# xaskasdf/ntransformer

Measured on AMD Instinct MI355X. Metric: decode tokens/sec (Llama-3.1-8B Q8_0 class, resident weights, greedy, batch 1), higher is better.
Workload: dtype f32; 1 GPU; Llama-3.1-8B-shaped Q8_0 GGUF tensors (seed 20260925), resident in HBM, 16-token prompt, greedy decode; ctx=4096, replicas=1, hipgraph=True

## Files before the change

### include/ntk_engine.h

```cpp
#ifndef NTK_ENGINE_H
#define NTK_ENGINE_H

#include "ntk.h"

#if defined(__GNUC__)
#pragma GCC visibility push(default)
#endif
#ifdef __cplusplus
extern "C" {
#endif

int ntk_rope_kv_store(float* q, const float* k, const float* v, const int* positions, int seq_len, int n_heads, int n_kv_heads, int head_dim,
                      float theta_base, float freq_scale, int interleaved, void* k_cache, void* v_cache, int start_pos, int max_seq, void* stream);
typedef struct ntk_gemv_seg {
    const void* W;
    float*      y;
    int         rows;
    int         dtype;
} ntk_gemv_seg;

int ntk_gemv_fused(const ntk_gemv_seg* segs, int nseg, const float* x, int in_features, const float* norm_w,
                   float eps, const float* resid, int silu_pair, void* stream);

size_t ntk_q8l_bytes(int rows, int in_features);
int ntk_q8l_pack(void* dst, const void* raw, int rows, int in_features, void* stream);
int ntk_q8l_unpack(void* raw, const void* packed, int rows, int in_features, void* stream);

size_t ntk_rp_bytes(int dtype, int rows, int in_features);
int ntk_rp_pack(void* dst, const void* raw, int rows, int in_features, int dtype, void* stream);
int ntk_rp_dequant(float* out, const void* rp, int rows, int in_features, int dtype, void* stream);
int ntk_rp_unpack(void* raw, const void* rp, int rows, int in_features, int dtype, void* stream);
int ntk_gemv_rp(float* y, const void* rp, const float* x, int out_features, int in_features, int weight_dtype, void* stream);
int ntk_gemv_rp_fused(const ntk_gemv_seg* segs, int nseg, const float* x, int in_features, const float* norm_w, float eps,
                      const float* resid, int silu_pair, void* stream);
int ntk_debug_rp_prologue(uint8_t* out, const float* x, const float* norm_w, float eps, int in_features, int nsub, int nwaves, void* stream);
int ntk_debug_mfma_i8_probe(int* D, const int8_t* A, const int8_t* B, void* stream);

int ntk_attention_decode_fused(float* output, const float* q, const float* k, const float* v, void* k_cache,
                               void* v_cache, const int* d_pos, const float* inv_freq, int n_heads, int n_kv_heads,
                               int head_dim, int max_seq, float scale, float theta_base, float freq_scale,
                               void* stream);

size_t ntk_attention_split_scratch_bytes(int n_heads, int head_dim, int nsplit);
int ntk_attention_decode_split(float* output, const float* q, const float* k, const float* v, void* k_cache,
                               void* v_cache, const int* d_pos, const float* inv_freq, int n_heads, int n_kv_heads,
                               int head_dim, int max_seq, float scale, float theta_base, float freq_scale, int nsplit,
                               float* scratch, void* stream);
int ntk_attention_split_scratch_init(float* scratch, int n_heads, void* stream);
int ntk_attention_decode_split_merged(float* output, const float* q, const float* k, const float* v, void* k_cache,
                                      void* v_cache, const int* d_pos, const float* inv_freq, int n_heads, int n_kv_heads,
                                      int head_dim, int max_seq, float scale, float theta_base, float freq_scale, int nsplit,
                                      float* scratch, void* stream);

#define NTK_ATTN_BATCH_MAX 16
typedef struct ntk_kv_batch {
    void* k[NTK_ATTN_BATCH_MAX];
    void* v[NTK_ATTN_BATCH_MAX];
} ntk_kv_batch;
int ntk_attention_decode_batch(float* output, const float* q, const float* k, const float* v, const ntk_kv_batch* caches, const int* positions,
                               int n_rows, const float* inv_freq, int n_heads, int n_kv_heads, int head_dim, int max_seq, float scale,
                               float theta_base, float freq_scale, int nsplit, float* scratch, void* stream);

size_t ntk_kv_q8_cache_bytes(int max_seq, int n_kv_heads, int head_dim);
int ntk_kv_store_q8(void* k_cache, void* v_cache, const float* k, const float* v, int seq_len, int n_kv_heads, int head_dim, int start_pos,
                    int max_seq, void* stream);
int ntk_rope_kv_store_q8(float* q, const float* k, const float* v, const int* positions, int seq_len, int n_heads, int n_kv_heads, int head_dim,
                         float theta_base, float freq_scale, int interleaved, void* k_cache, void* v_cache, int start_pos, int max_seq,
                         void* stream);
int ntk_attention_decode_q8(float* output, const float* q, const float* k, const float* v, void* k_cache, void* v_cache, const int* d_pos,
                            const float* inv_freq, int n_heads, int n_kv_heads, int head_dim, int max_seq, float scale, float theta_base,
                            float freq_scale, int nsplit, float* scratch, void* stream);
int ntk_kv_dequant_q8_f16(void* k_f16, void* v_f16, const void* k_cache, const void* v_cache, int n_rows, int n_kv_heads, int head_dim,
                          int max_seq, void* stream);

int ntk_debug_gemv_fused_form(const ntk_gemv_seg* segs, int nseg, const float* x, int in_features, const float* norm_w, float eps,
                              const float* resid, int silu_pair, int integer_activations, void* stream);

size_t   ntk_tp_comm_bytes(size_t max_floats);
void*    ntk_tp_comm_alloc(size_t bytes);
int      ntk_tp_comm_reset(void* comm, void* stream);
float*   ntk_tp_slot(void* comm, size_t max_floats, unsigned call_index);
int      ntk_tp_allreduce_add(float* hidden, void* const* peers, int rank, int world, size_t max_floats, unsigned call_index, int n, void* stream);
int      ntk_tp_advance_epoch(void* comm, void* stream);
unsigned ntk_tp_error(void* comm);
int      ntk_ipc_export(void* devptr, void* handle64);
int      ntk_ipc_open(const void* handle64, void** devptr);
int      ntk_ipc_close(void* devptr);

int ntk_gemm_quant(float* Y, const void* W, const float* X, int n_tokens, int out_features, int in_features,
                   int weight_dtype, const float* resid, void* stream);

typedef struct ntk_gemm_partials {
    const float* part[3];
    float*       y[3];
    int          rows[3];
    int          nseg, n_tokens, nsplit;
} ntk_gemm_partials;
typedef struct ntk_gemm_desc {
    const ntk_gemv_seg* segs;
    int                 nseg;
    const float*        X;
    int                 n_tokens, in_features;
    const float*        resid;
    void*               workspace;
    size_t              workspace_bytes;
    int                 reuse_x;
    const float*        row_max;
    ntk_gemm_partials*  partials;
    int                 weights_repacked;
    int                 full_form;
} ntk_gemm_desc;
size_t ntk_gemm_quant_workspace_bytes(int in_features, int out_features);
int ntk_gemm_quant_f16(const ntk_gemm_desc* desc, void* stream);
int ntk_reduce_rmsnorm_rowmax(float* hidden, const ntk_gemm_partials* partials, const float* weight, float eps, float* x_out, float* row_max,
                              float* zero_tokens, void* stream);
int ntk_reduce_silu_mul_rowmax(float* output, const ntk_gemm_partials* partials, float* row_max, void* stream);
int ntk_rmsnorm_rowmax(float* output, const float* input, const float* weight, int n_tokens, int hidden_size, float eps, float* row_max,
                       float* zero_tokens, void* stream);
int ntk_silu_mul_rowmax(float* output, const float* gate, const float* up, int n_tokens, int width, float* row_max, void* stream);
int ntk_gemm_prepare_x(const float* X, int n_tokens, int in_features, void* workspace, void* stream);
int ntk_rmsnorm_prepare_x(float* output, const float* input, const float* weight, int n_tokens, int hidden_size, float eps, void* workspace, void* stream);
int ntk_reduce_rmsnorm_prepare_x(float* hidden, const ntk_gemm_partials* partials, const float* weight, float eps, float* x_out, void* workspace, void* stream);
int ntk_silu_mul_prepare_x(float* output, const float* gate, const float* up, int n_tokens, int width, void* workspace, void* stream);
int ntk_reduce_silu_mul_prepare_x(float* output, const ntk_gemm_partials* partials, void* workspace, void* stream);

int ntk_embed_rows(float* out, const void* table, const int* tokens, int n_tokens, int hidden, int dtype,
                   void* stream);

int ntk_argmax(const float* logits, int n, int* d_out_token, int* h_mirror, float* scratch, void* stream);

int ntk_logprob_rows(const float* logits, int n_rows, int vocab, int ld, const int* targets, float* logprob, int* top1, void* stream);

size_t ntk_sample_scratch_bytes(int n);
int ntk_sample_top_k(float* logits, int n, const int* d_recent, int n_recent, float repeat_penalty, float temperature,
                     int top_k, float top_p, float r, int* d_out_token, int* h_mirror, void* scratch, void* stream);
int ntk_repeat_penalty(float* logits, int n, const int* d_recent, int n_recent, float repeat_penalty, void* stream);

#define NTK_SAMPLE_ROWS_MAX 16
typedef struct ntk_sample_rows {
    float temperature[NTK_SAMPLE_ROWS_MAX], top_p[NTK_SAMPLE_ROWS_MAX], repeat_penalty[NTK_SAMPLE_ROWS_MAX], r[NTK_SAMPLE_ROWS_MAX];
    int   top_k[NTK_SAMPLE_ROWS_MAX], n_recent[NTK_SAMPLE_ROWS_MAX];
} ntk_sample_rows;
size_t ntk_sample_rows_scratch_bytes(int n_rows, int vocab);
int ntk_sample_rows_top_k(float* logits, int n_rows, int vocab, int ld, const int* d_recent, int recent_ld, const ntk_sample_rows* rows, int* d_out,
                          int* h_mirror, void* scratch, void* stream);

int ntk_argmax_advance(const float* logits, int n, int* d_out_token, int* h_mirror, unsigned long long* h_ring4, int* d_pos,
                       float* scratch, void* stream);

int ntk_debug_sclk(unsigned long long* d_out2, void* stream);
int ntk_debug_sclk_begin(unsigned* d_flag, unsigned long long* d_out2, void* side_stream);
int ntk_debug_sclk_end(unsigned* d_flag, void* other_stream);

void ntk_debug_malloc_budget(long long bytes);

int ntk_advance_pos(int* d_pos, void* stream);

#ifdef __cplusplus
}
#endif
#if defined(__GNUC__)
#pragma GCC visibility pop
#endif
#endif
```

### ntransformer_amd/_lib.py

```python
from __future__ import annotations

import ctypes as C
import os

_HERE = os.path.dirname(os.path.abspath(__file__))
LIB_PATH = os.environ.get("NTK_LIB_PATH") or os.path.join(_HERE, "libntransformer_hip.so")

NTK_OK = 0
_STATUS = {0: "ok", -1: "unsupported dtype", -2: "bad shape", -3: "HIP launch/runtime error", -4: "misaligned pointer",
           -5: "null pointer", -6: "no usable GPU", -7: "out of memory", -8: "I/O error", -9: "malformed GGUF"}


class NtkError(RuntimeError):
    def __init__(self, status: int, what: str = ""):
        self.status = status
        super().__init__("ntk status %d (%s)%s" % (status, _STATUS.get(status, "?"), (": " + what) if what else ""))


def check(status: int, what: str = "") -> None:
    if status != NTK_OK:
        raise NtkError(status, what)


class KvBatch(C.Structure):
    _fields_ = [("k", C.c_void_p * 16), ("v", C.c_void_p * 16)]


class SampleRows(C.Structure):
    _fields_ = [("temperature", C.c_float * 16), ("top_p", C.c_float * 16), ("repeat_penalty", C.c_float * 16), ("r", C.c_float * 16),
                ("top_k", C.c_int * 16), ("n_recent", C.c_int * 16)]


class GemvSeg(C.Structure):
    _fields_ = [("W", C.c_void_p), ("y", C.c_void_p), ("rows", C.c_int), ("dtype", C.c_int)]


class GemmPartials(C.Structure):
    _fields_ = [("part", C.c_void_p * 3), ("y", C.c_void_p * 3), ("rows", C.c_int * 3), ("nseg", C.c_int), ("n_tokens", C.c_int), ("nsplit", C.c_int)]


class GemmDesc(C.Structure):
    _fields_ = [("segs", C.POINTER(GemvSeg)), ("nseg", C.c_int), ("X", C.c_void_p), ("n_tokens", C.c_int), ("in_features", C.c_int), ("resid", C.c_void_p),
                ("workspace", C.c_void_p), ("workspace_bytes", C.c_size_t), ("reuse_x", C.c_int), ("row_max", C.c_void_p),
                ("partials", C.POINTER(GemmPartials)), ("weights_repacked", C.c_int), ("full_form", C.c_int)]


_lib = None


def lib() -> C.CDLL:
    global _lib
    if _lib is not None:
        return _lib
    if not os.path.exists(LIB_PATH):
        raise ImportError("%s is missing: run `python -c 'import __graft_entry__ as g; g.build()'` "
                          "(hipcc --offload-arch=gfx950); there is no CPU fallback" % LIB_PATH)
    L = C.CDLL(LIB_PATH, mode=C.RTLD_GLOBAL)
    vp, i, f, sz = C.c_void_p, C.c_int, C.c_float, C.c_size_t
    sig = {
        "ntk_abi_version": (i, []),
        "ntk_status_string": (C.c_char_p, [i]),
        "ntk_row_bytes": (sz, [i, C.c_int64]),
        "ntk_device_count": (i, []),
        "ntk_device_init": (i, [i]),
        "ntk_device_name": (i, [C.c_char_p, sz]),
        "ntk_device_mem_info": (i, [C.POINTER(sz), C.POINTER(sz)]),
        "ntk_stream": (vp, [i]),
        "ntk_stream_synchronize": (i, [vp]),
        "ntk_device_synchronize": (i, []),
        "ntk_event_create": (vp, []),
        "ntk_event_destroy": (i, [vp]),
        "ntk_event_record": (i, [vp, vp]),
        "ntk_event_synchronize": (i, [vp]),
        "ntk_event_elapsed_ms": (i, [vp, vp, C.POINTER(f)]),
        "nt_hip_malloc": (vp, [sz]), "nt_hip_free": (None, [vp]),
        "nt_hip_memcpy_h2d": (None, [vp, vp, sz]), "nt_hip_memcpy_d2h": (None, [vp, vp, sz]),
        "nt_hip_memcpy_d2d": (None, [vp, vp, sz]), "nt_hip_memset": (None, [vp, i, sz]),
        "nt_hip_malloc_host": (vp, [sz]), "nt_hip_free_host": (None, [vp]),
        "ntk_memcpy_h2d_async": (i, [vp, vp, sz, vp]), "ntk_memcpy_d2h_async": (i, [vp, vp, sz, vp]),
        "nt_cuda_malloc": (vp, [sz]), "nt_cuda_free": (None, [vp]),
        "nt_cuda_memcpy_h2d": (None, [vp, vp, sz]), "nt_cuda_memcpy_d2h": (None, [vp, vp, sz]),
        "nt_cuda_memcpy_d2d": (None, [vp, vp, sz]), "nt_cuda_memset": (None, [vp, i, sz]),
        "nt_cuda_malloc_host": (vp, [sz]), "nt_cuda_free_host": (None, [vp]),
        "ntk_rmsnorm": (i, [vp, vp, vp, i, i, f, vp]),
        "ntk_rmsnorm_f16": (i, [vp, vp, vp, i, i, f, vp]),
        "ntk_rope": (i, [vp, vp, vp, i, i, i, i, i, f, f, i, vp]),
        "ntk_softmax": (i, [vp, vp, i, i, vp]),
        "ntk_masked_softmax": (i, [vp, vp, vp, i, i, vp]),
        "ntk_gemv": (i, [vp, vp, vp, i, i, i, vp]),
        "ntk_gemv_add": (i, [vp, vp, vp, i, i, i, vp]),
        "ntk_gemm_f32": (i, [vp, vp, vp, i, i, i, vp]),
        "ntk_silu_mul": (i, [vp, vp, vp, i, vp]),
        "ntk_rmsnorm_rowmax": (i, [vp, vp, vp, i, i, f, vp, vp, vp]),
        "ntk_rope_kv_store": (i, [vp, vp, vp, vp, i, i, i, i, f, f, i, vp, vp, i, i, vp]),
        "ntk_silu_mul_rowmax": (i, [vp, vp, vp, i, i, vp, vp]),
        "ntk_add_bias": (i, [vp, vp, i, vp]),
        "ntk_attention_decode": (i, [vp, vp, vp, vp, i, i, i, i, i, f, vp]),
        "ntk_attention_prefill": (i, [vp, vp, vp, vp, i, i, i, i, i, i, f, vp]),
        "ntk_copy_to_kv_cache": (i, [vp, vp, vp, vp, i, i, i, i, i, vp]),
        "ntk_add": (i, [vp, vp, vp, i, vp]),
        "ntk_add_inplace": (i, [vp, vp, i, vp]),
        "ntk_copy": (i, [vp, vp, i, vp]),
        "ntk_cosine_similarity": (i, [vp, vp, vp, i, vp]),
        "ntk_gemv_fused": (i, [C.POINTER(GemvSeg), i, vp, i, vp, f, vp, i, vp]),
        "ntk_debug_gemv_fused_form": (i, [C.POINTER(GemvSeg), i, vp, i, vp, f, vp, i, i, vp]),
        "ntk_q8l_bytes": (sz, [i, i]),
        "ntk_q8l_pack": (i, [vp, vp, i, i, vp]),
        "ntk_q8l_unpack": (i, [vp, vp, i, i, vp]),
        "ntk_rp_bytes": (sz, [i, i, i]),
        "ntk_rp_pack": (i, [vp, vp, i, i, i, vp]),
        "ntk_rp_dequant": (i, [vp, vp, i, i, i, vp]),
        "ntk_rp_unpack": (i, [vp, vp, i, i, i, vp]),
        "ntk_gemv_rp": (i, [vp, vp, vp, i, i, i, vp]),
        "ntk_gemv_rp_fused": (i, [C.POINTER(GemvSeg), i, vp, i, vp, f, vp, i, vp]),
        "ntk_debug_rp_prologue": (i, [vp, vp, vp, f, i, i, i, vp]),
        "ntk_debug_mfma_i8_probe": (i, [vp, vp, vp, vp]),
        "ntk_gemm_quant": (i, [vp, vp, vp, i, i, i, i, vp, vp]),
        "ntk_attention_decode_split": (i, [vp, vp, vp, vp, vp, vp, vp, vp, i, i, i, i, f, f, f, i, vp, vp]),
        "ntk_attention_split_scratch_bytes": (C.c_size_t, [i, i, i]),
        "ntk_attention_split_scratch_init": (i, [vp, i, vp]),
        "ntk_attention_decode_split_merged": (i, [vp, vp, vp, vp, vp, vp, vp, vp, i, i, i, i, f, f, f, i, vp, vp]),
        "ntk_attention_decode_fused": (i, [vp, vp, vp, vp, vp, vp, vp, vp, i, i, i, i, f, f, f, vp]),
        "ntk_attention_decode_batch": (i, [vp, vp, vp, vp, vp, vp, i, vp, i, i, i, i, f, f, f, i, vp, vp]),
        "ntk_kv_q8_cache_bytes": (C.c_size_t, [i, i, i]),
        "ntk_kv_store_q8": (i, [vp, vp, vp, vp, i, i, i, i, i, vp]),
        "ntk_rope_kv_store_q8": (i, [vp, vp, vp, vp, i, i, i, i, f, f, i, vp, vp, i, i, vp]),
        "ntk_attention_decode_q8": (i, [vp, vp, vp, vp, vp, vp, vp, vp, i, i, i, i, f, f, f, i, vp, vp]),
        "ntk_kv_dequant_q8_f16": (i, [vp, vp, vp, vp, i, i, i, i, vp]),
        "ntk_embed_rows": (i, [vp, vp, vp, i, i, i, vp]),
        "ntk_argmax": (i, [vp, i, vp, vp, vp, vp]),
        "ntk_logprob_rows": (i, [vp, i, i, i, vp, vp, vp, vp]),
        "ntk_sample_rows_scratch_bytes": (C.c_size_t, [i, i]),
        "ntk_sample_rows_top_k": (i, [vp, i, i, i, vp, i, C.POINTER(SampleRows), vp, vp, vp, vp]),
        "ntk_advance_pos": (i, [vp, vp]),
        "ntk_debug_sclk": (i, [vp, vp]),
        "ntk_debug_sclk_begin": (i, [vp, vp, vp]),
        "ntk_debug_sclk_end": (i, [vp, vp]),
    }
    for name, (res, args) in sig.items():
        fn = getattr(L, name)
        fn.restype = res
        fn.argtypes = args
    _lib = L
    return L


EXPORTS_NTK_H = None
```

### ntransformer_amd/csrc/attention.hip

```cpp
#include "common.hip.h"
#include "attention_merge.hip.h"
#include "attention_decode.hip.h"
#include <cfloat>
#include <cstdlib>

namespace ntk {

template <int LPR>
__global__ __launch_bounds__(256) void attention_kernel(float* __restrict__ output, const float* __restrict__ Q,
                                                        const uint16_t* __restrict__ kc, const uint16_t* __restrict__ vc,
                                                        int n_keys_base, int causal, int n_heads, int n_kv_heads, int hd,
                                                        float scale) {
    extern __shared__ __attribute__((aligned(16))) float lds[];
    const int head = blockIdx.x, qi = blockIdx.y;
    const int n_keys = causal ? n_keys_base + qi + 1 : n_keys_base;
    float* qs = lds;
    float* red = qs + hd;
    float* part = red + 16;
    float* sc = part + (blockDim.x >> 6) * hd;
    const size_t qoff = ((size_t)qi * n_heads + head) * hd;
    for (int d = threadIdx.x; d < hd; d += blockDim.x) qs[d] = Q[qoff + d];
    __syncthreads();
    attend<LPR>(output + qoff, qs, kc, vc, n_keys, nullptr, nullptr, head / (n_heads / n_kv_heads), n_kv_heads, hd,
                scale, sc, part, red);
}

template <int LPR>
__global__ __launch_bounds__(256) void attention_decode_fused_kernel(
    float* __restrict__ output, const float* __restrict__ q, const float* __restrict__ k, const float* __restrict__ v,
    uint16_t* __restrict__ kc, uint16_t* __restrict__ vc, const int* __restrict__ d_pos, int n_heads, int n_kv_heads,
    int hd, int max_seq, float scale, float theta, float fscale) {
    attention_decode_fused_row<LPR>(output, q, k, v, kc, vc, d_pos, n_heads, n_kv_heads, hd, max_seq, scale, theta, fscale, (int)blockIdx.x);
}


template <int LPR, int D>
__global__ __launch_bounds__(256) void attention_decode_fused_v3_kernel(
    float* __restrict__ output, const float* __restrict__ q, const float* __restrict__ k, const float* __restrict__ v,
    uint16_t* __restrict__ kc, uint16_t* __restrict__ vc, const int* __restrict__ d_pos, const float* __restrict__ inv_freq,
    int n_heads, int n_kv_heads, int hd, int max_seq, float scale, float theta, float fscale) {
    attention_decode_walk<LPR, D, false>(output, q, k, v, kc, vc, d_pos, inv_freq, n_heads, n_kv_heads, hd, max_seq, scale, theta, fscale,
                                         (int)blockIdx.x, 0, 1);
}

template <int LPR, int D, bool MERGE>
__global__ __launch_bounds__(256) void attention_decode_split_kernel(
    float* __restrict__ part, const float* __restrict__ q, const float* __restrict__ k, const float* __restrict__ v,
    uint16_t* __restrict__ kc, uint16_t* __restrict__ vc, const int* __restrict__ d_pos, const float* __restrict__ inv_freq,
    int n_heads, int n_kv_heads, int hd, int max_seq, float scale, float theta, float fscale, float* __restrict__ output,
    unsigned* __restrict__ counters) {
    const int group = n_heads / n_kv_heads;
    const int kv_head = blockIdx.x % n_kv_heads, head = kv_head * group + blockIdx.x / n_kv_heads;
    const int sp = blockIdx.y, nsplit = gridDim.y;
    attention_decode_walk<LPR, D, true, MERGE>(part + ((size_t)head * nsplit + sp) * (hd + 2), q, k, v, kc, vc, d_pos, inv_freq, n_heads,
                                               n_kv_heads, hd, max_seq, scale, theta, fscale, head, sp, nsplit);
    if constexpr (MERGE) {
        extern __shared__ __attribute__((aligned(16))) float lds[];
        if (!att_merge_arrive(counters + head, nsplit, (int)threadIdx.x, reinterpret_cast<volatile int*>(lds))) return;
        const int wave = (int)threadIdx.x >> 6, lane = (int)threadIdx.x & 63;
        if (64 * wave < hd)
            att_merge_head_wave<1>(output + (size_t)head * hd, part + (size_t)head * nsplit * (hd + 2), hd, nsplit, lane, 64 * wave + lane);
    }
}

__global__ __launch_bounds__(128) void attention_split_combine_kernel(float* __restrict__ output, const float* __restrict__ part,
                                                                      int hd, int nsplit, int n_kv_heads) {
    attention_split_combine_head(output, part, hd, nsplit, n_kv_heads, (int)blockIdx.x, (int)gridDim.x);
}

constexpr int FA_QT = 32;
constexpr int FA_KT = 64;
constexpr int FA_QPW = 8;

template <int LPR>
__global__ __launch_bounds__(256) void attention_prefill_tiled_kernel(float* __restrict__ output, const float* __restrict__ Q,
                                                                     const uint16_t* __restrict__ kc, const uint16_t* __restrict__ vc,
                                                                     int T, int start_pos, int n_heads, int n_kv_heads, float scale) {
    constexpr int HD = 8 * LPR, PPW = 64 / LPR;
    extern __shared__ __attribute__((aligned(16))) uint8_t fa_lds[];
    uint16_t* kt = reinterpret_cast<uint16_t*>(fa_lds);
    uint16_t* vt = kt + FA_KT * HD;
    float* qt = reinterpret_cast<float*>(vt + FA_KT * HD);
    const int head = blockIdx.x, q0 = blockIdx.y * FA_QT;
    const int tid = threadIdx.x, lane = tid & 63, wave = tid >> 6;
    const int kv_head = head / (n_heads / n_kv_heads);
    const size_t stride = (size_t)n_kv_heads * HD;
    const int sub = lane / LPR, part_i = lane % LPR;
    const int nq = min(FA_QT, T - q0);
    for (int i = tid; i < nq * HD; i += 256) qt[i] = Q[((size_t)(q0 + i / HD) * n_heads + head) * HD + (i % HD)];
    float m[FA_QPW], l[FA_QPW], acc[FA_QPW][8];
#pragma unroll
    for (int u = 0; u < FA_QPW; ++u) {
        m[u] = -INFINITY; l[u] = 0.0f;
#pragma unroll
        for (int j = 0; j < 8; ++j) acc[u][j] = 0.0f;
    }
    const int n_keys = start_pos + q0 + nq;
    for (int k0 = 0; k0 < n_keys; k0 += FA_KT) {
        __syncthreads();
        const int nk = min(FA_KT, n_keys - k0);
        for (int i = tid; i < nk * LPR; i += 256) {
            const int r = i / LPR, c = i % LPR;
            const size_t g = (size_t)(k0 + r) * stride + (size_t)kv_head * HD + 8 * c;
            *reinterpret_cast<u32x4*>(kt + r * HD + 8 * c) = *reinterpret_cast<const u32x4*>(kc + g);
            *reinterpret_cast<u32x4*>(vt + r * HD + 8 * c) = *reinterpret_cast<const u32x4*>(vc + g);
        }
        __syncthreads();
#pragma unroll
        for (int u = 0; u < FA_QPW; ++u) {
            const int qi = wave * FA_QPW + u;
            if (qi >= nq) continue;
            const int last = start_pos + q0 + qi;
            if (k0 > last) continue;
            float qreg[8];
#pragma unroll
            for (int j = 0; j < 8; ++j) qreg[j] = qt[qi * HD + 8 * part_i + j];
            const int kend = min(nk, last - k0 + 1);
            for (int r0 = 0; r0 < kend; r0 += PPW) {
                const int r = r0 + sub, rr = min(r, kend - 1);
                float kf[8], vf[8];
                unpack8(*reinterpret_cast<const u32x4*>(kt + rr * HD + 8 * part_i), kf);
                unpack8(*reinterpret_cast<const u32x4*>(vt + rr * HD + 8 * part_i), vf);
                float sc = 0.0f;
#pragma unroll
                for (int j = 0; j < 8; ++j) sc = fmaf(qreg[j], kf[j], sc);
                sc = group_sum<LPR>(sc);
                sc = r < kend ? sc * scale : -INFINITY;
                const float mn = fmaxf(m[u], sc);
                const float a = (mn == -INFINITY) ? 1.0f : expf(m[u] - mn), pw = (mn == -INFINITY) ? 0.0f : expf(sc - mn);
                l[u] = fmaf(l[u], a, pw);
#pragma unroll
                for (int j = 0; j < 8; ++j) acc[u][j] = fmaf(acc[u][j], a, pw * vf[j]);
                m[u] = mn;
            }
        }
    }
#pragma unroll
    for (int u = 0; u < FA_QPW; ++u) {
        const int qi = wave * FA_QPW + u;
        if (qi >= nq) continue;
        float mm = m[u], ll = l[u];
#pragma unroll
        for (int off = LPR; off < 64; off <<= 1) {
            const float mo = __shfl_xor(mm, off, 64), lo = __shfl_xor(ll, off, 64);
            const float mn = fmaxf(mm, mo);
            const float wa = (mm == -INFINITY) ? 0.0f : expf(mm - mn), wb = (mo == -INFINITY) ? 0.0f : expf(mo - mn);
            ll = fmaf(ll, wa, lo * wb);
#pragma unroll
            for (int j = 0; j < 8; ++j) acc[u][j] = fmaf(acc[u][j], wa, __shfl_xor(acc[u][j], off, 64) * wb);
            mm = mn;
        }
        if (sub == 0) {
            const float inv = ll > 0.0f ? 1.0f / ll : 0.0f;
            float* o = output + ((size_t)(q0 + qi) * n_heads + head) * HD + 8 * part_i;
#pragma unroll
            for (int j = 0; j < 8; ++j) o[j] = acc[u][j] * inv;
        }
    }
}

__global__ void rope_kernel(float* __restrict__ q, float* __restrict__ k, const int* __restrict__ positions, int seq_len,
                            int n_heads, int n_kv_heads, int head_dim, float theta, float fscale, int interleaved) {
    const int idx = blockIdx.x * blockDim.x + threadIdx.x;
    const int half_dim = head_dim / 2;
    const int total_q = seq_len * n_heads * half_dim, total_k = seq_len * n_kv_heads * half_dim;
    if (idx >= total_q + total_k) return;
    const bool is_key = idx >= total_q;
    const int local = is_key ? idx - total_q : idx;
    const int n_h = is_key ? n_kv_heads : n_heads;
    const int pair = local % half_dim, head = (local / half_dim) % n_h, sp = local / (half_dim * n_h);
    float* data = (is_key ? k : q) + ((size_t)sp * n_h + head) * head_dim;
    const int i0 = interleaved ? 2 * pair : pair, i1 = interleaved ? 2 * pair + 1 : pair + half_dim;
    float a = data[i0], b = data[i1];
    rope_pair(a, b, positions[sp], pair, head_dim, theta, fscale);
    data[i0] = a;
    data[i1] = b;
}

__global__ __launch_bounds__(256) void rope_rows_kernel(float* __restrict__ q, float* __restrict__ k, const int* __restrict__ positions,
                                                        int n_heads, int n_kv_heads, int head_dim, float theta, float fscale, int interleaved) {
    __shared__ float cs[2][128];
    const int sp = blockIdx.x, half_dim = head_dim / 2;
    const int pos = positions[sp];
    for (int i = threadIdx.x; i < half_dim; i += blockDim.x) {
        const float freq = 1.0f / (float)pow((double)theta, (double)((2.0f * i) / head_dim));
        const float angle = pos * freq * fscale;
        cs[0][i] = cosf(angle);
        cs[1][i] = sinf(angle);
    }
    __syncthreads();
    const int total = (n_heads + n_kv_heads) * half_dim;
    for (int idx = threadIdx.x; idx < total; idx += blockDim.x) {
        const int pair = idx % half_dim, head = idx / half_dim;
        float* data = head < n_heads ? q + ((size_t)sp * n_heads + head) * head_dim : k + ((size_t)sp * n_kv_heads + (head - n_heads)) * head_dim;
        const int i0 = interleaved ? 2 * pair : pair, i1 = interleaved ? 2 * pair + 1 : pair + half_dim;
// ... 20 lines not shown
    const bool store = cp < max_seq;
    const int total = (n_heads + n_kv_heads) * half_dim;
    for (int idx = threadIdx.x; idx < total; idx += blockDim.x) {
        const int pair = idx % half_dim, head = idx / half_dim;
        const int i0 = interleaved ? 2 * pair : pair, i1 = interleaved ? 2 * pair + 1 : pair + half_dim;
        const float c = cs[0][pair], sn = cs[1][pair];
        if (head < n_heads) {
            float* data = q + ((size_t)sp * n_heads + head) * head_dim;
            const float a = data[i0], b = data[i1];
            rope_rotate(a, b, c, sn, data[i0], data[i1]);
        } else {
            const int kh = head - n_heads;
            const float* data = k + ((size_t)sp * n_kv_heads + kh) * head_dim;
            float ra, rb;
            rope_rotate(data[i0], data[i1], c, sn, ra, rb);
            if (store) {
                uint16_t* row = kc + (size_t)cp * per_pos + (size_t)kh * head_dim;
                row[i0] = f2h(ra);
                row[i1] = f2h(rb);
            }
        }
    }
    if (store)
        for (int e = threadIdx.x; e < per_pos; e += blockDim.x) vc[(size_t)cp * per_pos + e] = f2h(v[(size_t)sp * per_pos + e]);
}

__global__ void kv_store_kernel(uint16_t* __restrict__ kc, uint16_t* __restrict__ vc, const float* __restrict__ k,
                                const float* __restrict__ v, int total, int per_pos, int start_pos, int max_seq) {
    const int idx = blockIdx.x * blockDim.x + threadIdx.x;
    if (idx >= total) return;
    const int t = idx / per_pos, e = idx % per_pos;
    const int cp = start_pos + t;
    if (cp >= max_seq) return;
    kc[(size_t)cp * per_pos + e] = f2h(k[idx]);
    vc[(size_t)cp * per_pos + e] = f2h(v[idx]);
}

static size_t attn_lds(int hd, int n_keys, int nvec) {
    return sizeof(float) * ((size_t)nvec * hd + 16 + 4 * (size_t)hd + (size_t)n_keys + 1);
}

int launch_attention_decode_kvhead_mfma(float* part, const float* q, const float* k, const float* v, uint16_t* kc, uint16_t* vc,
                                        const int* d_pos, const float* inv_freq, int nh, int nkv, int max_seq, float scale, float theta,
                                        float fscale, int nsplit, float* merged_output, unsigned* counters, hipStream_t st);
int launch_attention_prefill_mfma(float* out, const float* Q, const uint16_t* kc, const uint16_t* vc, int T, int start_pos, int nh, int nkv,
                                  int hd, float scale, hipStream_t st);

static int launch_attention(float* out, const float* Q, const void* kc, const void* vc, int T, int n_keys_base, int causal,
                            int nh, int nkv, int hd, float scale, hipStream_t st) {
    if (nh <= 0 || nkv <= 0 || hd <= 0 || nh % nkv != 0 || T < 0) return NTK_E_SHAPE;
    if (T == 0) return NTK_OK;
    const int max_keys = causal ? n_keys_base + T : n_keys_base;
    const bool aligned = (reinterpret_cast<uintptr_t>(kc) & 15) == 0 && (reinterpret_cast<uintptr_t>(vc) & 15) == 0;
    const uint16_t* k16 = static_cast<const uint16_t*>(kc);
    const uint16_t* v16 = static_cast<const uint16_t*>(vc);
    static const bool tiled_off = NTK_TUNE_ENV_INT("NTK_PREFILL_ATTENTION_1TO1", 0) != 0;
    static const bool mfma_off = NTK_TUNE_ENV_INT("NTK_PREFILL_ATTENTION_NO_MFMA", 0) != 0;
    if (causal && T > 1 && aligned && hd == 128 && !tiled_off && !mfma_off) {
        const int rc = launch_attention_prefill_mfma(out, Q, k16, v16, T, n_keys_base, nh, nkv, hd, scale, st);
        if (rc != NTK_E_SHAPE && rc != NTK_E_ALIGN) return rc;
    }
    if (causal && T > 1 && aligned && (hd == 64 || hd == 128 || hd == 256) && !tiled_off) {
        const size_t fl = (size_t)2 * FA_KT * hd * sizeof(uint16_t) + (size_t)FA_QT * hd * sizeof(float);
        const dim3 fgrid(nh, (T + FA_QT - 1) / FA_QT);
        if (hd == 128) hipLaunchKernelGGL(attention_prefill_tiled_kernel<16>, fgrid, dim3(256), fl, st, out, Q, k16, v16, T, n_keys_base, nh, nkv, scale);
        else if (hd == 64) hipLaunchKernelGGL(attention_prefill_tiled_kernel<8>, fgrid, dim3(256), fl, st, out, Q, k16, v16, T, n_keys_base, nh, nkv, scale);
        else {
            static bool once = hipFuncSetAttribute(reinterpret_cast<const void*>(attention_prefill_tiled_kernel<32>),
                                                   hipFuncAttributeMaxDynamicSharedMemorySize, (int)fl) == hipSuccess;
            if (!once) return NTK_E_LAUNCH;
            hipLaunchKernelGGL(attention_prefill_tiled_kernel<32>, fgrid, dim3(256), fl, st, out, Q, k16, v16, T, n_keys_base, nh, nkv, scale);
        }
        return last_launch_status();
    }
    const size_t lds = attn_lds(hd, max_keys, 1);
    if (lds > 160 * 1024) return NTK_E_SHAPE;
    dim3 grid(nh, T), block(256);
#define NTK_ATT(LPR_)                                                                                                   \
    do {                                                                                                                \
        if (lds > 64 * 1024)                                                                                            \
            (void)hipFuncSetAttribute(reinterpret_cast<const void*>(attention_kernel<LPR_>),                            \
                                      hipFuncAttributeMaxDynamicSharedMemorySize, (int)lds);                            \
        hipLaunchKernelGGL(attention_kernel<LPR_>, grid, block, lds, st, out, Q, k16, v16, n_keys_base, causal, nh, nkv, hd, scale); \
    } while (0)
    if (aligned && hd == 128) NTK_ATT(16);
    else if (aligned && hd == 64) NTK_ATT(8);
    else if (aligned && hd == 256) NTK_ATT(32);
    else NTK_ATT(0);
#undef NTK_ATT
    return last_launch_status();
}

int launch_attention_split_combine(float* output, const float* part, int n_heads, int hd, int nsplit, int n_kv_heads, hipStream_t st) {
    hipLaunchKernelGGL(attention_split_combine_kernel, dim3(n_heads), dim3(128), 0, st, output, part, hd, nsplit, n_kv_heads);
    return last_launch_status();
}

}

extern "C" {

int ntk_rope(float* q, float* k, const int* positions, int , int seq_len, int n_heads, int n_kv_heads,
             int head_dim, float theta_base, float freq_scale, int interleaved, void* stream) {
    if (!q || !k || !positions) return NTK_E_NULL;
    if (seq_len < 0 || n_heads < 0 || n_kv_heads < 0 || head_dim <= 0 || (head_dim & 1)) return NTK_E_SHAPE;
    const int total = seq_len * (n_heads + n_kv_heads) * (head_dim / 2);
    if (total == 0) return NTK_OK;
    if (seq_len >= 4 && head_dim <= 256)
        hipLaunchKernelGGL(ntk::rope_rows_kernel, dim3(seq_len), dim3(256), 0, ntk::resolve_stream(stream), q, k, positions, n_heads, n_kv_heads,
                           head_dim, theta_base, freq_scale, interleaved);
    else
        hipLaunchKernelGGL(ntk::rope_kernel, dim3((total + 255) / 256), dim3(256), 0, ntk::resolve_stream(stream), q, k,
                           positions, seq_len, n_heads, n_kv_heads, head_dim, theta_base, freq_scale, interleaved);
    return ntk::last_launch_status();
}

int ntk_rope_kv_store(float* q, const float* k, const float* v, const int* positions, int seq_len, int n_heads, int n_kv_heads, int head_dim,
                      float theta_base, float freq_scale, int interleaved, void* k_cache, void* v_cache, int start_pos, int max_seq, void* stream) {
    if (!q || !k || !v || !positions || !k_cache || !v_cache) return NTK_E_NULL;
    if (seq_len < 0 || n_heads <= 0 || n_kv_heads <= 0 || head_dim <= 0 || (head_dim & 1) || head_dim > 256 || start_pos < 0 || max_seq <= 0) return NTK_E_SHAPE;
    if (seq_len == 0) return NTK_OK;
    hipLaunchKernelGGL(ntk::rope_kv_store_rows_kernel, dim3(seq_len), dim3(256), 0, ntk::resolve_stream(stream), q, k, v, positions, n_heads, n_kv_heads,
                       head_dim, theta_base, freq_scale, interleaved, static_cast<uint16_t*>(k_cache), static_cast<uint16_t*>(v_cache), start_pos, max_seq);
    return ntk::last_launch_status();
}

int ntk_copy_to_kv_cache(void* k_cache, void* v_cache, const float* k, const float* v, int seq_len, int n_kv_heads,
                         int head_dim, int start_pos, int max_seq, void* stream) {
    if (!k_cache || !v_cache || !k || !v) return NTK_E_NULL;
    if (seq_len < 0 || n_kv_heads <= 0 || head_dim <= 0 || start_pos < 0) return NTK_E_SHAPE;
    const int per = n_kv_heads * head_dim, total = seq_len * per;
    if (total == 0) return NTK_OK;
    hipLaunchKernelGGL(ntk::kv_store_kernel, dim3((total + 255) / 256), dim3(256), 0, ntk::resolve_stream(stream),
                       static_cast<uint16_t*>(k_cache), static_cast<uint16_t*>(v_cache), k, v, total, per, start_pos, max_seq);
    return ntk::last_launch_status();
}

int ntk_attention_decode(float* output, const float* q, const void* k_cache, const void* v_cache, int seq_len, int n_heads,
                         int n_kv_heads, int head_dim, int , float scale, void* stream) {
    if (!output || !q || !k_cache || !v_cache) return NTK_E_NULL;
    if (seq_len <= 0) return NTK_E_SHAPE;
    return ntk::launch_attention(output, q, k_cache, v_cache, 1, seq_len, 0, n_heads, n_kv_heads, head_dim, scale,
                                 ntk::resolve_stream(stream));
}

int ntk_attention_prefill(float* output, const float* Q, const void* k_cache, const void* v_cache, int seq_len, int start_pos,
                          int n_heads, int n_kv_heads, int head_dim, int , float scale, void* stream) {
    if (!output || !Q || !k_cache || !v_cache) return NTK_E_NULL;
    if (seq_len < 0 || start_pos < 0) return NTK_E_SHAPE;
    return ntk::launch_attention(output, Q, k_cache, v_cache, seq_len, start_pos, 1, n_heads, n_kv_heads, head_dim, scale,
                                 ntk::resolve_stream(stream));
}

int ntk_attention_decode_fused(float* output, const float* q, const float* k, const float* v, void* k_cache, void* v_cache,
                               const int* d_pos, const float* inv_freq, int n_heads, int n_kv_heads, int head_dim, int max_seq,
                               float scale, float theta_base, float freq_scale, void* stream) {
    if (!output || !q || !k || !v || !k_cache || !v_cache || !d_pos) return NTK_E_NULL;
    if (n_heads <= 0 || n_kv_heads <= 0 || n_heads % n_kv_heads != 0 || head_dim <= 0 || (head_dim & 1) || max_seq <= 0)
        return NTK_E_SHAPE;
    if ((size_t)max_seq * n_kv_heads * head_dim * 2 >= 0xF0000000ull) return NTK_E_SHAPE;
    hipStream_t st = ntk::resolve_stream(stream);
    const bool aligned = (reinterpret_cast<uintptr_t>(k_cache) & 15) == 0 && (reinterpret_cast<uintptr_t>(v_cache) & 15) == 0;
    uint16_t* k16 = static_cast<uint16_t*>(k_cache);
    uint16_t* v16 = static_cast<uint16_t*>(v_cache);
    if (aligned && (head_dim == 128 || head_dim == 64 || head_dim == 256)) {
        const int G = 4 * (64 / (head_dim / 8));
        const size_t lds = sizeof(float) * ((size_t)3 * head_dim + 2 * G + (size_t)G * head_dim);
#define NTK_ATTV(...) hipLaunchKernelGGL((ntk::attention_decode_fused_v3_kernel<__VA_ARGS__>), dim3(n_heads), dim3(256), lds, st, output, q, k, v, \
                                           k16, v16, d_pos, inv_freq, n_heads, n_kv_heads, head_dim, max_seq, scale, theta_base, freq_scale)
        if (head_dim == 128) NTK_ATTV(16, 4);
        else if (head_dim == 64) NTK_ATTV(8, 4);
        else NTK_ATTV(32, 4);
#undef NTK_ATTV
        return ntk::last_launch_status();
    }
    const size_t lds = ntk::attn_lds(head_dim, max_seq, 3);
    if (lds > 160 * 1024) return NTK_E_SHAPE;
    if (lds > 64 * 1024)
        (void)hipFuncSetAttribute(reinterpret_cast<const void*>(ntk::attention_decode_fused_kernel<0>),
                                  hipFuncAttributeMaxDynamicSharedMemorySize, (int)lds);
    hipLaunchKernelGGL(ntk::attention_decode_fused_kernel<0>, dim3(n_heads), dim3(256), lds, st, output, q, k, v, k16, v16, d_pos,
                       n_heads, n_kv_heads, head_dim, max_seq, scale, theta_base, freq_scale);
    return ntk::last_launch_status();
}

size_t ntk_attention_split_scratch_bytes(int n_heads, int head_dim, int nsplit) {
    return ntk::att_merge_header_bytes(n_heads) + (size_t)n_heads * (size_t)nsplit * (size_t)(head_dim + 2) * sizeof(float);
}

int ntk_attention_split_scratch_init(float* scratch, int n_heads, void* stream) {
    if (!scratch) return NTK_E_NULL;
    if (n_heads <= 0) return NTK_E_SHAPE;
    return hipMemsetAsync(scratch, 0, ntk::att_merge_header_bytes(n_heads), ntk::resolve_stream(stream)) == hipSuccess ? NTK_OK : NTK_E_LAUNCH;
}

static int attention_decode_split_impl(float* output, const float* q, const float* k, const float* v, void* k_cache, void* v_cache,
                                       const int* d_pos, const float* inv_freq, int n_heads, int n_kv_heads, int head_dim, int max_seq,
                                       float scale, float theta_base, float freq_scale, int nsplit, float* scratch_all, void* stream, bool merged) {
    if (!output || !q || !k || !v || !k_cache || !v_cache || !d_pos || !scratch_all) return NTK_E_NULL;
    if (n_heads <= 0 || n_kv_heads <= 0 || n_heads % n_kv_heads != 0 || max_seq <= 0 || nsplit < 1 || nsplit > 1024)
        return NTK_E_SHAPE;
    if (merged && nsplit > ntk::ATT_MERGE_MAX_SPLITS) return NTK_E_SHAPE;
    unsigned* counters = reinterpret_cast<unsigned*>(scratch_all);
    float* scratch = reinterpret_cast<float*>(reinterpret_cast<uint8_t*>(scratch_all) + ntk::att_merge_header_bytes(n_heads));
    if (head_dim != 128 && head_dim != 64 && head_dim != 256) return NTK_E_SHAPE;
    if ((size_t)max_seq * n_kv_heads * head_dim * 2 >= 0xF0000000ull) return NTK_E_SHAPE;
    if ((reinterpret_cast<uintptr_t>(k_cache) & 15) || (reinterpret_cast<uintptr_t>(v_cache) & 15)) return NTK_E_ALIGN;
    hipStream_t st = ntk::resolve_stream(stream);
    uint16_t* k16 = static_cast<uint16_t*>(k_cache);
    uint16_t* v16 = static_cast<uint16_t*>(v_cache);
    static const int kvhead_form = NTK_TUNE_ENV_INT("NTK_ATTN_KVHEAD", 1);
    if (head_dim == 128 && n_heads / n_kv_heads <= 16 && ((kvhead_form == 1 && nsplit >= 16) || kvhead_form == 2)) {
        const int rc = ntk::launch_attention_decode_kvhead_mfma(scratch, q, k, v, k16, v16, d_pos, inv_freq, n_heads, n_kv_heads, max_seq,
                                                                scale, theta_base, freq_scale, nsplit, merged ? output : nullptr, counters, st);
        if (rc != NTK_OK || merged) return rc;
        hipLaunchKernelGGL(ntk::attention_split_combine_kernel, dim3(n_heads), dim3(128), 0, st, output, scratch, head_dim, nsplit, n_kv_heads);
        return ntk::last_launch_status();
    }
    const int G = 4 * (64 / (head_dim / 8));
    const size_t lds = sizeof(float) * ((size_t)3 * head_dim + 2 * G + (size_t)G * head_dim);
#define NTK_ATTSP(...) hipLaunchKernelGGL((ntk::attention_decode_split_kernel<__VA_ARGS__>), dim3(n_heads, nsplit), dim3(256), lds, st, scratch, q, k, \
                                           v, k16, v16, d_pos, inv_freq, n_heads, n_kv_heads, head_dim, max_seq, scale, theta_base, freq_scale, output, counters)
    static const int split_d = NTK_TUNE_ENV_INT("NTK_ATTN_SPLIT_D", 4);
    if (merged) {
        if (head_dim == 128) NTK_ATTSP(16, 4, true);
        else if (head_dim == 64) NTK_ATTSP(8, 4, true);
        else NTK_ATTSP(32, 4, true);
        return ntk::last_launch_status();
    }
    if (head_dim == 128 && split_d == 8) NTK_ATTSP(16, 8, false);
    else if (head_dim == 128) NTK_ATTSP(16, 4, false);
    else if (head_dim == 64) NTK_ATTSP(8, 4, false);
    else NTK_ATTSP(32, 4, false);
#undef NTK_ATTSP
    if (ntk::last_launch_status() != NTK_OK) return NTK_E_LAUNCH;
    hipLaunchKernelGGL(ntk::attention_split_combine_kernel, dim3(n_heads), dim3(128), 0, st, output, scratch, head_dim, nsplit, n_kv_heads);
    return ntk::last_launch_status();
}

int ntk_attention_decode_split(float* output, const float* q, const float* k, const float* v, void* k_cache, void* v_cache,
                               const int* d_pos, const float* inv_freq, int n_heads, int n_kv_heads, int head_dim, int max_seq,
                               float scale, float theta_base, float freq_scale, int nsplit, float* scratch, void* stream) {
    return attention_decode_split_impl(output, q, k, v, k_cache, v_cache, d_pos, inv_freq, n_heads, n_kv_heads, head_dim, max_seq, scale, theta_base,
                                       freq_scale, nsplit, scratch, stream, false);
}

int ntk_attention_decode_split_merged(float* output, const float* q, const float* k, const float* v, void* k_cache, void* v_cache,
                                      const int* d_pos, const float* inv_freq, int n_heads, int n_kv_heads, int head_dim, int max_seq,
                                      float scale, float theta_base, float freq_scale, int nsplit, float* scratch, void* stream) {
    return attention_decode_split_impl(output, q, k, v, k_cache, v_cache, d_pos, inv_freq, n_heads, n_kv_heads, head_dim, max_seq, scale, theta_base,
                                       freq_scale, nsplit, scratch, stream, true);
}

}
```

### ntransformer_amd/csrc/attention_decode.hip.h

```cpp
#pragma once
#include "common.hip.h"
#include "attention_merge.hip.h"
#include <cfloat>
#include <cstdlib>

namespace ntk {

typedef uint32_t u32x4 __attribute__((ext_vector_type(4)));

__device__ __forceinline__ void unpack8(const u32x4 r, float (&f)[8]) {
    f[0] = h2f((uint16_t)(r.x & 0xFFFF)); f[1] = h2f((uint16_t)(r.x >> 16));
    f[2] = h2f((uint16_t)(r.y & 0xFFFF)); f[3] = h2f((uint16_t)(r.y >> 16));
    f[4] = h2f((uint16_t)(r.z & 0xFFFF)); f[5] = h2f((uint16_t)(r.z >> 16));
    f[6] = h2f((uint16_t)(r.w & 0xFFFF)); f[7] = h2f((uint16_t)(r.w >> 16));
}

#ifdef NTK_ATTN_NO_ASM
__device__ __forceinline__ void pv_update(float (&acc)[8], const u32x4 r, const float p) {
    const uint32_t w[4] = {r.x, r.y, r.z, r.w};
#pragma unroll
    for (int i = 0; i < 4; ++i) {
        acc[2 * i] = fmaf(p, h2f((uint16_t)(w[i] & 0xFFFFu)), acc[2 * i]);
        acc[2 * i + 1] = fmaf(p, h2f((uint16_t)(w[i] >> 16)), acc[2 * i + 1]);
    }
}
#else
__device__ __forceinline__ void pv_update(float (&acc)[8], const u32x4 r, const float p) {
    asm("s_nop 1\n\t"
        "v_fma_mix_f32 %0, %8, %12, %0 op_sel_hi:[1,0,0]\n\t"
        "v_fma_mix_f32 %1, %8, %12, %1 op_sel:[1,0,0] op_sel_hi:[1,0,0]\n\t"
        "v_fma_mix_f32 %2, %9, %12, %2 op_sel_hi:[1,0,0]\n\t"
        "v_fma_mix_f32 %3, %9, %12, %3 op_sel:[1,0,0] op_sel_hi:[1,0,0]\n\t"
        "v_fma_mix_f32 %4, %10, %12, %4 op_sel_hi:[1,0,0]\n\t"
        "v_fma_mix_f32 %5, %10, %12, %5 op_sel:[1,0,0] op_sel_hi:[1,0,0]\n\t"
        "v_fma_mix_f32 %6, %11, %12, %6 op_sel_hi:[1,0,0]\n\t"
        "v_fma_mix_f32 %7, %11, %12, %7 op_sel:[1,0,0] op_sel_hi:[1,0,0]"
        : "+v"(acc[0]), "+v"(acc[1]), "+v"(acc[2]), "+v"(acc[3]), "+v"(acc[4]), "+v"(acc[5]), "+v"(acc[6]), "+v"(acc[7])
        : "v"(r.x), "v"(r.y), "v"(r.z), "v"(r.w), "v"(p));
}
#endif

__device__ __forceinline__ void rope_pair(float& x0, float& x1, int pos, int pair_idx, int head_dim, float theta, float fscale) {
    const float freq = 1.0f / (float)pow((double)theta, (double)((2.0f * pair_idx) / head_dim));
    const float angle = pos * freq * fscale;
    const float c = cosf(angle), s = sinf(angle);
    const float a = x0, b = x1;
    rope_rotate(a, b, c, s, x0, x1);
}

template <int LPR>
__device__ void attend(float* out, const float* qs, const uint16_t* kc, const uint16_t* vc, int n_cache,
                       const float* k_extra, const float* v_extra, int kv_head, int n_kv_heads, int hd,
                       float scale, float* sc, float* part, float* red) {
    const int tid = threadIdx.x, lane = tid & 63, wave = tid >> 6, nwaves = blockDim.x >> 6;
    const size_t stride = (size_t)n_kv_heads * hd;
    const uint16_t* kbase = kc + (size_t)kv_head * hd;
    const uint16_t* vbase = vc + (size_t)kv_head * hd;
    const int n_keys = n_cache + (k_extra ? 1 : 0);

    if constexpr (LPR > 0) {
        constexpr int PPW = 64 / LPR;
        const int sub = lane / LPR, part_i = lane % LPR;
        float qreg[8];
#pragma unroll
        for (int j = 0; j < 8; ++j) qreg[j] = qs[8 * part_i + j];
        for (int p0 = wave * PPW; p0 < n_cache; p0 += nwaves * PPW) {
            const int pos = p0 + sub;
            float s = 0.0f;
            if (pos < n_cache) {
                const u32x4 raw = *reinterpret_cast<const u32x4*>(kbase + pos * stride + 8 * part_i);
                float kf[8];
                unpack8(raw, kf);
#pragma unroll
                for (int j = 0; j < 8; ++j) s = fmaf(qreg[j], kf[j], s);
            }
            s = group_sum<LPR>(s);
            if (part_i == 0 && pos < n_cache) sc[pos] = s * scale;
        }
    } else {
        for (int pos = tid; pos < n_cache; pos += blockDim.x) {
            const uint16_t* k = kbase + pos * stride;
            float s = 0.0f;
            for (int d = 0; d < hd; ++d) s = fmaf(qs[d], h2f(k[d]), s);
            sc[pos] = s * scale;
        }
    }
    if (k_extra && wave == 0) {
        float s = 0.0f;
        for (int d = lane; d < hd; d += 64) s = fmaf(qs[d], k_extra[d], s);
        s = wave_sum(s);
        if (lane == 0) sc[n_cache] = s * scale;
    }
    __syncthreads();

    float m = -FLT_MAX;
    for (int pos = tid; pos < n_keys; pos += blockDim.x) m = fmaxf(m, sc[pos]);
    m = block_max(m, red);
    float l = 0.0f;
    for (int pos = tid; pos < n_keys; pos += blockDim.x) {
        const float e = expf(sc[pos] - m);
        sc[pos] = e;
        l += e;
    }
    l = block_sum(l, red);
    const float inv = (l > 0.0f) ? 1.0f / l : 0.0f;
    __syncthreads();

    if constexpr (LPR > 0) {
        constexpr int PPW = 64 / LPR;
        const int sub = lane / LPR, part_i = lane % LPR;
        float acc[8];
#pragma unroll
        for (int j = 0; j < 8; ++j) acc[j] = 0.0f;
        for (int p0 = wave * PPW; p0 < n_cache; p0 += nwaves * PPW) {
            const int pos = p0 + sub;
            if (pos < n_cache) {
                const float pw = sc[pos];
                const u32x4 raw = *reinterpret_cast<const u32x4*>(vbase + pos * stride + 8 * part_i);
                float vf[8];
                unpack8(raw, vf);
#pragma unroll
                for (int j = 0; j < 8; ++j) acc[j] = fmaf(pw, vf[j], acc[j]);
            }
        }
#pragma unroll
        for (int off = LPR; off < 64; off <<= 1) {
#pragma unroll
            for (int j = 0; j < 8; ++j) acc[j] += __shfl_xor(acc[j], off, 64);
        }
        if (sub == 0) {
#pragma unroll
            for (int j = 0; j < 8; ++j) part[wave * hd + 8 * part_i + j] = acc[j];
        }
        __syncthreads();
        for (int d = tid; d < hd; d += blockDim.x) {
            float t = 0.0f;
            for (int w = 0; w < nwaves; ++w) t += part[w * hd + d];
            if (v_extra) t = fmaf(sc[n_cache], v_extra[d], t);
            out[d] = t * inv;
        }
    } else {
        for (int d = tid; d < hd; d += blockDim.x) {
            float t = 0.0f;
            for (int pos = 0; pos < n_cache; ++pos) t = fmaf(sc[pos], h2f(vbase[pos * stride + d]), t);
            if (v_extra) t = fmaf(sc[n_cache], v_extra[d], t);
            out[d] = t * inv;
        }
    }
}

template <int LPR>
__device__ __forceinline__ void attention_decode_fused_row(
    float* __restrict__ output, const float* __restrict__ q, const float* __restrict__ k, const float* __restrict__ v,
    uint16_t* __restrict__ kc, uint16_t* __restrict__ vc, const int* __restrict__ d_pos, int n_heads, int n_kv_heads,
    int hd, int max_seq, float scale, float theta, float fscale, const int head) {
    extern __shared__ __attribute__((aligned(16))) float lds[];
    const int group = n_heads / n_kv_heads, kv_head = head / group;
    const int pos = *d_pos;
    float* qs = lds;
    float* kx = qs + hd;
    float* vx = kx + hd;
    float* red = vx + hd;
    float* part = red + 16;
    float* sc = part + (blockDim.x >> 6) * hd;
    const int half_dim = hd / 2;
    const size_t cache_row = ((size_t)pos * n_kv_heads + kv_head) * hd;
    const bool writer = (head % group == 0) && pos < max_seq;
    for (int i = threadIdx.x; i < half_dim; i += blockDim.x) {
        float a = q[(size_t)head * hd + i], b = q[(size_t)head * hd + i + half_dim];
        rope_pair(a, b, pos, i, hd, theta, fscale);
        qs[i] = a; qs[i + half_dim] = b;
        float ka = k[(size_t)kv_head * hd + i], kb = k[(size_t)kv_head * hd + i + half_dim];
        rope_pair(ka, kb, pos, i, hd, theta, fscale);
        const uint16_t ha = f2h(ka), hb = f2h(kb);
        kx[i] = h2f(ha); kx[i + half_dim] = h2f(hb);
        if (writer) { kc[cache_row + i] = ha; kc[cache_row + i + half_dim] = hb; }
    }
    for (int i = threadIdx.x; i < hd; i += blockDim.x) {
        const uint16_t hv = f2h(v[(size_t)kv_head * hd + i]);
        vx[i] = h2f(hv);
        if (writer) vc[cache_row + i] = hv;
    }
    __syncthreads();
    attend<LPR>(output + (size_t)head * hd, qs, kc, vc, pos, kx, vx, kv_head, n_kv_heads, hd, scale, sc, part, red);
}

template <int LPR, int D, bool SPLIT, bool MERGE = false>
__device__ __forceinline__ void attention_decode_walk(
    float* __restrict__ output, const float* __restrict__ q, const float* __restrict__ k, const float* __restrict__ v,
    uint16_t* __restrict__ kc, uint16_t* __restrict__ vc, const int* __restrict__ d_pos, const float* __restrict__ inv_freq,
    const int n_heads, const int n_kv_heads, const int hd, const int max_seq, const float scale, const float theta, const float fscale,
    const int head, const int sp, const int nsplit) {
    constexpr int PPW = 64 / LPR, NW = 4, G = NW * PPW;
    constexpr float EMPTY = -3.0e38f;
    extern __shared__ __attribute__((aligned(16))) float lds[];
    const int tid = threadIdx.x, lane = tid & 63, wave = tid >> 6;
    const int group = n_heads / n_kv_heads, kv_head = head / group;
    const int stepG = nsplit * G, first = sp * G;
    float* qs = lds;
    float* kx = qs + hd;
    float* vx = kx + hd;
    float* ms = vx + hd;
    float* ls = ms + G;
    float* accs = ls + G;
    const int half_dim = hd / 2;
    const size_t stride = (size_t)n_kv_heads * hd;
    const int sub = lane / LPR, part_i = lane % LPR, g = wave * PPW + sub;
    const uint16_t* kbase = kc + (size_t)kv_head * hd + 8 * part_i;
    const uint16_t* vbase = vc + (size_t)kv_head * hd + 8 * part_i;
    const int pmax = max_seq - 1;

    const int ri = tid & 63, role = tid >> 6;
    float in_a = 0.0f, in_b = 0.0f, in_c = 0.0f, in_d = 0.0f, freq = 0.0f;
    const bool rot = role < 2 && ri < half_dim;
    if (rot) {
        const float* src = role == 0 ? q + (size_t)head * hd : k + (size_t)kv_head * hd;
        in_a = src[ri]; in_b = src[ri + half_dim];
        freq = inv_freq ? inv_freq[ri] : 1.0f / (float)pow((double)theta, (double)((2.0f * ri) / hd));
        if (half_dim > 64) { in_c = src[ri + 64]; in_d = src[ri + 64 + half_dim]; }
    }
    float vin0 = 0.0f, vin1 = 0.0f;
    const int vi = tid - 128;
    if (role >= 2) {
        if (vi < hd) vin0 = v[(size_t)kv_head * hd + vi];
        if (vi + 128 < hd) vin1 = v[(size_t)kv_head * hd + vi + 128];
    }

    const unsigned row_bytes = (unsigned)stride * 2u, off_max = (unsigned)pmax * row_bytes, adv = (unsigned)(stepG * D) * row_bytes;
    const char* kb = reinterpret_cast<const char*>(kbase);
    const char* vb = reinterpret_cast<const char*>(vbase);
    unsigned roff[D];
    u32x4 kraw[D], vraw[D];
#pragma unroll
    for (int d = 0; d < D; ++d) {
        roff[d] = min((unsigned)(first + g + stepG * d) * row_bytes, off_max);
        kraw[d] = *reinterpret_cast<const u32x4*>(kb + roff[d]);
        vraw[d] = *reinterpret_cast<const u32x4*>(vb + roff[d]);
    }
    const int pos = *d_pos;
    const size_t cache_row = (size_t)pos * stride + (size_t)kv_head * hd;
    const bool writer = (head % group == 0) && sp == 0 && pos < max_seq;
    uint16_t st_h[4] = {0, 0, 0, 0};
    if (rot) {
        auto rotate = [&](const int i, const float a, const float b, const float f, uint16_t& ha, uint16_t& hb) {
            const float angle = pos * f * fscale;
            float c, sn;
            sincosf(angle, &sn, &c);
            float ra, rb;
            rope_rotate(a, b, c, sn, ra, rb);
            if (role == 0) { qs[i] = ra; qs[i + half_dim] = rb; }
            else {
                ha = f2h(ra); hb = f2h(rb);
                kx[i] = h2f(ha); kx[i + half_dim] = h2f(hb);
            }
        };
        rotate(ri, in_a, in_b, freq, st_h[0], st_h[1]);
        if (half_dim > 64) {
            const int i2 = ri + 64;
            const float f2 = inv_freq ? inv_freq[i2] : 1.0f / (float)pow((double)theta, (double)((2.0f * i2) / hd));
            rotate(i2, in_c, in_d, f2, st_h[2], st_h[3]);
        }
    }
    if (role >= 2) {
        if (vi < hd) { st_h[0] = f2h(vin0); vx[vi] = h2f(st_h[0]); }
        if (vi + 128 < hd) { st_h[1] = f2h(vin1); vx[vi + 128] = h2f(st_h[1]); }
    }
    __syncthreads();

    float qreg[8];
#pragma unroll
    for (int j = 0; j < 8; ++j) qreg[j] = qs[8 * part_i + j];
    float m = EMPTY, l = 0.0f, acc[8];
#pragma unroll
    for (int j = 0; j < 8; ++j) acc[j] = 0.0f;
    auto batch = [&](const float (*kf)[8], const u32x4* vr, const bool* valid, const int np, const bool masked) {
        float sc[D];
        float mn = m;
#pragma unroll
        for (int d = 0; d < D; ++d) {
            if (d >= np) { sc[d] = EMPTY; continue; }
            float t = 0.0f;
#pragma unroll
            for (int j = 0; j < 8; ++j) t = fmaf(qreg[j], kf[d][j], t);
            t = group_sum<LPR>(t) * scale;
            sc[d] = (!masked || valid[d]) ? t : EMPTY;
            mn = fmaxf(mn, sc[d]);
        }
        const float a = __expf(m - mn);
        l *= a;
#pragma unroll
        for (int j = 0; j < 8; ++j) acc[j] *= a;
#pragma unroll
        for (int d = 0; d < D; ++d) {
            if (d >= np) continue;
            const float pw = (!masked || valid[d]) ? __expf(sc[d] - mn) : 0.0f;
            l += pw;
            pv_update(acc, vr[d], pw);
        }
        m = mn;
    };
    auto walk_batch = [&](const int base, const bool masked) {
        float kf[D][8];
        u32x4 vr[D];
        bool valid[D];
#pragma unroll
        for (int d = 0; d < D; ++d) {
            valid[d] = base + g + stepG * d < pos;
            vr[d] = vraw[d];
            if (masked && !valid[d]) vr[d] = u32x4{0u, 0u, 0u, 0u};
            unpack8(kraw[d], kf[d]);
        }
        __builtin_amdgcn_sched_barrier(0);
        if (base + stepG * D < pos) {
#pragma unroll
            for (int d = 0; d < D; ++d) {
                roff[d] = min(roff[d] + adv, off_max);
                kraw[d] = *reinterpret_cast<const u32x4*>(kb + roff[d]);
                vraw[d] = *reinterpret_cast<const u32x4*>(vb + roff[d]);
            }
        }
        __builtin_amdgcn_sched_barrier(0);
        batch(kf, vr, valid, D, masked);
    };
    int base = first;
    for (; base + stepG * (D - 1) + G <= pos; base += stepG * D) walk_batch(base, false);
    if (base < pos) walk_batch(base, true);
    {
        float kf[D][8];
        u32x4 vr[D];
        bool valid[D];
#pragma unroll
        for (int j = 0; j < 8; ++j) kf[0][j] = kx[8 * part_i + j];
        {
            const float* vxp = vx + 8 * part_i;
            vr[0].x = (uint32_t)f2h(vxp[0]) | ((uint32_t)f2h(vxp[1]) << 16); vr[0].y = (uint32_t)f2h(vxp[2]) | ((uint32_t)f2h(vxp[3]) << 16);
            vr[0].z = (uint32_t)f2h(vxp[4]) | ((uint32_t)f2h(vxp[5]) << 16); vr[0].w = (uint32_t)f2h(vxp[6]) | ((uint32_t)f2h(vxp[7]) << 16);
        }
        valid[0] = first + g == pos % stepG;
        batch(kf, vr, valid, 1, true);
    }
    if (part_i == 0) { ms[g] = m; ls[g] = l; }
#pragma unroll
    for (int j = 0; j < 8; ++j) accs[g * hd + 8 * part_i + j] = acc[j];
    __syncthreads();
    float M = ms[0];
    for (int i = 1; i < G; ++i) M = fmaxf(M, ms[i]);
    if (tid < G) qs[tid] = expf(ms[tid] - M);
    __syncthreads();
    for (int d = tid; d < hd; d += blockDim.x) {
        float L = 0.0f, o = 0.0f;
        for (int i = 0; i < G; ++i) {
            const float w = qs[i];
            L = fmaf(w, ls[i], L);
            o = fmaf(w, accs[i * hd + d], o);
        }
        if constexpr (SPLIT) {
            att_part_store<MERGE>(output + d, o);
            if (d == 0) { att_part_store<MERGE>(output + hd, M); att_part_store<MERGE>(output + hd + 1, L); }
        } else {
            output[(size_t)head * hd + d] = o / L;
        }
    }
    if (writer) {
        if (role == 1 && rot) {
            kc[cache_row + ri] = st_h[0]; kc[cache_row + ri + half_dim] = st_h[1];
            if (half_dim > 64) { kc[cache_row + ri + 64] = st_h[2]; kc[cache_row + ri + 64 + half_dim] = st_h[3]; }
        }
        if (role >= 2) {
            if (vi < hd) vc[cache_row + vi] = st_h[0];
            if (vi + 128 < hd) vc[cache_row + vi + 128] = st_h[1];
        }
    }
}

__device__ __forceinline__ void attention_split_combine_head(float* __restrict__ output, const float* __restrict__ part, int hd, int nsplit,
                                                             int n_kv_heads, const int block, const int nblocks) {
    constexpr int B = 32;
    __shared__ __attribute__((aligned(16))) float wsh[1024], lsh[1024];
    const int group = nblocks / n_kv_heads;
    const int head = (block % n_kv_heads) * group + block / n_kv_heads, tid = threadIdx.x;
    const float* ph = part + (size_t)head * nsplit * (hd + 2);
    const int n32 = (nsplit + B - 1) / B * B;
    float mreg[8], lreg[8];
#pragma unroll
    for (int u = 0; u < 8; ++u) {
        mreg[u] = -INFINITY; lreg[u] = 0.0f;
        if (128 * u < nsplit) {
            const int s0 = tid + 128 * u;
            const float* ps = ph + (size_t)min(s0, nsplit - 1) * (hd + 2) + hd;
            const float mv = ps[0], lv = ps[1];
            if (s0 < nsplit) { mreg[u] = mv; lreg[u] = lv; }
        }
    }
    const int d0 = min(tid, hd - 1);
    float v0[B];
#pragma unroll
    for (int u = 0; u < B; ++u) v0[u] = ph[(size_t)min(u, nsplit - 1) * (hd + 2) + d0];
    __builtin_amdgcn_sched_barrier(0);
#pragma unroll
    for (int u = 0; u < 8; ++u)
        if (tid + 128 * u < n32) { wsh[tid + 128 * u] = mreg[u]; lsh[tid + 128 * u] = lreg[u]; }
    __syncthreads();
    float M = -INFINITY;
    for (int s0 = 0; s0 < n32; s0 += B) {
#pragma unroll
        for (int u = 0; u < B; ++u) M = fmaxf(M, wsh[s0 + u]);
    }
    __syncthreads();
#pragma unroll
    for (int u = 0; u < 8; ++u)
        if (tid + 128 * u < n32) wsh[tid + 128 * u] = (mreg[u] == -INFINITY) ? 0.0f : expf(mreg[u] - M);
    __syncthreads();
    float L = 0.0f;
// ... 24 lines not shown
```

### ntransformer_amd/csrc/elementwise.hip

```cpp
#include "common.hip.h"
#include <cfloat>

namespace ntk {

template <bool HALF_OUT>
__global__ __launch_bounds__(1024) void rmsnorm_kernel(void* __restrict__ output, const float* __restrict__ input,
                                                       const float* __restrict__ weight, int hidden, float eps) {
    __shared__ float red[16];
    const float* x = input + (size_t)blockIdx.x * hidden;
    float ssq = 0.0f;
    for (int i = threadIdx.x; i < hidden; i += blockDim.x) ssq = fmaf(x[i], x[i], ssq);
    const float tot = block_sum(ssq, red);
    const float rms_inv = 1.0f / sqrtf(tot / (float)hidden + eps);
    for (int i = threadIdx.x; i < hidden; i += blockDim.x) {
        const float v = x[i] * rms_inv * weight[i];
        if constexpr (HALF_OUT) reinterpret_cast<uint16_t*>(output)[(size_t)blockIdx.x * hidden + i] = f2h(v);
        else reinterpret_cast<float*>(output)[(size_t)blockIdx.x * hidden + i] = v;
    }
}

template <bool MASKED>
__global__ __launch_bounds__(1024) void softmax_kernel(float* __restrict__ out, const float* __restrict__ in,
                                                       const uint8_t* __restrict__ mask, int cols) {
    __shared__ float red[16];
    const float* x = in + (size_t)blockIdx.x * cols;
    const uint8_t* mk = MASKED ? mask + (size_t)blockIdx.x * cols : nullptr;
    float* y = out + (size_t)blockIdx.x * cols;
    float m = -FLT_MAX;
    for (int i = threadIdx.x; i < cols; i += blockDim.x)
        if (!MASKED || mk[i]) m = fmaxf(m, x[i]);
    m = block_max(m, red);
    float l = 0.0f;
    for (int i = threadIdx.x; i < cols; i += blockDim.x)
        if (!MASKED || mk[i]) l += expf(x[i] - m);
    l = block_sum(l, red);
    const float inv = l > 0.0f ? 1.0f / l : 0.0f;
    for (int i = threadIdx.x; i < cols; i += blockDim.x) y[i] = (!MASKED || mk[i]) ? expf(x[i] - m) * inv : 0.0f;
}

__global__ void silu_mul_kernel(float* __restrict__ out, const float* __restrict__ gate, const float* __restrict__ up, int n) {
    const int i = blockIdx.x * blockDim.x + threadIdx.x;
    if (i < n) {
        const float g = gate[i];
        out[i] = g / (1.0f + expf(-g)) * up[i];
    }
}
__global__ void add_kernel(float* __restrict__ o, const float* __restrict__ a, const float* __restrict__ b, int n) {
    const int i = blockIdx.x * blockDim.x + threadIdx.x;
    if (i < n) o[i] = a[i] + b[i];
}
__global__ void copy_kernel(float* __restrict__ d, const float* __restrict__ s, int n) {
    const int i = blockIdx.x * blockDim.x + threadIdx.x;
    if (i < n) d[i] = s[i];
}
__global__ void gemm_f32_kernel(float* __restrict__ C, const float* __restrict__ A, const float* __restrict__ B, int M, int N, int K) {
    const int col = blockIdx.x * blockDim.x + threadIdx.x, row = blockIdx.y * blockDim.y + threadIdx.y;
    if (row >= M || col >= N) return;
    float s = 0.0f;
    for (int k = 0; k < K; ++k) s = fmaf(A[(size_t)row * K + k], B[(size_t)col * K + k], s);
    C[(size_t)row * N + col] = s;
}
__global__ __launch_bounds__(256) void cosine_kernel(float* __restrict__ result, const float* __restrict__ a,
                                                     const float* __restrict__ b, int n) {
    __shared__ float red[16];
    float d = 0.0f, na = 0.0f, nb = 0.0f;
    for (int i = threadIdx.x; i < n; i += blockDim.x) {
        d = fmaf(a[i], b[i], d); na = fmaf(a[i], a[i], na); nb = fmaf(b[i], b[i], nb);
    }
    d = block_sum(d, red); na = block_sum(na, red); nb = block_sum(nb, red);
    if (threadIdx.x == 0) {
        const float den = sqrtf(na) * sqrtf(nb);
        *result = den > 1e-8f ? d / den : 0.0f;
    }
}

__device__ float embed_elem(const uint8_t* __restrict__ table, int tok, int hidden, int dt, int e) {
    switch (dt) {
        case NTK_DT_F32: return reinterpret_cast<const float*>(table)[(size_t)tok * hidden + e];
        case NTK_DT_F16: return h2f(reinterpret_cast<const uint16_t*>(table)[(size_t)tok * hidden + e]);
        case NTK_DT_Q8_0: {
            const uint8_t* b = table + ((size_t)tok * (hidden / 32) + e / 32) * 34;
            const float d = h2f((uint16_t)(b[0] | (b[1] << 8)));
            return __fmul_rn(d, (float)(int8_t)b[2 + (e & 31)]);
        }
        case NTK_DT_Q4_0: {
            const uint8_t* b = table + ((size_t)tok * (hidden / 32) + e / 32) * 18;
            const float d = h2f((uint16_t)(b[0] | (b[1] << 8)));
            const int j = e & 31;
            const int nib = j < 16 ? (b[2 + j] & 0x0F) : (b[2 + j - 16] >> 4);
            return __fmul_rn(d, (float)(nib - 8));
        }
        case NTK_DT_Q4_K: {
            const uint8_t* b = table + ((size_t)tok * (hidden / 256) + e / 256) * 144;
            const float d = h2f((uint16_t)(b[0] | (b[1] << 8))), dmin = h2f((uint16_t)(b[2] | (b[3] << 8)));
            const int w = e & 255, sub = w >> 5, l = w & 31, chunk = sub >> 1;
            const uint8_t* s = b + 4;
            uint32_t sc, mn;
            if (sub < 4) { sc = s[sub] & 63; mn = s[sub + 4] & 63; }
            else { sc = (s[sub + 4] & 0x0F) | ((s[sub - 4] >> 6) << 4); mn = (s[sub + 4] >> 4) | ((s[sub] >> 6) << 4); }
            const uint8_t qb = b[16 + 32 * chunk + l];
            const int nib = (sub & 1) ? (qb >> 4) : (qb & 0x0F);
            return __fsub_rn(__fmul_rn(__fmul_rn(d, (float)sc), (float)nib), __fmul_rn(dmin, (float)mn));
        }
        case NTK_DT_Q6_K: {
            const uint8_t* b = table + ((size_t)tok * (hidden / 256) + e / 256) * 210;
            const float d = h2f((uint16_t)(b[208] | (b[209] << 8)));
            const int w = e & 255, hf = w >> 7, g = (w >> 5) & 3, l = w & 31, is = l >> 4;
            const uint8_t* ql = b + 64 * hf;
            const uint8_t* qh = b + 128 + 32 * hf;
            const int8_t sc = (int8_t)b[192 + 8 * hf + is + 2 * g];
            const uint8_t qlb = ql[l + 32 * (g & 1)];
            const int lo = (g >> 1) ? (qlb >> 4) : (qlb & 0x0F);
            const int q = (lo | (((qh[l] >> (2 * g)) & 3) << 4)) - 32;
            return __fmul_rn(__fmul_rn(d, (float)sc), (float)q);
        }
        default: return 0.0f;
    }
}
__global__ void embed_rows_kernel(float* __restrict__ out, const uint8_t* __restrict__ table, const int* __restrict__ tokens,
                                  int hidden, int dt) {
    const int tok = tokens[blockIdx.x];
    const int e = blockIdx.y * blockDim.x + threadIdx.x;
    if (e < hidden) out[(size_t)blockIdx.x * hidden + e] = embed_elem(table, tok, hidden, dt, e);
}

__device__ __forceinline__ void amax_merge(float& v, int& i, float ov, int oi) {
    if (ov > v || (ov == v && oi < i)) { v = ov; i = oi; }
}
__global__ __launch_bounds__(256) void argmax_stage1(const float* __restrict__ x, int n, float* __restrict__ sv, int* __restrict__ si) {
    __shared__ float rv[4];
    __shared__ int ri[4];
    float v = -FLT_MAX;
    int idx = 0x7FFFFFFF;
    for (int i = blockIdx.x * blockDim.x + threadIdx.x; i < n; i += gridDim.x * blockDim.x) amax_merge(v, idx, x[i], i);
    for (int off = 32; off > 0; off >>= 1) amax_merge(v, idx, __shfl_xor(v, off, 64), __shfl_xor(idx, off, 64));
    if ((threadIdx.x & 63) == 0) { rv[threadIdx.x >> 6] = v; ri[threadIdx.x >> 6] = idx; }
    __syncthreads();
    if (threadIdx.x == 0) {
        for (int w = 1; w < 4; ++w) amax_merge(v, idx, rv[w], ri[w]);
        sv[blockIdx.x] = v; si[blockIdx.x] = idx;
    }
}
__global__ __launch_bounds__(256) void argmax_stage2(const float* __restrict__ sv, const int* __restrict__ si, int nblk,
                                                     int* __restrict__ d_out, int* __restrict__ h_mirror) {
    __shared__ float rv[4];
    __shared__ int ri[4];
    float v = -FLT_MAX;
    int idx = 0x7FFFFFFF;
    for (int i = threadIdx.x; i < nblk; i += blockDim.x) amax_merge(v, idx, sv[i], si[i]);
    for (int off = 32; off > 0; off >>= 1) amax_merge(v, idx, __shfl_xor(v, off, 64), __shfl_xor(idx, off, 64));
    if ((threadIdx.x & 63) == 0) { rv[threadIdx.x >> 6] = v; ri[threadIdx.x >> 6] = idx; }
    __syncthreads();
    if (threadIdx.x == 0) {
        for (int w = 1; w < 4; ++w) amax_merge(v, idx, rv[w], ri[w]);
        if (idx == 0x7FFFFFFF) idx = 0;
        *d_out = idx;
        if (h_mirror) *h_mirror = idx;
    }
}
__global__ void advance_pos_kernel(int* p) { if (threadIdx.x == 0 && blockIdx.x == 0) *p += 1; }

__global__ __launch_bounds__(64) void sclk_probe_kernel(unsigned long long* out) {
    const unsigned long long t0 = __builtin_amdgcn_s_memtime(), r0 = __builtin_amdgcn_s_memrealtime();
    unsigned long long r1 = r0;
    float acc = (float)threadIdx.x;
    while (r1 - r0 < 5000ull) {
#pragma unroll
        for (int i = 0; i < 64; ++i) acc = fmaf(acc, 1.0000001f, 1e-9f);
        r1 = __builtin_amdgcn_s_memrealtime();
    }
    const unsigned long long t1 = __builtin_amdgcn_s_memtime();
    if (threadIdx.x == 0) { out[0] = t1 - t0; out[1] = r1 - r0; }
    if (acc == 12345.678f) out[2] = 0;
}

__global__ __launch_bounds__(64) void sclk_span_kernel(const unsigned* flag, unsigned long long* out) {
    const unsigned long long t0 = __builtin_amdgcn_s_memtime(), r0 = __builtin_amdgcn_s_memrealtime();
    unsigned long long r1 = r0;
    for (;;) {
        __builtin_amdgcn_s_sleep(64);
        r1 = __builtin_amdgcn_s_memrealtime();
        if (__hip_atomic_load(flag, __ATOMIC_RELAXED, __HIP_MEMORY_SCOPE_SYSTEM) != 0u || r1 - r0 > 300000000ull) break;
    }
    const unsigned long long t1 = __builtin_amdgcn_s_memtime();
    if (threadIdx.x == 0) { out[0] = t1 - t0; out[1] = r1 - r0; }
}

__global__ __launch_bounds__(256) void argmax_advance_stage2(const float* __restrict__ sv, const int* __restrict__ si, int nblk,
                                                             int* __restrict__ d_out, int* __restrict__ h_mirror,
                                                             unsigned long long* __restrict__ h_ring, int* __restrict__ d_pos) {
    __shared__ float rv[4];
    __shared__ int ri[4];
    float v = -FLT_MAX;
    int idx = 0x7FFFFFFF;
    for (int i = threadIdx.x; i < nblk; i += blockDim.x) amax_merge(v, idx, sv[i], si[i]);
    for (int off = 32; off > 0; off >>= 1) amax_merge(v, idx, __shfl_xor(v, off, 64), __shfl_xor(idx, off, 64));
    if ((threadIdx.x & 63) == 0) { rv[threadIdx.x >> 6] = v; ri[threadIdx.x >> 6] = idx; }
    __syncthreads();
    if (threadIdx.x == 0) {
        for (int w = 1; w < 4; ++w) amax_merge(v, idx, rv[w], ri[w]);
        if (idx == 0x7FFFFFFF) idx = 0;
        const int pos = *d_pos;
        *d_out = idx;
        if (h_mirror) *h_mirror = idx;
        if (h_ring)
            __hip_atomic_store(h_ring + (pos & 3), (unsigned long long)(unsigned)idx | ((unsigned long long)(unsigned)(pos + 1) << 32),
                               __ATOMIC_RELEASE, __HIP_MEMORY_SCOPE_SYSTEM);
        *d_pos = pos + 1;
    }
}

static inline dim3 g1(int n) { return dim3((n + 255) / 256); }

}

extern "C" {
using namespace ntk;

static int rms_block(int hidden) { return hidden <= 1024 ? 256 : (hidden <= 4096 ? 512 : 1024); }

int ntk_rmsnorm(float* output, const float* input, const float* weight, int batch_size, int hidden_size, float eps, void* stream) {
    if (!output || !input || !weight) return NTK_E_NULL;
    if (batch_size < 0 || hidden_size <= 0) return NTK_E_SHAPE;
    if (batch_size == 0) return NTK_OK;
    hipLaunchKernelGGL(rmsnorm_kernel<false>, dim3(batch_size), dim3(rms_block(hidden_size)), 0, resolve_stream(stream),
                       (void*)output, input, weight, hidden_size, eps);
    return last_launch_status();
}
int ntk_rmsnorm_f16(void* output, const float* input, const float* weight, int batch_size, int hidden_size, float eps, void* stream) {
    if (!output || !input || !weight) return NTK_E_NULL;
    if (batch_size < 0 || hidden_size <= 0) return NTK_E_SHAPE;
    if (batch_size == 0) return NTK_OK;
    hipLaunchKernelGGL(rmsnorm_kernel<true>, dim3(batch_size), dim3(rms_block(hidden_size)), 0, resolve_stream(stream),
                       output, input, weight, hidden_size, eps);
    return last_launch_status();
}
int ntk_softmax(float* output, const float* input, int rows, int cols, void* stream) {
    if (!output || !input) return NTK_E_NULL;
    if (rows < 0 || cols <= 0) return NTK_E_SHAPE;
    if (rows == 0) return NTK_OK;
    hipLaunchKernelGGL(softmax_kernel<false>, dim3(rows), dim3(cols <= 1024 ? 256 : 1024), 0, resolve_stream(stream), output,
                       input, (const uint8_t*)nullptr, cols);
    return last_launch_status();
}
int ntk_masked_softmax(float* output, const float* input, const uint8_t* mask, int rows, int cols, void* stream) {
    if (!output || !input || !mask) return NTK_E_NULL;
    if (rows < 0 || cols <= 0) return NTK_E_SHAPE;
    if (rows == 0) return NTK_OK;
    hipLaunchKernelGGL(softmax_kernel<true>, dim3(rows), dim3(cols <= 1024 ? 256 : 1024), 0, resolve_stream(stream), output,
                       input, mask, cols);
    return last_launch_status();
}
int ntk_gemm_f32(float* C, const float* A, const float* B, int M, int N, int K, void* stream) {
    if (!C || !A || !B) return NTK_E_NULL;
    if (M < 0 || N < 0 || K < 0) return NTK_E_SHAPE;
    if (M == 0 || N == 0) return NTK_OK;
    hipLaunchKernelGGL(gemm_f32_kernel, dim3((N + 15) / 16, (M + 15) / 16), dim3(16, 16), 0, resolve_stream(stream), C, A, B, M, N, K);
    return last_launch_status();
}
int ntk_silu_mul(float* output, const float* gate, const float* up, int size, void* stream) {
    if (!output || !gate || !up) return NTK_E_NULL;
    if (size < 0) return NTK_E_SHAPE;
    if (size == 0) return NTK_OK;
    hipLaunchKernelGGL(silu_mul_kernel, g1(size), dim3(256), 0, resolve_stream(stream), output, gate, up, size);
    return last_launch_status();
}
int ntk_add(float* out, const float* a, const float* b, int size, void* stream) {
    if (!out || !a || !b) return NTK_E_NULL;
    if (size < 0) return NTK_E_SHAPE;
    if (size == 0) return NTK_OK;
    hipLaunchKernelGGL(add_kernel, g1(size), dim3(256), 0, resolve_stream(stream), out, a, b, size);
    return last_launch_status();
}
int ntk_add_inplace(float* a, const float* b, int size, void* stream) { return ntk_add(a, a, b, size, stream); }
int ntk_add_bias(float* y, const float* bias, int size, void* stream) { return ntk_add(y, y, bias, size, stream); }
int ntk_copy(float* dst, const float* src, int size, void* stream) {
    if (!dst || !src) return NTK_E_NULL;
    if (size < 0) return NTK_E_SHAPE;
    if (size == 0) return NTK_OK;
    hipLaunchKernelGGL(copy_kernel, g1(size), dim3(256), 0, resolve_stream(stream), dst, src, size);
    return last_launch_status();
}
int ntk_cosine_similarity(float* result, const float* a, const float* b, int size, void* stream) {
    if (!result || !a || !b) return NTK_E_NULL;
    if (size < 0) return NTK_E_SHAPE;
    hipLaunchKernelGGL(cosine_kernel, dim3(1), dim3(256), 0, resolve_stream(stream), result, a, b, size);
    return last_launch_status();
}
int ntk_embed_rows(float* out, const void* table, const int* tokens, int n_tokens, int hidden, int dtype, void* stream) {
    if (!out || !table || !tokens) return NTK_E_NULL;
    if (n_tokens < 0 || hidden <= 0) return NTK_E_SHAPE;
    if (n_tokens == 0) return NTK_OK;
    hipLaunchKernelGGL(embed_rows_kernel, dim3(n_tokens, (hidden + 255) / 256), dim3(256), 0, resolve_stream(stream), out, (const uint8_t*)table,
                       tokens, hidden, dtype);
    const int st = last_launch_status();
    if (st != NTK_OK) return st;
    switch (dtype) {
        case NTK_DT_F32: case NTK_DT_F16: case NTK_DT_Q8_0: case NTK_DT_Q4_0: case NTK_DT_Q4_K: case NTK_DT_Q6_K: return NTK_OK;
        default: return NTK_E_DTYPE;
    }
}
int ntk_argmax(const float* logits, int n, int* d_out_token, int* h_mirror, float* scratch, void* stream) {
    if (!logits || !d_out_token || !scratch) return NTK_E_NULL;
    if (n <= 0) return NTK_E_SHAPE;
    const int nblk = n < 256 * 8 ? 1 : (n / (256 * 8) < 1024 ? n / (256 * 8) : 1024);
    float* sv = scratch;
    int* si = reinterpret_cast<int*>(scratch + 1024);
    hipStream_t st = resolve_stream(stream);
    hipLaunchKernelGGL(argmax_stage1, dim3(nblk), dim3(256), 0, st, logits, n, sv, si);
    hipLaunchKernelGGL(argmax_stage2, dim3(1), dim3(256), 0, st, (const float*)sv, (const int*)si, nblk, d_out_token, h_mirror);
    return last_launch_status();
}
int ntk_argmax_advance(const float* logits, int n, int* d_out_token, int* h_mirror, unsigned long long* h_ring4, int* d_pos, float* scratch,
                       void* stream) {
    if (!logits || !d_out_token || !scratch || !d_pos) return NTK_E_NULL;
    if (n <= 0) return NTK_E_SHAPE;
    const int nblk = n < 256 * 8 ? 1 : (n / (256 * 8) < 1024 ? n / (256 * 8) : 1024);
    float* sv = scratch;
    int* si = reinterpret_cast<int*>(scratch + 1024);
    hipStream_t st = resolve_stream(stream);
    hipLaunchKernelGGL(argmax_stage1, dim3(nblk), dim3(256), 0, st, logits, n, sv, si);
    hipLaunchKernelGGL(argmax_advance_stage2, dim3(1), dim3(256), 0, st, (const float*)sv, (const int*)si, nblk, d_out_token, h_mirror, h_ring4, d_pos);
    return last_launch_status();
}
int ntk_debug_sclk(unsigned long long* d_out2, void* stream) {
    if (!d_out2) return NTK_E_NULL;
    hipLaunchKernelGGL(sclk_probe_kernel, dim3(1), dim3(64), 0, resolve_stream(stream), d_out2);
    return last_launch_status();
}
int ntk_debug_sclk_begin(unsigned* d_flag, unsigned long long* d_out2, void* side_stream) {
    if (!d_flag || !d_out2 || !side_stream) return NTK_E_NULL;
    hipStream_t st = static_cast<hipStream_t>(side_stream);
    if (hipMemsetAsync(d_flag, 0, 4, st) != hipSuccess) return NTK_E_LAUNCH;
    hipLaunchKernelGGL(sclk_span_kernel, dim3(1), dim3(64), 0, st, (const unsigned*)d_flag, d_out2);
    return last_launch_status();
}
int ntk_debug_sclk_end(unsigned* d_flag, void* other_stream) {
    if (!d_flag || !other_stream) return NTK_E_NULL;
    static const unsigned one = 1u;
    return hipMemcpyAsync(d_flag, &one, 4, hipMemcpyHostToDevice, static_cast<hipStream_t>(other_stream)) == hipSuccess ? NTK_OK : NTK_E_LAUNCH;
}
int ntk_advance_pos(int* d_pos, void* stream) {
    if (!d_pos) return NTK_E_NULL;
    hipLaunchKernelGGL(advance_pos_kernel, dim3(1), dim3(64), 0, resolve_stream(stream), d_pos);
    return last_launch_status();
}

}
```

### ntransformer_amd/csrc/engine/capi.cpp

```cpp
#include "../../../include/ntransformer.h"
#include "../../../include/ntk_engine.h"
#include "engine.h"

#include <cstdlib>
#include <cstring>
#include <new>
#include <thread>

using nt::Engine;

namespace {
Engine* E(nt_engine_t e) { return static_cast<Engine*>(e); }
nt::SynthSpec to_spec(const nt_synth_spec& s) {
    nt::SynthSpec o;
    o.hidden = s.hidden; o.inter = s.inter; o.layers = s.layers; o.heads = s.heads; o.kv_heads = s.kv_heads;
    o.vocab = s.vocab; o.ctx = s.ctx; o.eps = s.eps; o.theta = s.theta; o.bos = s.bos; o.eos = s.eos;
    o.mix = s.mix ? s.mix : "Q8_0";
    o.seed = s.seed;
    return o;
}
int threads_or_default(int n) {
    if (n > 0) return n;
    const int h = (int)std::thread::hardware_concurrency();
    return h > 0 ? h : 8;
}
}

extern "C" {

nt_engine_t nt_engine_create(void) { return new (std::nothrow) Engine(); }
void nt_engine_destroy(nt_engine_t e) { delete E(e); }

int nt_engine_load(nt_engine_t e, const char* path) { return nt_engine_load_ex(e, path, 4096); }

int nt_engine_load_ex(nt_engine_t e, const char* path, int max_context) {
    if (!e || !path) return NTK_E_NULL;
    try { return E(e)->load(path, max_context > 0 ? max_context : 4096); } catch (...) { return NTK_E_NOMEM; }
}

int nt_engine_load_synthetic(nt_engine_t e, const nt_synth_spec* spec, int max_context) {
    if (!e || !spec) return NTK_E_NULL;
    try { return E(e)->load_synthetic(to_spec(*spec), max_context > 0 ? max_context : 4096); } catch (...) { return NTK_E_NOMEM; }
}

int nt_engine_load_shared(nt_engine_t e, nt_engine_t src, int max_context) {
    if (!e || !src || e == src) return NTK_E_NULL;
    try { return E(e)->load_shared(*E(src), max_context > 0 ? max_context : 4096); } catch (...) { return NTK_E_NOMEM; }
}

int nt_engine_set_option(nt_engine_t e, const char* key, const char* value) {
    if (!e || !key || !value) return NTK_E_NULL;
    const bool on = atoi(value) != 0;
    const std::string k = key;
    if (k == "fused") E(e)->options().fused = on;
    else if (k == "graph") E(e)->options().graph = on;
    else if (k == "batched_prefill") { E(e)->options().batched_prefill = on; E(e)->model().set_batched_prefill(on); }
    else if (k == "device_sampling") E(e)->options().device_sampling = on;
    else if (k == "f16_prefill" || k == "bf16_prefill") E(e)->model().set_bf16_prefill(on);
    else if (k == "fuse_attention") { const int rc = E(e)->model().set_fuse_attention(on); if (rc != NTK_OK) E(e)->set_error(E(e)->model().error()); return rc; }
    else if (k == "kv_cache") {
        const int rc = E(e)->loaded() ? (E(e)->set_error("kv_cache must be set before the model is loaded"), NTK_E_SHAPE) : E(e)->model().set_kv_cache(value);
        if (rc != NTK_OK && !E(e)->loaded()) E(e)->set_error(E(e)->model().error());
        return rc;
    }
    else if (k == "sequences") {
        const int rc = E(e)->loaded() ? (E(e)->set_error("sequences must be set before the model is loaded"), NTK_E_SHAPE) : E(e)->model().set_sequences(atoi(value));
        if (rc != NTK_OK && !E(e)->loaded()) E(e)->set_error(E(e)->model().error());
        return rc;
    }
    else if (k == "prefill_row_max") E(e)->model().set_prefill_row_max(on);
    else if (k == "prefill_fused_split") E(e)->model().set_prefill_fused_split(on);
    else if (k == "attention_merge") return E(e)->model().set_attention_merge(on);
    else if (k == "repack") return E(e)->model().set_repack(atoi(value));
    else if (k == "persistent") { E(e)->options().persistent = on; E(e)->model().set_persistent(atoi(value)); }
    else if (k == "score_rows") {
        const int rc = E(e)->model().set_score_rows(atoi(value));
        if (rc != NTK_OK) E(e)->set_error(E(e)->model().error());
        return rc;
    }
    else if (k == "synth_threads") E(e)->options().synth_threads = atoi(value);
    else return NTK_E_SHAPE;
    return NTK_OK;
}

const char* nt_engine_last_error(nt_engine_t e) { return e ? E(e)->error().c_str() : "null engine"; }

void nt_gen_params_default(nt_gen_params* p) {
    if (!p) return;
    const nt::GenerateConfig d;
    p->max_tokens = d.max_tokens; p->temperature = d.temperature; p->top_k = d.top_k; p->top_p = d.top_p;
    p->repeat_penalty = d.repeat_penalty; p->repeat_window = d.repeat_window; p->seed = d.seed; p->stop_at_eos = 1;
}

char* nt_engine_generate(nt_engine_t e, const char* prompt, int max_tokens, float temperature, int top_k, float top_p) {
    if (!e || !prompt || !E(e)->loaded()) return nullptr;
    try {
        nt::GenerateConfig c;
        c.max_tokens = max_tokens; c.temperature = temperature; c.top_k = top_k; c.top_p = top_p;
        c.verbose = false;
        const std::string out = E(e)->generate(prompt, c);
        char* r = static_cast<char*>(malloc(out.size() + 1));
        if (!r) return nullptr;
        memcpy(r, out.c_str(), out.size() + 1);
        return r;
    } catch (...) { return nullptr; }
}
void nt_free(char* p) { free(p); }

int nt_engine_vocab_size(nt_engine_t e) { return e && E(e)->loaded() ? E(e)->model().config().vocab_size : -1; }
int nt_engine_n_layers(nt_engine_t e) { return e && E(e)->loaded() ? E(e)->model().config().n_layers : -1; }
int nt_engine_hidden_size(nt_engine_t e) { return e && E(e)->loaded() ? E(e)->model().config().hidden_size : -1; }
int nt_engine_max_context(nt_engine_t e) { return e && E(e)->loaded() ? E(e)->model().config().max_seq_len : -1; }

int nt_engine_generate_tokens(nt_engine_t e, const int* prompt, int n_prompt, const nt_gen_params* p, int* out, int out_cap) {
    if (!e || !prompt || !p || (!out && out_cap > 0)) return NTK_E_NULL;
    if (n_prompt <= 0) return NTK_E_SHAPE;
    try {
        nt::GenerateConfig c;
        c.max_tokens = p->max_tokens; c.temperature = p->temperature; c.top_k = p->top_k; c.top_p = p->top_p;
        c.repeat_penalty = p->repeat_penalty; c.repeat_window = p->repeat_window; c.seed = p->seed;
        std::vector<int> gen;
        const int rc = E(e)->generate_tokens(std::vector<int>(prompt, prompt + n_prompt), c, gen, p->stop_at_eos != 0);
        if (rc != NTK_OK) return rc;
        const int n = (int)std::min<size_t>(gen.size(), (size_t)out_cap);
        for (int i = 0; i < n; ++i) out[i] = gen[i];
        return n;
    } catch (...) { return NTK_E_NOMEM; }
}

int nt_engine_last_stats(nt_engine_t e, nt_stats* o) {
    if (!e || !o) return NTK_E_NULL;
    const nt::Stats& s = E(e)->last_stats();
    o->prompt_tokens = s.prompt_tokens; o->gen_tokens = s.gen_tokens; o->prefill_ms = s.prefill_ms;
    o->decode_ms = s.decode_ms; o->decode_tok_s = s.decode_tok_s();
    return NTK_OK;
}

int nt_engine_forward(nt_engine_t e, const int* tokens, int n, int start_pos, float* logits_out) {
    if (!e || !tokens || !logits_out) return NTK_E_NULL;
    if (!E(e)->loaded()) return NTK_E_NULL;
    float* d = E(e)->model().forward(tokens, n, start_pos);
    if (!d) return NTK_E_LAUNCH;
    return E(e)->model().copy_logits(logits_out);
}

int nt_engine_seq_forward(nt_engine_t e, int slot, const int* tokens, int n, int start_pos, float* logits_out) {
    if (!e || !tokens || !logits_out) return NTK_E_NULL;
    if (!E(e)->loaded()) return NTK_E_NULL;
    if (slot < 0 || slot >= E(e)->model().sequences()) { E(e)->set_error("seq_forward: no such sequence slot"); return NTK_E_SHAPE; }
    float* d = E(e)->model().forward(tokens, n, start_pos, slot);
    if (!d) { E(e)->set_error(E(e)->model().error()); return NTK_E_LAUNCH; }
    return E(e)->model().copy_logits(logits_out);
}

int nt_engine_decode_batch(nt_engine_t e, const int* slots, const int* tokens, const int* positions, int n, float* logits_out, int* next_out) {
    if (!e || !E(e)->loaded()) return NTK_E_NULL;
    try {
        const int rc = E(e)->model().decode_batch(slots, tokens, positions, n, logits_out, next_out);
        if (rc != NTK_OK) E(e)->set_error(E(e)->model().error());
        return rc;
    } catch (...) { return NTK_E_NOMEM; }
}

int nt_engine_generate_batch(nt_engine_t e, const int* const* prompts, const int* prompt_lens, int n, const nt_gen_params* p, int* out, int out_stride,
                             int* out_counts) {
    if (!e || !prompts || !prompt_lens || !p || !out || !out_counts) return NTK_E_NULL;
    try { return E(e)->generate_batch(prompts, prompt_lens, n, *p, out, out_stride, out_counts); } catch (...) { return NTK_E_NOMEM; }
}

int nt_engine_decode_batch_sample(nt_engine_t e, const int* slots, const int* tokens, const int* positions, int n, const nt_gen_params* params,
                                  const int* const* recent, const int* n_recent, const float* r, float* logits_out, int* next_out) {
    if (!e || !E(e)->loaded()) return NTK_E_NULL;
    try { return E(e)->decode_batch_sample(slots, tokens, positions, n, params, recent, n_recent, r, logits_out, next_out); } catch (...) { return NTK_E_NOMEM; }
}

int nt_engine_generate_batch_ex(nt_engine_t e, const int* const* prompts, const int* prompt_lens, int n, const nt_gen_params* params, int* out, int out_stride,
                                int* out_counts) {
    if (!e || !prompts || !prompt_lens || !params || !out || !out_counts) return NTK_E_NULL;
    try { return E(e)->generate_batch_ex(prompts, prompt_lens, n, params, out, out_stride, out_counts); } catch (...) { return NTK_E_NOMEM; }
}

int nt_batch_validate(const int* slots, const int* tokens, const int* positions, int n, int sequences, int max_seq, int vocab) {
    return nt::Model::validate_batch(slots, tokens, positions, n, sequences, max_seq, vocab, nullptr);
}

int nt_engine_score_tokens(nt_engine_t e, const int* tokens, const int* targets, int n, int start_pos, float* logprob_out, int* top1_out) {
    if (!e || !tokens || !targets || !logprob_out) return NTK_E_NULL;
    try {
        const int rc = E(e)->score(tokens, targets, n, start_pos, logprob_out, top1_out);
        if (rc != NTK_OK) return rc;
        int scored = 0;
        for (int i = 0; i < n; ++i) scored += targets[i] >= 0;
        return scored;
    } catch (...) { return NTK_E_NOMEM; }
}

int nt_engine_decode_fused(nt_engine_t e, int token, int pos, int use_graph, float* logits_out) {
    if (!e || !logits_out || !E(e)->loaded()) return NTK_E_NULL;
    nt::Model& m = E(e)->model();
    if (pos < 0 || pos >= m.config().max_seq_len) return NTK_E_SHAPE;
    m.set_device_pos(pos);
    int rc = m.set_device_token(token);
    if (rc != NTK_OK) return rc;
    rc = m.decode_step_fused(false, use_graph != 0);
    if (rc != NTK_OK) return rc;
    rc = m.copy_logits(logits_out);
    if (rc != NTK_OK) return rc;
    return m.check_persistent();
}

int nt_engine_debug_run_layers(nt_engine_t e, const float* hidden_in, int n_tokens, int start_pos, int first_layer, int n_layers, int mode,
                               float* hidden_out) {
    if (!e || !E(e)->loaded()) return NTK_E_NULL;
    return E(e)->model().debug_run_layers(hidden_in, n_tokens, start_pos, first_layer, n_layers, mode, hidden_out);
}
int nt_engine_debug_kv_read(nt_engine_t e, int layer, int pos0, int n, uint16_t* k_out, uint16_t* v_out) {
    if (!e || !E(e)->loaded()) return NTK_E_NULL;
    return E(e)->model().debug_kv(layer, pos0, n, k_out, v_out, false);
}
int nt_engine_debug_kv_read_slot(nt_engine_t e, int slot, int layer, int pos0, int n, uint16_t* k_out, uint16_t* v_out) {
    if (!e || !E(e)->loaded()) return NTK_E_NULL;
    return E(e)->model().debug_kv(layer, pos0, n, k_out, v_out, false, slot);
}
int nt_engine_debug_kv_write(nt_engine_t e, int layer, int pos0, int n, const uint16_t* k, const uint16_t* v) {
    if (!e || !E(e)->loaded()) return NTK_E_NULL;
// ... 216 lines not shown
```

### ntransformer_amd/csrc/engine/model.cpp

```cpp
#include "model_impl.h"
#include <thread>

namespace nt {

Model::~Model() { free_all(); }

void Model::drop_graphs(int slot) {
    for (auto& row : graphs_)
        for (int k = 0; k <= kAttnRegimes; ++k) {
            if (slot >= 0 && k != slot) continue;
            if (row[k]) (void)hipGraphExecDestroy(reinterpret_cast<hipGraphExec_t>(row[k]));
            row[k] = nullptr;
        }
}

void Model::free_all() {
    drop_graphs();
    destroy_persistent_plan();
    persistent_on_ = false;
    for (int r = 0; r < 8; ++r) {
        if (tp_peer_opened_[r] && tp_peers_[r]) (void)ntk_ipc_close(tp_peers_[r]);
        tp_peers_[r] = nullptr;
        tp_peer_opened_[r] = false;
    }
    tp_connected_ = false;
    tp_comm_ = nullptr;
    tp_call_ = 0;
    if (own_stream_ && stream_) (void)hipStreamDestroy(static_cast<hipStream_t>(stream_));
    own_stream_ = false;
    stream_ = nullptr;
    for (void* p : allocs_) nt_hip_free(p);
    allocs_.clear();
    auto free_host = [](auto*& p) { if (p) nt_hip_free_host(p); p = nullptr; };
    free_host(h_token_); free_host(h_ring_); free_host(h_recent_); free_host(h_batch_recent_); free_host(h_batch_next_);
    sample_scratch_ = gemm_ws_ = gemm_ws2_ = nullptr;
    d_recent_ = nullptr;
    attn_sync_ = nullptr;
    shares_weights_ = false;
    layers_.clear();
    token_embd_ = output_norm_ = output_ = DevTensor();
    weight_bytes_ = repack_bytes_ = raw_freed_bytes_ = 0;
    raw_scratch_ = nullptr; raw_scratch_bytes_ = raw_cursor_ = 0; raw_err_ = 0;
    repack_done_ = output_tied_ = false;
    host_pos_ = attn_regime_ = 0;
    k_cache_ = v_cache_ = nullptr;
    slot_k_.clear(); slot_v_.clear();
    batch_logits_ = batch_logprob_ = batch_attn_scratch_ = nullptr; batch_in_ = batch_next_ = batch_recent_ = nullptr; batch_sample_scratch_ = nullptr;
    kv_capture_ = nullptr; kv_capture_layer_ = -1; kv_capture_T_ = 0;
    k_cache_q8_ = v_cache_q8_ = nullptr; kv_f16_k_ = kv_f16_v_ = nullptr; kv_q8_layer_bytes_ = 0; kv_cache_bytes_ = 0;
    hidden_ = residual_ = workspace_ = logits_ = argmax_scratch_ = rope_inv_freq_ = attn_scratch_ = row_max_ = nullptr;
    positions_ = tokens_dev_ = d_pos_ = d_token_ = nullptr;
    score_logits_ = score_logprob_ = nullptr; score_targets_ = score_top1_ = nullptr; score_cap_ = 0;
    score_ws_ = nullptr; score_ws_bytes_ = 0;
}

int Model::share_weights(const Model& src, int max_context) {
    if (&src == this) { err_ = "share_weights: a model cannot share its own weights"; return NTK_E_NULL; }
    free_all();
    if (src.layers_.empty()) { err_ = "share_weights: the source model is not loaded"; return NTK_E_NULL; }
    if (src.tp_world_ != 1 || src.shares_weights_) {
        err_ = "share_weights: the source must hold whole tensors of its own (no tensor parallelism, not itself a sharing sequence)";
        return NTK_E_SHAPE;
    }
    cfg_ = src.cfg_;
    cfg_full_ = src.cfg_;
    if (max_context > 0) cfg_.max_seq_len = max_context;
    vocab_ = src.vocab_;
    layers_ = src.layers_;
    token_embd_ = src.token_embd_; output_norm_ = src.output_norm_; output_ = src.output_;
    output_tied_ = src.output_tied_;
    weight_bytes_ = src.weight_bytes_;
    repack_ = src.repack_; repack_wanted_ = src.repack_; repack_done_ = true;
    repack_bytes_ = 0;
    shares_weights_ = true;
    if (src.raw_freed_bytes_ > 0 && src.raw_scratch_bytes_ > 0) {
        void* d = nt_hip_malloc(src.raw_scratch_bytes_);
        if (!d) { err_ = "share_weights: no device memory for the unpack scratch"; free_all(); return NTK_E_NOMEM; }
        allocs_.push_back(d);
        raw_scratch_ = d; raw_scratch_bytes_ = src.raw_scratch_bytes_;
        raw_freed_bytes_ = src.raw_freed_bytes_;
    }
    int rc = own_stream();
    if (rc == NTK_OK) rc = alloc_buffers();
    if (rc != NTK_OK) free_all();
    return rc;
}

int Model::set_attention_merge(bool on) {
    if (on == attn_merge_) return NTK_OK;
    if (!layers_.empty()) {
        NT_TRY(sync());
        drop_graphs();
    }
    attn_merge_ = on;
    return NTK_OK;
}

int Model::set_repack(int level) {
    level = level < 0 ? 0 : level > 3 ? 3 : level;
    if (shares_weights_) { err_ = "set_repack: this sequence shares another model's tensors"; return NTK_E_SHAPE; }
    repack_wanted_ = level;
    if (layers_.empty()) { repack_ = level; return NTK_OK; }
    if (level == 3) level = 2;
    if (level == repack_) return NTK_OK;
    NT_TRY(sync());
    drop_graphs();
    int rc = NTK_OK;
    if (level < 2 && raw_freed_bytes_ > 0) rc = restore_raw_all();
    if (rc == NTK_OK && level > 0 && !repack_done_) {
        rc = repack_all();
        if (rc == NTK_E_NOMEM) { fprintf(stderr, "warning: decode repack incomplete (device memory): the rest stays on the raw path\n"); rc = NTK_OK; err_.clear(); }
    }
    if (rc != NTK_OK) { err_ = std::string("set_repack: ") + ntk_status_string(rc); return rc; }
    repack_ = level;
    if (level == 2) {
        destroy_persistent_plan();
        persistent_on_ = false;
        rc = drop_raw_all();
    }
    return rc;
}

uint64_t Model::bytes_per_token(int pos) const {
    uint64_t b = 0;
    for (const auto& L : layers_)
        for (auto m : kLayerMatrices) b += (L.*m).nbytes;
    b += output_.nbytes;
    b += (uint64_t)(2 * cfg_.n_layers + 1) * cfg_.hidden_size * 4;
    const uint64_t kv_elems = (uint64_t)cfg_.n_kv_heads * cfg_.head_dim;
    const uint64_t kv_row = kv_q8_ ? kv_elems + kv_elems / 16 : kv_elems * 2;
    b += 2ull * cfg_.n_layers * kv_row * (uint64_t)(pos + 1) + 2ull * cfg_.n_layers * kv_row;
    b += ntk_row_bytes(token_embd_.dtype, cfg_.hidden_size);
    return b;
}

int Model::set_device_token(int token) {
    if (token < 0 || token >= cfg_.vocab_size) { err_ = "token id out of range"; return NTK_E_SHAPE; }
    *h_token_ = token;
    return ntk_memcpy_h2d_async(d_token_, h_token_, 4, stream_);
}
int Model::set_device_pos(int pos) {
    host_pos_ = pos;
    NT_TRY(ntk_memcpy_h2d_async(d_pos_, &pos, 4, stream_));
    NT_TRY(ntk_stream_synchronize(stream_));
    if (h_ring_) memset(h_ring_, 0, 64);
    return NTK_OK;
}
int Model::sync() { return ntk_stream_synchronize(stream_); }
int Model::host_token() const { return *h_token_; }
int Model::copy_logits(float* host) {
    NT_TRY(ntk_memcpy_d2h_async(host, logits_, (size_t)cfg_.vocab_size * 4, stream_));
    return ntk_stream_synchronize(stream_);
}

int Model::sample_on_device(const int* recent, int n_recent, float repeat_penalty, float temperature, int top_k, float top_p, float r) {
    if (!sample_scratch_ || !d_recent_ || !h_recent_) return NTK_E_NOMEM;
    if (n_recent > kRecentCap) { recent += n_recent - kRecentCap; n_recent = kRecentCap; }
    void* s = stream_;
    if (repeat_penalty > 1.0f && n_recent > 0) {
        memcpy(h_recent_, recent, (size_t)n_recent * 4);
        NT_TRY(ntk_memcpy_h2d_async(d_recent_, h_recent_, (size_t)n_recent * 4, s));
    } else {
        n_recent = 0;
    }
    if (temperature <= 0.0f) {
        NT_TRY(ntk_repeat_penalty(logits_, cfg_.vocab_size, d_recent_, n_recent, repeat_penalty, s));
        return ntk_argmax(logits_, cfg_.vocab_size, d_token_, h_token_, argmax_scratch_, s);
    }
    return ntk_sample_top_k(logits_, cfg_.vocab_size, d_recent_, n_recent, repeat_penalty, temperature, top_k, top_p, r, d_token_,
                            h_token_, sample_scratch_, s);
}

int Model::wait_token(int pos, int* token) {
    volatile unsigned long long* slot = h_ring_ + (pos & 3);
    const unsigned want = (unsigned)(pos + 1);
    for (unsigned spins = 0;; ++spins) {
        const unsigned long long v = *slot;
        if ((unsigned)(v >> 32) == want) { *token = (int)(unsigned)v; return NTK_OK; }
#if defined(__x86_64__) || defined(__i386__)
        __builtin_ia32_pause();
#else
        std::this_thread::yield();
#endif
        if ((spins & 0xFFFFu) == 0xFFFFu) {
            const auto now = std::chrono::steady_clock::now();
            if (spins == 0xFFFFu) wait_t0_ = now;
            else if (std::chrono::duration<double>(now - wait_t0_).count() > 2.0) break;
        }
    }
    static bool warned = false;
    if (!warned) { warned = true; fprintf(stderr, "warning: the pinned token ring was not seen updating for 2 s (host memory not coherent with a running kernel?); falling back to a stream synchronisation per token\n"); }
    NT_TRY(ntk_stream_synchronize(stream_));
    const unsigned long long v = *slot;
    if ((unsigned)(v >> 32) != want) { err_ = "decode step finished without publishing its token"; return NTK_E_LAUNCH; }
    *token = (int)(unsigned)v;
    return NTK_OK;
}

int Model::set_sequences(int n) {
    if (n < 1 || n > kMaxSequences) { err_ = "sequences must lie in 1 .. " + std::to_string(kMaxSequences); return NTK_E_SHAPE; }
    sequences_ = n;
    return NTK_OK;
}

int Model::set_kv_cache(const std::string& kind) {
    if (kind != "f16" && kind != "q8_0") { err_ = "kv_cache: unknown format '" + kind + "' (f16 or q8_0)"; return NTK_E_DTYPE; }
    if (!layers_.empty()) { err_ = "kv_cache must be set before the model is loaded"; return NTK_E_SHAPE; }
    const bool q8 = kind == "q8_0";
    if (q8 && fuse_attention_) { err_ = "kv_cache=q8_0 is not supported with the attention-inside-Wo launch (fuse_attention)"; return NTK_E_SHAPE; }
    kv_q8_ = q8;
    return NTK_OK;
}

int Model::set_fuse_attention(bool on) {
    if (on && kv_q8_) { err_ = "fuse_attention (attention inside the Wo launch) is not supported with kv_cache=q8_0"; return NTK_E_SHAPE; }
    fuse_attention_ = on;
    return NTK_OK;
}

bool Model::use_persistent_now() const {
    return persistent_plan_ && persistent_on_ && attn_regime_ == 0 && !prof_;
}

void Model::set_persistent(int level) {
    const bool on = level != 0;
    persistent_on_ = false;
    persistent_wanted_ = level;
    if (on && !experiments_built()) fprintf(stderr, "note: the persistent token kernels are built by experiments/Makefile only (experiments/libntransformer_hip_exp.so); this library decodes with fused launches\n");
    if (persistent_plan_ && persistent_kind_ != (level == 2 ? 2 : 1)) {
        (void)sync();
        destroy_persistent_plan();
    }
    if (!on || tp_world_ != 1 || layers_.empty()) return;
    if (kv_q8_) { fprintf(stderr, "note: the persistent token kernels read the F16 KV cache; kv_cache=q8_0 decodes with fused launches\n"); return; }
    if (raw_freed_bytes_ > 0) (void)set_repack(1);
    if (!persistent_plan_) (void)build_persistent_plan(level == 2 ? 2 : 1);
    persistent_on_ = persistent_plan_ != nullptr;
}

const char* Model::decode_path() const {
    if (persistent_plan_ && persistent_on_ && persistent_kind_ == 2)
        return attn_regime_ == 0 ? "persistent layer engine (1 launch per token: loader / consumer waves, granule hand-offs; fused launches beyond the single-pass attention regime)"
                                 : "fused (5 launches/layer; persistent layer engine below the split-attention regime)";
    if (persistent_plan_ && persistent_on_)
        return attn_regime_ == 0 ? "persistent (1 launch per token in the single-pass attention regime, fused launches beyond)"
                                 : "fused (5 launches/layer; persistent below the split-attention regime)";
    return "fused (5 launches/layer)";
}

int Model::check_persistent() {
    NT_TRY(check_tp());
    return check_experiments();
}

Model::Views Model::views(int T) const {
    const size_t qd = (size_t)T * cfg_.n_heads * cfg_.head_dim, kvd = (size_t)T * cfg_.n_kv_heads * cfg_.head_dim;
    float* const q = workspace_;
    return {q, q + qd, q + qd + kvd, q + qd + 2 * kvd, workspace_, workspace_ + (size_t)T * cfg_.intermediate_size};
}

int Model::init_device() {
    const char* e = getenv("NTK_DEVICE");
    const int st = ntk_device_init(e ? atoi(e) : 0);
    if (st != NTK_OK) err_ = "no usable GPU (HIP device init failed)";
    return st;
}

int Model::own_stream() {
    hipStream_t own = nullptr;
    if (hipStreamCreateWithFlags(&own, hipStreamNonBlocking) != hipSuccess) { err_ = "stream creation failed"; return NTK_E_LAUNCH; }
    stream_ = own;
    own_stream_ = true;
    return NTK_OK;
}

}
```

### ntransformer_amd/csrc/engine/model.h

```cpp
#pragma once
#include <array>
#include <chrono>
#include <cstdint>
#include <string>
#include <vector>
#include "gguf.h"
#include "synth.h"

struct ntk_sample_rows;

struct ihipGraphExec_t;

namespace nt {

struct DevTensor {
    void* ptr = nullptr;
    int dtype = 0;
    int64_t in_f = 0, out_f = 0;
    size_t nbytes = 0;
    void* rp = nullptr;
    size_t rp_bytes = 0;
};

struct LayerWeights {
    DevTensor attn_norm, wq, wk, wv, wo, ffn_norm, w_gate, w_up, w_down;
};
inline constexpr std::array<DevTensor LayerWeights::*, 7> kLayerMatrices = {&LayerWeights::wq, &LayerWeights::wk, &LayerWeights::wv, &LayerWeights::wo,
                                                                            &LayerWeights::w_gate, &LayerWeights::w_up, &LayerWeights::w_down};

enum Shard { WHOLE, ROWS, COLS };

class Model {
public:
    Model() = default;
    ~Model();
    Model(const Model&) = delete;
    Model& operator=(const Model&) = delete;

    int load(const std::string& gguf_path, int max_context);
    int load_synthetic(const SynthSpec& spec, int max_context, int nthreads);
    int share_weights(const Model& src, int max_context);

    float* forward(const int* tokens, int seq_len, int start_pos, int slot = 0);

    int score(const int* tokens, const int* targets, int seq_len, int start_pos, float* logprob_out, int* top1_out, int slot = 0);

    static constexpr int kMaxSequences = 16;
    int set_sequences(int n);
    int sequences() const { return sequences_; }
    int decode_batch(const int* slots, const int* tokens, const int* positions, int B, float* logits_out, int* next_out);
    static constexpr int kMaxRecent = 4096;
    int decode_batch_sample(const int* slots, const int* tokens, const int* positions, int B, const ntk_sample_rows& rows, const int* const* recent,
                            float* logits_out, float* const* row_logits, int* next_out);
    static int validate_batch(const int* slots, const int* tokens, const int* positions, int B, int sequences, int max_seq, int vocab, std::string* why);
    int set_score_rows(int rows);

    int decode_step_fused(bool greedy, bool use_graph);
    int set_device_token(int token);
    int set_device_pos(int pos);
    static constexpr int kAttnRegimes = 3;
    static int attention_regime(int pos, int head_dim) {
        if (pos < 544) return 0;
        return pos < (head_dim == 128 ? 3072 : 16384) ? 1 : 2;
    }
    static int attention_splits(int regime, int head_dim) { return regime <= 1 ? 8 : head_dim == 128 ? 32 : 16; }
    static constexpr int kMaxAttnSplits = 32;
    void pick_attention_regime();
    int sync();
    int host_token() const;
    int wait_token(int pos, int* token);
    float* logits_ptr() { return logits_; }
    int copy_logits(float* host);
    int sample_on_device(const int* recent, int n_recent, float repeat_penalty, float temperature, int top_k, float top_p, float r);
    static bool device_sampler_supports(float temperature, int top_k, int vocab) {
        return temperature <= 0.0f || (top_k > 0 && top_k <= 64 && top_k < vocab && vocab <= 131072);
    }

    const ModelConfig& config() const { return cfg_; }
    const GgufVocab& vocab() const { return vocab_; }
    const std::string& error() const { return err_; }
    uint64_t weight_bytes() const { return weight_bytes_; }
    uint64_t bytes_per_token(int pos) const;
    void set_batched_prefill(bool on) { batched_prefill_ = on; }
    void set_persistent(int level);
    int persistent_kind() const { return persistent_plan_ ? persistent_kind_ : 0; }
    int set_fuse_attention(bool on);
    int set_kv_cache(const std::string& kind);
    bool kv_q8() const { return kv_q8_; }
    static int kv_q8_splits(int regime) { return regime == 0 ? 4 : regime == 1 ? 16 : 32; }
    uint64_t kv_cache_bytes() const { return kv_cache_bytes_; }
    int debug_kv_inputs_capture(int layer);
    int debug_kv_inputs_read(int n, float* k, float* v);
    int debug_kv_q8(int layer, int pos0, int n, uint8_t* k_blocks, uint8_t* v_blocks, bool write);
    void set_prefill_row_max(bool on) { prefill_row_max_ = on; }
    void set_prefill_fused_split(bool on) { prefill_fused_split_ = on; }
    int set_attention_merge(bool on);
    int set_repack(int level);
    bool repack() const { return repack_ != 0; }
    int repack_level() const { return repack_; }
    uint64_t repack_bytes() const { return repack_bytes_; }
    uint64_t resident_weight_bytes() const { return weight_bytes_ - raw_freed_bytes_ + repack_bytes_ + raw_scratch_bytes_; }
    void set_bf16_prefill(bool on) { bf16_prefill_ = on; }
    bool persistent_available() const { return persistent_plan_ != nullptr; }
    void* persistent_plan() const { return persistent_plan_; }
    const char* decode_path() const;
    int check_persistent();
    int check_tp();
    int debug_run_layers(const float* hidden_in, int T, int start_pos, int first, int count, int mode, float* hidden_out);
    int debug_kv(int layer, int pos0, int n, uint16_t* k, uint16_t* v, bool write, int slot = 0);
    int profile_token(float ms[4], int calls[4], bool coarse);
    void* stream() const { return stream_; }

    int tp_configure(int rank, int world);
    int tp_rank() const { return tp_rank_; }
    int tp_world() const { return tp_world_; }
    int tp_export(void* handle64, void** raw);
    int tp_connect(const void* handles, void* const* raws);
    unsigned tp_error();
    static int slice_columns(void* dst, const void* src, int dtype, int64_t out_f, int64_t in_f, int rank, int world);

private:
    int load_impl(const std::string& gguf_path, int max_context);
    int finish_load();
    int init_device();
    int own_stream();
    int alloc_buffers();
    int upload(DevTensor& dst, const void* host, int dtype, int64_t in_f, int64_t out_f, size_t nbytes);
    int upload_shard(DevTensor& dst, const void* host_full, int dtype, int64_t in_f, int64_t out_f, size_t nbytes_full, Shard how);
    struct TensorSlot { DevTensor* dst; Shard how; int64_t in_f, out_f; };
    bool slot_of(const std::string& name, TensorSlot* slot);
    template <class F> void for_each_projection(F&& fn) { for (auto& L : layers_) for (auto m : kLayerMatrices) fn(L.*m); fn(output_); }
    int repack_all();
    int repack_one(DevTensor& t);
    int drop_raw_all();
    int restore_raw_all();
    void raw_begin() { raw_cursor_ = 0; }
    const void* raw_of(const DevTensor& t);
    int tp_check_shapes();
    int tp_allreduce(float* hidden, int n);
    float* tp_slot() const;
    void free_all();
    void drop_graphs(int slot = -1);
    struct Views { float *q, *k, *v, *attn_out, *gate, *up; };
    Views views(int T) const;
    int enqueue_token(bool greedy);
    int enqueue_layers(int first, int last);
    int decode_project(const DevTensor* const* ws, float* const* ys, int n, const float* x, const DevTensor* norm, const float* resid, int kind,
                       int silu_pair = 0, bool timed = true);
    struct KvTarget { int slot; const int* slots; int max_pos; };
    int layers_1to1(int T, int start_pos, int first, int last, const KvTarget& kv = KvTarget{0, nullptr, 0});
    int lm_head(float* logits, const float* X, int n, const float* row_max);
    bool lm_head_f16() const;
    int lm_head_workspace(const char* who);
    int batch_buffers();
    int batch_logits(const int* slots, const int* tokens, const int* positions, int B);
    int batch_sample_buffers();
    int score_buffers();
    void prof_mark(int cls, bool begin);
    bool use_persistent_now() const;
    static bool experiments_built();
    int build_persistent_plan(int kind);
    void destroy_persistent_plan();
    int launch_persistent();
    int attention_in_wo(const LayerWeights& L, int layer);
    int check_experiments();

    ModelConfig cfg_;
    GgufVocab vocab_;
    std::string err_;
    std::vector<LayerWeights> layers_;
    DevTensor token_embd_, output_norm_, output_;
    bool output_tied_ = false;
    uint64_t weight_bytes_ = 0;
    std::vector<void*> allocs_;
    bool shares_weights_ = false;

    uint16_t* k_cache_ = nullptr;
    uint16_t* v_cache_ = nullptr;
    bool kv_q8_ = false;
    int sequences_ = 1;
    std::vector<uint16_t*> slot_k_, slot_v_;
    float* batch_logits_ = nullptr;
    int* batch_in_ = nullptr;
    int batch_host_[3 * 16] = {};
    float* batch_logprob_ = nullptr;
    int* batch_next_ = nullptr;
    float* batch_attn_scratch_ = nullptr;
    int* batch_recent_ = nullptr;
    int* h_batch_recent_ = nullptr;
    void* batch_sample_scratch_ = nullptr;
    int* h_batch_next_ = nullptr;
    uint8_t* k_cache_q8_ = nullptr;
    uint8_t* v_cache_q8_ = nullptr;
    size_t kv_q8_layer_bytes_ = 0;
    uint16_t* kv_f16_k_ = nullptr;
    uint16_t* kv_f16_v_ = nullptr;
    uint64_t kv_cache_bytes_ = 0;
    float* kv_capture_ = nullptr;
    int kv_capture_layer_ = -1, kv_capture_T_ = 0;
    float* hidden_ = nullptr;
    float* residual_ = nullptr;
    float* workspace_ = nullptr;
    size_t workspace_floats_ = 0;
    float* logits_ = nullptr;
    int score_rows_ = 256;
    float* score_logits_ = nullptr;
    int score_cap_ = 0;
    int* score_targets_ = nullptr;
    float* score_logprob_ = nullptr;
    int* score_top1_ = nullptr;
    void* score_ws_ = nullptr;
    size_t score_ws_bytes_ = 0;
    int* positions_ = nullptr;
    int* tokens_dev_ = nullptr;
    int* d_pos_ = nullptr;
    int* d_token_ = nullptr;
    int* h_token_ = nullptr;
    unsigned long long* h_ring_ = nullptr;
    std::chrono::steady_clock::time_point wait_t0_;
    float* argmax_scratch_ = nullptr;
    void* sample_scratch_ = nullptr;
    int* d_recent_ = nullptr;
    int* h_recent_ = nullptr;
    static constexpr int kRecentCap = kMaxRecent;
    float* rope_inv_freq_ = nullptr;
    void* stream_ = nullptr;
    bool batched_prefill_ = true;
    struct Timed { int cls; void* a; void* b; int n; bool shared_a; };
    bool prof_coarse_ = false;
    std::vector<Timed>* prof_ = nullptr;
    static constexpr int kPersistentSlot = kAttnRegimes;
    ihipGraphExec_t* graphs_[2][kAttnRegimes + 1] = {};
    int host_pos_ = 0;
    int attn_regime_ = 0;
    float* attn_scratch_ = nullptr;
    bool prefill_row_max_ = true;
    float* row_max_ = nullptr;
    void* gemm_ws_ = nullptr;
    void* gemm_ws2_ = nullptr;
    bool prefill_fused_split_ = true;
    size_t gemm_ws_bytes_ = 0;
    bool bf16_prefill_ = true;
    unsigned* attn_sync_ = nullptr;
    int repack_ = 3;
    int repack_wanted_ = 3;
    bool repack_done_ = false;
    uint64_t repack_bytes_ = 0;
    uint64_t raw_freed_bytes_ = 0;
    void* raw_scratch_ = nullptr;
    size_t raw_scratch_bytes_ = 0, raw_cursor_ = 0;
    int raw_err_ = 0;
    bool attn_merge_ = false;
    bool fuse_attention_ = false;
    int tp_rank_ = 0, tp_world_ = 1;
    void* tp_comm_ = nullptr;
    size_t tp_max_floats_ = 0;
    void* tp_peers_[8] = {nullptr, nullptr, nullptr, nullptr, nullptr, nullptr, nullptr, nullptr};
    bool tp_peer_opened_[8] = {false, false, false, false, false, false, false, false};
    bool tp_connected_ = false;
    unsigned tp_call_ = 0;
    bool own_stream_ = false;
    ModelConfig cfg_full_;
    void* persistent_plan_ = nullptr;
    bool persistent_on_ = false;
    int persistent_wanted_ = 0;
    int persistent_kind_ = 1;
};

}
```

### ntransformer_amd/csrc/engine/model_decode.cpp

```cpp
#include "model_impl.h"

namespace nt {

void Model::prof_mark(int cls, bool begin) {
    if (!prof_) return;
    void* s = stream_;
    if (prof_coarse_) {
        if (!begin) return;
        if (!prof_->empty() && prof_->back().cls == cls) { ++prof_->back().n; return; }
        void* e = ntk_event_create();
        ntk_event_record(e, s);
        const bool shared = !prof_->empty();
        if (shared) prof_->back().b = e;
        prof_->push_back({cls, e, nullptr, 1, shared});
        return;
    }
    void* e = ntk_event_create();
    ntk_event_record(e, s);
    if (begin) prof_->push_back({cls, e, nullptr, 1, false}); else prof_->back().b = e;
}

int Model::enqueue_token(bool greedy) {
    const int H = cfg_.hidden_size;
    void* s = stream_;
    tp_call_ = 0;
    prof_mark(2, true);
    const int est = ntk_embed_rows(hidden_, token_embd_.ptr, d_token_, 1, H, token_embd_.dtype, s);
    prof_mark(2, false);
    if (est != NTK_OK && est != NTK_E_DTYPE) return est;
    if (use_persistent_now()) {
        NT_TRY(launch_persistent());
    } else {
        NT_TRY(enqueue_layers(0, cfg_.n_layers));
        const DevTensor* const w = &output_;
        const bool timed = is_quant(w->dtype);
        if (timed) prof_mark(0, true);
        NT_TRY(decode_project(&w, &logits_, 1, hidden_, &output_norm_, nullptr, 16, 0, false));
        if (timed) prof_mark(0, false);
    }
    prof_mark(2, true);
    if (greedy) NT_TRY(ntk_argmax_advance(logits_, cfg_.vocab_size, d_token_, h_token_, h_ring_, d_pos_, argmax_scratch_, s));
    else NT_TRY(ntk_advance_pos(d_pos_, s));
    if (tp_world_ > 1) NT_TRY(ntk_tp_advance_epoch(tp_comm_, s));
    prof_mark(2, false);
    return NTK_OK;
}

int Model::decode_project(const DevTensor* const* ws, float* const* ys, int n, const float* x, const DevTensor* norm, const float* resid, int kind,
                          int silu_pair, bool timed) {
    const int H = cfg_.hidden_size;
    void* s = stream_;
    auto mark = [&](bool begin) { if (timed) prof_mark(0, begin); };
    const float* nw = norm ? (const float*)norm->ptr : nullptr;
    auto one_launch = [&](bool rp, const float* r, int silu) {
        ntk_gemv_seg segs[3];
        if (!rp) raw_begin();
        for (int a = 0; a < n; ++a) segs[a] = {rp ? ws[a]->rp : raw_of(*ws[a]), ys[a], (int)ws[a]->out_f, ws[a]->dtype};
        mark(true);
        const int st = (rp ? ntk_gemv_rp_fused : ntk_gemv_fused)(segs, n, x, (int)ws[0]->in_f, nw, cfg_.norm_eps, r, silu, s);
        mark(false);
        return st;
    };
    bool all_rp = repack_ && (rp_mask() & kind), all_quant = true, mixed = false;
    for (int a = 0; a < n; ++a) {
        all_rp = all_rp && ws[a]->rp != nullptr && ws[a]->in_f == ws[0]->in_f;
        all_quant = all_quant && is_quant(ws[a]->dtype);
        mixed = mixed || ws[a]->dtype != ws[0]->dtype;
    }
    if (all_rp) {
        const int st = one_launch(true, resid, silu_pair);
        if (!not_taken(st)) return st;
    }
    if (n > 1 && !resid && all_quant && mixed) {
        const int st = one_launch(false, nullptr, 0);
        if (!not_taken(st)) return st;
    }
    bool done[3] = {false, false, false};
    for (int a = 0; a < n; ++a) {
        if (done[a]) continue;
        const DevTensor& w = *ws[a];
        if (!is_quant(w.dtype)) {
            const float* xin = x;
            if (nw) {
                NT_TRY(ntk_rmsnorm(residual_ + H, x, nw, 1, (int)w.in_f, cfg_.norm_eps, s));
                xin = residual_ + H;
            }
            float* y = resid ? residual_ : ys[a];
            raw_begin();
            NT_TRY(ntk_gemv(y, raw_of(w), xin, (int)w.out_f, (int)w.in_f, w.dtype, s));
            if (resid) NT_TRY(ntk_add(ys[a], resid, residual_, (int)w.out_f, s));
            done[a] = true;
            continue;
        }
        ntk_gemv_seg segs[3];
        int m = 0;
        raw_begin();
        for (int b = a; b < n; ++b) {
            if (done[b] || ws[b]->dtype != w.dtype) continue;
            segs[m++] = {raw_of(*ws[b]), ys[b], (int)ws[b]->out_f, ws[b]->dtype};
            done[b] = true;
        }
        mark(true);
        NT_TRY(ntk_gemv_fused(segs, m, x, (int)w.in_f, nw, cfg_.norm_eps, resid, silu_pair, s));
        mark(false);
    }
    return NTK_OK;
}

int Model::enqueue_layers(int first, int last_layer) {
    const int H = cfg_.hidden_size, I = cfg_.intermediate_size, hd = cfg_.head_dim, nh = cfg_.n_heads, nkv = cfg_.n_kv_heads;
    void* s = stream_;
    const float scale = 1.0f / sqrtf((float)hd);
    const size_t kv_layer = (size_t)cfg_.max_seq_len * nkv * hd;
    const Views act = views(1);
    auto project_add = [&](const DevTensor& w, const float* x, int kind) -> int {
        const DevTensor* const wp = &w;
        float* y = tp_world_ > 1 ? tp_slot() : hidden_;
        NT_TRY(decode_project(&wp, &y, 1, x, nullptr, tp_world_ > 1 ? nullptr : hidden_, kind));
        return tp_world_ > 1 ? tp_allreduce(hidden_, H) : (int)NTK_OK;
    };

    for (int i = first; i < last_layer; ++i) {
        const LayerWeights& L = layers_[i];
        const DevTensor* const qkv[3] = {&L.wq, &L.wk, &L.wv};
        float* const qkv_out[3] = {act.q, act.k, act.v};
        NT_TRY(decode_project(qkv, qkv_out, 3, hidden_, &L.attn_norm, nullptr, 1));
        const int fused = fuse_attention_ ? attention_in_wo(L, i) : (int)NTK_E_SHAPE;
        if (fused != NTK_OK) {
            if (!not_taken(fused)) return fused;
            uint16_t* kc = kv_q8_ ? nullptr : k_cache_ + (size_t)i * kv_layer;
            uint16_t* vc = kv_q8_ ? nullptr : v_cache_ + (size_t)i * kv_layer;
            prof_mark(1, true);
            if (kv_q8_)
                NT_TRY(ntk_attention_decode_q8(act.attn_out, act.q, act.k, act.v, k_cache_q8_ + (size_t)i * kv_q8_layer_bytes_,
                                               v_cache_q8_ + (size_t)i * kv_q8_layer_bytes_, d_pos_, rope_inv_freq_, nh, nkv, hd, cfg_.max_seq_len, scale,
                                               cfg_.rope_theta, cfg_.rope_freq_scale, kv_q8_splits(attn_regime_), attn_scratch_, s));
            else if (attn_regime_ == 0)
                NT_TRY(ntk_attention_decode_fused(act.attn_out, act.q, act.k, act.v, kc, vc, d_pos_, rope_inv_freq_, nh, nkv, hd,
                                                  cfg_.max_seq_len, scale, cfg_.rope_theta, cfg_.rope_freq_scale, s));
            else
                NT_TRY((attn_merge_ ? ntk_attention_decode_split_merged : ntk_attention_decode_split)(
                    act.attn_out, act.q, act.k, act.v, kc, vc, d_pos_, rope_inv_freq_, nh, nkv, hd, cfg_.max_seq_len, scale, cfg_.rope_theta,
                    cfg_.rope_freq_scale, attention_splits(attn_regime_, hd), attn_scratch_, s));
            prof_mark(1, false);
            NT_TRY(project_add(L.wo, act.attn_out, 2));
        }
        const DevTensor* const ffn[2] = {&L.w_gate, &L.w_up};
        float* const ffn_out[2] = {act.gate, act.up};
        const bool pair = is_quant(L.w_gate.dtype) && L.w_gate.dtype == L.w_up.dtype;
        if (pair) prof_mark(0, true);
        NT_TRY(decode_project(ffn, ffn_out, 2, hidden_, &L.ffn_norm, nullptr, 4, pair, !pair));
        if (pair) prof_mark(0, false);
        else NT_TRY(ntk_silu_mul(act.gate, act.gate, act.up, I, s));
        NT_TRY(project_add(L.w_down, act.gate, 8));
    }
    return NTK_OK;
}

void Model::pick_attention_regime() {
    attn_regime_ = (attn_scratch_ && (cfg_.head_dim == 64 || cfg_.head_dim == 128 || cfg_.head_dim == 256))
                       ? attention_regime(host_pos_, cfg_.head_dim) : 0;
    ++host_pos_;
}

int Model::decode_step_fused(bool greedy, bool use_graph) {
    pick_attention_regime();
    if (!use_graph) return enqueue_token(greedy);
    ihipGraphExec_t*& slot = graphs_[greedy ? 1 : 0][use_persistent_now() ? kPersistentSlot : attn_regime_];
    hipStream_t st = static_cast<hipStream_t>(stream_);
    if (!slot) {
        hipGraphExec_t ex = nullptr;
        NT_TRY(capture_graph(st, tp_world_ > 1 ? hipStreamCaptureModeRelaxed : hipStreamCaptureModeThreadLocal, [&] { return enqueue_token(greedy); }, &ex));
        slot = reinterpret_cast<ihipGraphExec_t*>(ex);
    }
    return hipGraphLaunch(reinterpret_cast<hipGraphExec_t>(slot), st) == hipSuccess ? NTK_OK : NTK_E_LAUNCH;
}

int Model::profile_token(float ms[4], int calls[4], bool coarse) {
    std::vector<Timed> rec;
    rec.reserve(1024);
    prof_ = &rec;
    prof_coarse_ = coarse;
    pick_attention_regime();
    int rc = enqueue_token(true);
    if (coarse && !rec.empty()) {
        void* e = ntk_event_create();
        ntk_event_record(e, stream_);
        rec.back().b = e;
    }
    prof_ = nullptr;
    prof_coarse_ = false;
    if (rc == NTK_OK) rc = ntk_stream_synchronize(stream_);
    for (int c = 0; c < 4; ++c) { ms[c] = 0.0f; calls[c] = 0; }
    for (auto& t : rec) {
        float m = 0.0f;
        if (t.a && t.b && ntk_event_elapsed_ms(t.a, t.b, &m) == NTK_OK) { ms[t.cls] += m; calls[t.cls] += t.n; }
        ++calls[3];
    }
    for (auto& t : rec) {
        if (t.a && !t.shared_a) ntk_event_destroy(t.a);
        if (t.b) ntk_event_destroy(t.b);
    }
    return rc;
}

}
```

### ntransformer_amd/csrc/engine/model_load.cpp

```cpp
#include "model_impl.h"

namespace nt {

int Model::upload(DevTensor& dst, const void* host, int dtype, int64_t in_f, int64_t out_f, size_t nbytes) {
    void* d = nt_hip_malloc(padded_bytes(nbytes));
    if (!d) { err_ = "out of device memory"; return NTK_E_NOMEM; }
    allocs_.push_back(d);
    if (host && nbytes) {
        if (hipMemcpy(d, host, nbytes, hipMemcpyHostToDevice) != hipSuccess) { err_ = "weight upload (H2D copy) failed"; return NTK_E_LAUNCH; }
    }
    dst.ptr = d; dst.dtype = dtype; dst.in_f = in_f; dst.out_f = out_f; dst.nbytes = nbytes;
    weight_bytes_ += nbytes;
    return NTK_OK;
}

int Model::slice_columns(void* dst, const void* src, int dtype, int64_t out_f, int64_t in_f, int rank, int world) {
    if (!dst || !src) return NTK_E_NULL;
    if (world < 1 || rank < 0 || rank >= world || in_f % world != 0) return NTK_E_SHAPE;
    const int64_t in_l = in_f / world;
    const size_t rb_full = ntk_row_bytes(dtype, in_f), rb_loc = ntk_row_bytes(dtype, in_l);
    if (!rb_full || !rb_loc || rb_loc * (size_t)world != rb_full) return NTK_E_SHAPE;
    const uint8_t* s8 = static_cast<const uint8_t*>(src);
    uint8_t* d8 = static_cast<uint8_t*>(dst);
    for (int64_t r = 0; r < out_f; ++r) memcpy(d8 + (size_t)r * rb_loc, s8 + (size_t)r * rb_full + (size_t)rank * rb_loc, rb_loc);
// ... 165 lines not shown
            fr / 1073741824.0);
    return NTK_OK;
}

int Model::repack_one(DevTensor& t) {
    if (t.rp || !t.ptr) return NTK_OK;
    if (t.out_f <= 0 || t.out_f > 0x7FFFFFFF || t.in_f <= 0 || t.in_f > 32768) return NTK_OK;
    const bool q8 = t.dtype == NTK_DT_Q8_0;
    const size_t n = q8 ? ntk_q8l_bytes((int)t.out_f, (int)t.in_f) : ntk_rp_bytes(t.dtype, (int)t.out_f, (int)t.in_f);
    if (n == 0 || n > 0xFFFFFFF0ull) return NTK_OK;
    void* d = nt_hip_malloc(n + 256);
    if (!d) return NTK_E_NOMEM;
    allocs_.push_back(d);
    const int st = q8 ? ntk_q8l_pack(d, t.ptr, (int)t.out_f, (int)t.in_f, stream_) : ntk_rp_pack(d, t.ptr, (int)t.out_f, (int)t.in_f, t.dtype, stream_);
    if (st != NTK_OK) { err_ = std::string("decode repack failed: ") + ntk_status_string(st); return st; }
    t.rp = d;
    t.rp_bytes = n;
    repack_bytes_ += n;
    return NTK_OK;
}

int Model::repack_all() {
    int rc = NTK_OK;
    auto one = [&](DevTensor& t) { const int st = repack_one(t); if (st != NTK_OK && rc == NTK_OK) rc = st; return st; };
    for (auto& L : layers_) {
        if (one(L.*kLayerMatrices[0]) == NTK_E_NOMEM) break;
        for (size_t k = 1; k < kLayerMatrices.size(); ++k) one(L.*kLayerMatrices[k]);
        if (rc == NTK_E_NOMEM) break;
    }
    if (rc != NTK_E_NOMEM) one(output_);
    repack_done_ = true;
    const int sy = ntk_stream_synchronize(stream_);
    return rc != NTK_OK ? rc : sy;
}

int Model::drop_raw_all() {
    size_t need = 0;
    auto goes = [&](const DevTensor& t) { return t.rp && t.dtype != NTK_DT_Q8_0 && !(output_tied_ && t.ptr == token_embd_.ptr); };
    auto grp = [&](std::initializer_list<DevTensor*> ts) {
        size_t g = 0;
        for (DevTensor* t : ts) if (goes(*t)) g += padded_bytes(t->nbytes);
        need = std::max(need, g);
    };
    for (auto& L : layers_) { grp({&L.wq, &L.wk, &L.wv}); grp({&L.wo}); grp({&L.w_gate, &L.w_up}); grp({&L.w_down}); }
    grp({&output_});
    if (need == 0) return NTK_OK;
    if (!raw_scratch_ || raw_scratch_bytes_ < need) {
        void* d = nt_hip_malloc(need);
        if (!d) { fprintf(stderr, "warning: no device memory for the unpack scratch: the GGUF bytes stay resident beside the repack\n"); repack_ = 1; return NTK_OK; }
        allocs_.push_back(d);
        raw_scratch_ = d; raw_scratch_bytes_ = need;
    }
    auto drop = [&](DevTensor& t) {
        if (!t.ptr || !goes(t)) return;
        auto it = std::find(allocs_.begin(), allocs_.end(), t.ptr);
        if (it != allocs_.end()) allocs_.erase(it);
        nt_hip_free(t.ptr);
        t.ptr = nullptr;
        raw_freed_bytes_ += t.nbytes;
    };
    NT_TRY(ntk_stream_synchronize(stream_));
    for_each_projection(drop);
    return NTK_OK;
}

int Model::restore_raw_all() {
    int rc = NTK_OK;
    auto back = [&](DevTensor& t) {
        if (t.ptr || !t.rp || rc != NTK_OK) return;
        void* d = nt_hip_malloc(padded_bytes(t.nbytes));
        if (!d) { rc = NTK_E_NOMEM; return; }
        const int st = ntk_rp_unpack(d, t.rp, (int)t.out_f, (int)t.in_f, t.dtype, stream_);
        if (st != NTK_OK) { nt_hip_free(d); rc = st; return; }
        allocs_.push_back(d);
        t.ptr = d;
        raw_freed_bytes_ -= t.nbytes;
    };
    for_each_projection(back);
    const int sy = ntk_stream_synchronize(stream_);
    return rc != NTK_OK ? rc : sy;
}

const void* Model::raw_of(const DevTensor& t) {
    if (t.ptr) return t.ptr;
    if (!t.rp || !raw_scratch_) { raw_err_ = NTK_E_NULL; return nullptr; }
    const size_t n = padded_bytes(t.nbytes);
    if (raw_cursor_ + n > raw_scratch_bytes_) {
        if (!raw_err_) raw_err_ = NTK_E_NOMEM;
        return nullptr;
    }
    void* d = static_cast<uint8_t*>(raw_scratch_) + raw_cursor_;
    raw_cursor_ += n;
    const int st = ntk_rp_unpack(d, t.rp, (int)t.out_f, (int)t.in_f, t.dtype, stream_);
    if (st != NTK_OK) { raw_err_ = st; return nullptr; }
    return d;
}

int Model::alloc_buffers() {
    const size_t S = (size_t)cfg_.max_seq_len, H = (size_t)cfg_.hidden_size, L = (size_t)cfg_.n_layers;
    const size_t per = (size_t)cfg_.n_kv_heads * cfg_.head_dim;
    auto dev = [&](size_t bytes, bool zero) -> void* {
        void* p = nt_hip_malloc(bytes + 256);
        if (p) { allocs_.push_back(p); if (zero) nt_hip_memset(p, 0, bytes); }
        return p;
    };
    if (S * per * sizeof(uint16_t) >= 0xF0000000ull) { err_ = "context too long: one layer's K cache must stay below 3.75 GiB (32-bit row offsets)"; return NTK_E_SHAPE; }
    const size_t kvb = L * S * per * sizeof(uint16_t);
    if (kv_q8_) {
        if (cfg_.head_dim != 128 || cfg_.n_kv_heads <= 0 || cfg_.n_heads % cfg_.n_kv_heads != 0 || cfg_.n_heads / cfg_.n_kv_heads > 16) {
            err_ = "kv_cache=q8_0 needs head_dim 128 and at most 16 query heads per KV head (this model: head_dim " + std::to_string(cfg_.head_dim) +
                   ", " + std::to_string(cfg_.n_kv_heads > 0 ? cfg_.n_heads / cfg_.n_kv_heads : 0) + " query heads per KV head)";
            return NTK_E_SHAPE;
        }
        if (tp_world_ > 1) { err_ = "kv_cache=q8_0 is not supported with tensor parallelism"; return NTK_E_SHAPE; }
        if (fuse_attention_) { err_ = "kv_cache=q8_0 is not supported with the attention-inside-Wo launch (fuse_attention)"; return NTK_E_SHAPE; }
        kv_q8_layer_bytes_ = ntk_kv_q8_cache_bytes((int)S, cfg_.n_kv_heads, cfg_.head_dim);
        k_cache_q8_ = (uint8_t*)dev(L * kv_q8_layer_bytes_, true);
        v_cache_q8_ = (uint8_t*)dev(L * kv_q8_layer_bytes_, true);
        kv_f16_k_ = (uint16_t*)dev(S * per * sizeof(uint16_t), true);
        kv_f16_v_ = (uint16_t*)dev(S * per * sizeof(uint16_t), true);
        if (!k_cache_q8_ || !v_cache_q8_ || !kv_f16_k_ || !kv_f16_v_) { err_ = "buffer allocation failed (8-bit KV cache)"; return NTK_E_NOMEM; }
        kv_cache_bytes_ = 2ull * L * kv_q8_layer_bytes_ + 2ull * S * per * sizeof(uint16_t);
    } else {
        k_cache_ = (uint16_t*)dev(kvb, true);
        v_cache_ = (uint16_t*)dev(kvb, true);
        kv_cache_bytes_ = 2ull * kvb;
    }
    slot_k_.assign(1, k_cache_);
    slot_v_.assign(1, v_cache_);
    if (sequences_ > 1) {
        if (kv_q8_) { err_ = "sequences > 1 is not supported with kv_cache=q8_0"; return NTK_E_SHAPE; }
        if (tp_world_ > 1) { err_ = "sequences > 1 is not supported with tensor parallelism"; return NTK_E_SHAPE; }
        if ((size_t)sequences_ > S) { err_ = "sequences = " + std::to_string(sequences_) + " needs a context of at least as many positions (this load: " + std::to_string(S) + ")"; return NTK_E_SHAPE; }
        for (int i = 1; i < sequences_; ++i) {
            slot_k_.push_back((uint16_t*)dev(kvb, true));
            slot_v_.push_back((uint16_t*)dev(kvb, true));
            if (!slot_k_.back() || !slot_v_.back()) { err_ = "buffer allocation failed (KV cache of sequence slot " + std::to_string(i) + ")"; return NTK_E_NOMEM; }
            kv_cache_bytes_ += 2ull * kvb;
        }
    }
    hidden_ = (float*)dev(std::max<size_t>(S, 2) * H * 4, false);
    residual_ = (float*)dev(std::max<size_t>(S, 2) * H * 4, false);
    logits_ = (float*)dev((size_t)cfg_.vocab_size * 4, false);
    const size_t attn_ws = S * (size_t)(2 * cfg_.n_heads + 2 * cfg_.n_kv_heads) * cfg_.head_dim;
    const size_t ffn_ws = 2 * S * (size_t)cfg_.intermediate_size;
    workspace_floats_ = std::max(attn_ws, ffn_ws);
    workspace_ = (float*)dev(workspace_floats_ * 4, false);
    positions_ = (int*)dev(S * 4, false);
    tokens_dev_ = (int*)dev(S * 4, false);
    d_pos_ = (int*)dev(64, true);
    d_token_ = (int*)dev(64, true);
    argmax_scratch_ = (float*)dev(2 * 1024 * 4, false);
    rope_inv_freq_ = (float*)dev((size_t)cfg_.head_dim / 2 * 4 + 64, false);
    row_max_ = (float*)dev((size_t)S * 2 * 4, true);
    attn_scratch_ = (float*)dev(ntk_attention_split_scratch_bytes(cfg_.n_heads, cfg_.head_dim, kMaxAttnSplits), true);
    h_token_ = (int*)nt_hip_malloc_host(64);
    h_ring_ = (unsigned long long*)nt_hip_malloc_host(64);
    if (h_ring_) memset(h_ring_, 0, 64);
    sample_scratch_ = dev(ntk_sample_scratch_bytes(cfg_.vocab_size), false);
    attn_sync_ = (unsigned*)dev(4096, true);
    {
        const int H = cfg_.hidden_size, I = cfg_.intermediate_size, qkv = (cfg_.n_heads + 2 * cfg_.n_kv_heads) * cfg_.head_dim;
        const int shapes[][2] = {{H, qkv}, {H, cfg_.n_heads * cfg_.head_dim}, {H, cfg_.n_kv_heads * cfg_.head_dim}, {cfg_.n_heads * cfg_.head_dim, H},
                                 {H, 2 * I}, {H, I}, {I, H}};
        gemm_ws_bytes_ = 0;
        for (const auto& sh : shapes) gemm_ws_bytes_ = std::max(gemm_ws_bytes_, ntk_gemm_quant_workspace_bytes(sh[0], sh[1]));
    }
    gemm_ws_ = dev(gemm_ws_bytes_, false);
    gemm_ws2_ = dev(gemm_ws_bytes_, false);
    if (tp_world_ > 1) {
        tp_max_floats_ = S * H;
        tp_comm_ = ntk_tp_comm_alloc(ntk_tp_comm_bytes(tp_max_floats_));
        if (tp_comm_) allocs_.push_back(tp_comm_);
        if (!tp_comm_ || ntk_tp_comm_reset(tp_comm_, nullptr) != NTK_OK || ntk_device_synchronize() != NTK_OK) { err_ = "communication buffer allocation failed"; return NTK_E_NOMEM; }
    }
    d_recent_ = (int*)dev(kRecentCap * 4, false);
    h_recent_ = (int*)nt_hip_malloc_host(kRecentCap * 4);
    if ((!kv_q8_ && (!k_cache_ || !v_cache_)) || !hidden_ || !residual_ || !logits_ || !workspace_ || !positions_ || !tokens_dev_ ||
        !d_pos_ || !d_token_ || !argmax_scratch_ || !h_token_ || !h_ring_) {
        err_ = "buffer allocation failed";
        return NTK_E_NOMEM;
    }
    *h_token_ = 0;
    if (rope_inv_freq_) {
        std::vector<float> f((size_t)cfg_.head_dim / 2);
        for (int i = 0; i < cfg_.head_dim / 2; ++i) f[i] = 1.0f / powf(cfg_.rope_theta, (2.0f * i) / cfg_.head_dim);
        nt_hip_memcpy_h2d(rope_inv_freq_, f.data(), f.size() * 4);
    }
    if (sequences_ > 1) { NT_TRY(batch_buffers()); NT_TRY(batch_sample_buffers()); }
    return NTK_OK;
}

}
```

### ntransformer_amd/ops.py

```python
from __future__ import annotations

import ctypes as C
from typing import Optional, Sequence

import numpy as np

from . import _lib
from ._lib import GemvSeg, check


class DeviceBuffer:

    def __init__(self, nbytes: int):
        self.nbytes = int(nbytes)
        self.ptr = _lib.lib().nt_hip_malloc(max(self.nbytes, 1))
        if not self.ptr:
            raise _lib.NtkError(-7, "hipMalloc(%d)" % nbytes)

    @classmethod
    def from_numpy(cls, a: np.ndarray) -> "DeviceBuffer":
        a = np.ascontiguousarray(a)
        b = cls(a.nbytes)
        if a.nbytes:
            _lib.lib().nt_hip_memcpy_h2d(b.ptr, a.ctypes.data_as(C.c_void_p), a.nbytes)
# ... 195 lines not shown
    for i, (W, y, rows, dt) in enumerate(segs):
        arr[i].W, arr[i].y, arr[i].rows, arr[i].dtype = _p(W), _p(y), rows, int(dt)
    d = _lib.GemmDesc()
    d.segs, d.nseg, d.X, d.n_tokens, d.in_features, d.resid = arr, len(segs), _p(X), n_tokens, in_features, _p(resid)
    d.workspace, d.workspace_bytes, d.reuse_x, d.row_max = ws.ptr, n, int(reuse_x), _p(row_max)
    d.partials = C.pointer(partials) if partials is not None else None
    d.weights_repacked = 1 if repacked else 0
    d.full_form = 1 if full_form else 0
    L.ntk_gemm_quant_f16.argtypes = [C.POINTER(_lib.GemmDesc), C.c_void_p]
    st = L.ntk_gemm_quant_f16(C.byref(d), stream)
    if keep is not None:
        keep.append(ws)
    else:
        synchronize()
    return st


def gemm_quant_f16_prepared(segs, X, n_tokens, in_features, resid=None, row_max=None, stream=None):
    L = _lib.lib()
    L.ntk_gemm_quant_workspace_bytes.restype = C.c_size_t
    n = int(L.ntk_gemm_quant_workspace_bytes(C.c_int(in_features), C.c_int(sum(r for _, _, r, _ in segs))))
    ws = DeviceBuffer(n)
    arr = (GemvSeg * len(segs))()
    for i, (W, y, rows, dt) in enumerate(segs):
        arr[i].W, arr[i].y, arr[i].rows, arr[i].dtype = _p(W), _p(y), rows, int(dt)
    d = _lib.GemmDesc()
    d.segs, d.nseg, d.X, d.n_tokens, d.in_features, d.resid = arr, len(segs), _p(X), n_tokens, in_features, _p(resid)
    d.workspace, d.workspace_bytes, d.reuse_x, d.row_max = ws.ptr, n, 0, _p(row_max)
    L.ntk_gemm_quant_f16.argtypes = [C.POINTER(_lib.GemmDesc), C.c_void_p]

    def call(_keep=(ws, arr, d)):
        return L.ntk_gemm_quant_f16(C.byref(d), stream)
    return call


def gemm_quant_ws_multi(segs, X, n_tokens, in_features, stream=None, repacked=False):
    return _gemm_quant_f16(segs, X, n_tokens, in_features, stream=stream, repacked=repacked)


def gemm_quant_ws(Y, W, X, n_tokens, out_features, in_features, dtype, resid=None, stream=None, repacked=False):
    st = _gemm_quant_f16([(W, Y, out_features, dtype)], X, n_tokens, in_features, resid=resid, stream=stream, repacked=repacked)
    synchronize()
    return st


def gemm_quant_ws_rm(Y, W, X, n_tokens, out_features, in_features, dtype, row_max, resid=None, stream=None):
    st = _gemm_quant_f16([(W, Y, out_features, dtype)], X, n_tokens, in_features, resid=resid, row_max=row_max, stream=stream)
    synchronize()
    return st


def gemm_deferred_then_consumer(kind, W, X, n_tokens, rows, in_features, dtype, row_max=None, **kw):
    L = _lib.lib()
    pt = _lib.GemmPartials()
    keep = []
    if kind == "norm":
        y = DeviceBuffer(n_tokens * rows * 4)
        in_place = kw.get("in_place", True)
        check(_gemm_quant_f16([(W, kw["hidden"] if in_place else y, rows, dtype)], X, n_tokens, in_features, resid=kw["hidden"] if in_place else None,
                              row_max=row_max, partials=pt, keep=keep), "gemm deferred")
        L.ntk_reduce_rmsnorm_rowmax.argtypes = [C.c_void_p, C.POINTER(_lib.GemmPartials), C.c_void_p, C.c_float, C.c_void_p, C.c_void_p, C.c_void_p, C.c_void_p]
        check(L.ntk_reduce_rmsnorm_rowmax(_p(kw["hidden"]), C.byref(pt), _p(kw["weight"]), kw["eps"], _p(kw["x_out"]), _p(kw["row_max_out"]), _p(kw.get("zero")), None),
              "reduce_rmsnorm_rowmax")
    else:
        yg, yu = DeviceBuffer(n_tokens * rows * 4), DeviceBuffer(n_tokens * rows * 4)
        check(_gemm_quant_f16([(W[0], yg, rows, dtype), (W[1], yu, rows, dtype)], X, n_tokens, in_features, row_max=row_max, partials=pt, keep=keep),
              "gemm multi deferred")
        L.ntk_reduce_silu_mul_rowmax.argtypes = [C.c_void_p, C.POINTER(_lib.GemmPartials), C.c_void_p, C.c_void_p]
        check(L.ntk_reduce_silu_mul_rowmax(_p(kw["output"]), C.byref(pt), _p(kw["row_max_out"]), None), "reduce_silu_mul_rowmax")
    synchronize()
    return int(pt.nsplit)


def rope_kv_store(q, k, v, positions, seq_len, n_heads, n_kv_heads, head_dim, theta_base, freq_scale, interleaved, k_cache, v_cache, start_pos, max_seq):
    check(_lib.lib().ntk_rope_kv_store(_p(q), _p(k), _p(v), _p(positions), seq_len, n_heads, n_kv_heads, head_dim, theta_base, freq_scale,
                                       int(bool(interleaved)), _p(k_cache), _p(v_cache), start_pos, max_seq, None), "rope_kv_store")


def gemm_workspace(in_features, rows):
    L = _lib.lib()
    L.ntk_gemm_quant_workspace_bytes.restype = C.c_size_t
    return DeviceBuffer(int(L.ntk_gemm_quant_workspace_bytes(C.c_int(in_features), C.c_int(rows))))


def prepare_x(kind, workspace, n_tokens, width, **kw):
    L = _lib.lib()
    vp, i, f = C.c_void_p, C.c_int, C.c_float
    if kind == "x":
        L.ntk_gemm_prepare_x.argtypes = [vp, i, i, vp, vp]
        st = L.ntk_gemm_prepare_x(_p(kw["X"]), n_tokens, width, workspace.ptr, None)
    elif kind == "rmsnorm":
        L.ntk_rmsnorm_prepare_x.argtypes = [vp, vp, vp, i, i, f, vp, vp]
        st = L.ntk_rmsnorm_prepare_x(_p(kw["output"]), _p(kw["input"]), _p(kw["weight"]), n_tokens, width, kw["eps"], workspace.ptr, None)
    elif kind == "silu":
        L.ntk_silu_mul_prepare_x.argtypes = [vp, vp, vp, i, i, vp, vp]
        st = L.ntk_silu_mul_prepare_x(_p(kw["output"]), _p(kw["gate"]), _p(kw["up"]), n_tokens, width, workspace.ptr, None)
    elif kind == "reduce_rmsnorm":
        L.ntk_reduce_rmsnorm_prepare_x.argtypes = [vp, C.POINTER(_lib.GemmPartials), vp, f, vp, vp, vp]
        st = L.ntk_reduce_rmsnorm_prepare_x(_p(kw["hidden"]), C.byref(kw["partials"]), _p(kw["weight"]), kw["eps"], _p(kw["x_out"]), workspace.ptr, None)
    else:
        L.ntk_reduce_silu_mul_prepare_x.argtypes = [vp, C.POINTER(_lib.GemmPartials), vp, vp]
        st = L.ntk_reduce_silu_mul_prepare_x(_p(kw["output"]), C.byref(kw["partials"]), workspace.ptr, None)
    synchronize()
    return st


def launch_rmsnorm_rowmax(output, input, weight, n_tokens, hidden_size, eps, row_max, zero_tokens=None, stream=None):
    check(_lib.lib().ntk_rmsnorm_rowmax(_p(output), _p(input), _p(weight), n_tokens, hidden_size, eps, _p(row_max), _p(zero_tokens), stream), "rmsnorm_rowmax")


def launch_silu_mul_rowmax(output, gate, up, n_tokens, width, row_max, stream=None):
    check(_lib.lib().ntk_silu_mul_rowmax(_p(output), _p(gate), _p(up), n_tokens, width, _p(row_max), stream), "silu_mul_rowmax")


def sample_top_k(logits, n, recent, n_recent, repeat_penalty, temperature, top_k, top_p, r, d_out, stream=None):
    L = _lib.lib()
    L.ntk_sample_scratch_bytes.restype = C.c_size_t
    scratch = DeviceBuffer(int(L.ntk_sample_scratch_bytes(C.c_int(n))))
    L.ntk_sample_top_k.argtypes = [C.c_void_p, C.c_int, C.c_void_p, C.c_int, C.c_float, C.c_float, C.c_int, C.c_float, C.c_float,
                                   C.c_void_p, C.c_void_p, C.c_void_p, C.c_void_p]
    st = L.ntk_sample_top_k(_p(logits), n, _p(recent), n_recent, repeat_penalty, temperature, top_k, top_p, r, _p(d_out), None,
                            _p(scratch), stream)
    synchronize()
    return st


def sample_rows_top_k(logits, n_rows, vocab, ld, recent, recent_ld, rows, d_out, stream=None, null=()):
    L = _lib.lib()
    if not isinstance(rows, _lib.SampleRows):
        sr = _lib.SampleRows()
        for b, (temperature, top_k, top_p, repeat_penalty, r, n_recent) in enumerate(rows):
            sr.temperature[b], sr.top_k[b], sr.top_p[b], sr.repeat_penalty[b], sr.r[b], sr.n_recent[b] = temperature, top_k, top_p, repeat_penalty, r, n_recent
        rows = sr
    scratch = DeviceBuffer(int(L.ntk_sample_rows_scratch_bytes(min(max(n_rows, 1), 16), min(max(vocab, 1), 1 << 20))))
    arg = lambda name, v: None if name in null else v
    st = L.ntk_sample_rows_top_k(arg("logits", _p(logits)), n_rows, vocab, ld, _p(recent), recent_ld, arg("rows", C.pointer(rows)), arg("d_out", _p(d_out)), None,
                                 arg("scratch", _p(scratch)), stream)
    synchronize()
    return st


def gemm_quant(Y, W, X, n_tokens, out_features, in_features, dtype, resid=None, stream=None):
    check(_lib.lib().ntk_gemm_quant(_p(Y), _p(W), _p(X), n_tokens, out_features, in_features, int(dtype), _p(resid),
                                    stream), "gemm_quant")


def attention_decode_fused(output, q, k, v, k_cache, v_cache, d_pos, n_heads, n_kv_heads, head_dim, max_seq, scale,
                           theta_base, freq_scale=1.0, inv_freq=None, stream=None):
    check(_lib.lib().ntk_attention_decode_fused(_p(output), _p(q), _p(k), _p(v), _p(k_cache), _p(v_cache), _p(d_pos),
                                                _p(inv_freq), n_heads, n_kv_heads, head_dim, max_seq, scale, theta_base,
                                                freq_scale, stream), "attention_decode_fused")


def attention_decode_split(output, q, k, v, k_cache, v_cache, d_pos, n_heads, n_kv_heads, head_dim, max_seq, scale,
                           theta_base, nsplit, freq_scale=1.0, inv_freq=None, stream=None):
    scratch = DeviceBuffer(int(_lib.lib().ntk_attention_split_scratch_bytes(n_heads, head_dim, nsplit)))
    check(_lib.lib().ntk_attention_decode_split(_p(output), _p(q), _p(k), _p(v), _p(k_cache), _p(v_cache), _p(d_pos),
                                                _p(inv_freq), n_heads, n_kv_heads, head_dim, max_seq, scale, theta_base,
                                                freq_scale, nsplit, _p(scratch), stream), "attention_decode_split")
    synchronize()
    return None


def attention_decode_split_merged(output, q, k, v, k_cache, v_cache, d_pos, n_heads, n_kv_heads, head_dim, max_seq, scale,
                                  theta_base, nsplit, freq_scale=1.0, inv_freq=None, stream=None, launches=1):
    scratch = DeviceBuffer(int(_lib.lib().ntk_attention_split_scratch_bytes(n_heads, head_dim, nsplit)))
    check(_lib.lib().ntk_attention_split_scratch_init(_p(scratch), n_heads, stream), "attention_split_scratch_init")
    for _ in range(launches):
        check(_lib.lib().ntk_attention_decode_split_merged(_p(output), _p(q), _p(k), _p(v), _p(k_cache), _p(v_cache), _p(d_pos),
                                                           _p(inv_freq), n_heads, n_kv_heads, head_dim, max_seq, scale, theta_base,
                                                           freq_scale, nsplit, _p(scratch), stream), "attention_decode_split_merged")
    synchronize()
    return None


def attention_decode_batch(output, q, k, v, k_caches, v_caches, positions, n_rows, n_heads, n_kv_heads, head_dim, max_seq, scale,
                           theta_base, nsplit=1, freq_scale=1.0, inv_freq=None, stream=None, table=True):
    L = _lib.lib()
    kv = _lib.KvBatch()
    for b, (kc, vc) in enumerate(zip(k_caches, v_caches)):
        kv.k[b], kv.v[b] = _p(kc), _p(vc)
    scratch = DeviceBuffer(max(n_rows, 1) * int(L.ntk_attention_split_scratch_bytes(n_heads, head_dim, nsplit)))
    check(L.ntk_attention_decode_batch(_p(output), _p(q), _p(k), _p(v), C.addressof(kv) if table else None, _p(positions), n_rows, _p(inv_freq),
                                       n_heads, n_kv_heads, head_dim, max_seq, scale, theta_base, freq_scale, nsplit, _p(scratch), stream),
          "attention_decode_batch")
    synchronize()
    return None


def embed_rows(out, table, tokens, n_tokens, hidden, dtype, stream=None, allow_unsupported=False):
    st = _lib.lib().ntk_embed_rows(_p(out), _p(table), _p(tokens), n_tokens, hidden, int(dtype), stream)
    if not (allow_unsupported and st == -1):
        check(st, "embed_rows")
    return st


def argmax(logits, n, d_out_token, scratch, h_mirror=None, stream=None):
    check(_lib.lib().ntk_argmax(_p(logits), n, _p(d_out_token), _p(h_mirror), _p(scratch), stream), "argmax")


def logprob_rows(logits, n_rows, vocab, ld, targets, logprob, top1=None, stream=None):
    check(_lib.lib().ntk_logprob_rows(_p(logits), n_rows, vocab, ld, _p(targets), _p(logprob), _p(top1), stream), "logprob_rows")


def advance_pos(d_pos, stream=None):
    check(_lib.lib().ntk_advance_pos(_p(d_pos), stream), "advance_pos")


def sclk_mhz(stream=None) -> float:
    import numpy as np
    b = DeviceBuffer.zeros(24)
    check(_lib.lib().ntk_debug_sclk(_p(b), stream), "sclk probe")
    synchronize(stream)
    v = b.numpy(np.uint64)
    return 100.0 * float(v[0]) / max(float(v[1]), 1.0)


class SclkSpan:

    def __enter__(self):
        L = _lib.lib()
        self.flag, self.out = DeviceBuffer.zeros(8), DeviceBuffer.zeros(24)
        self.mhz = None
        check(L.ntk_debug_sclk_begin(_p(self.flag), _p(self.out), L.ntk_stream(1)), "sclk begin")
        return self

    def __exit__(self, *exc):
        import numpy as np
        L = _lib.lib()
        check(L.ntk_debug_sclk_end(_p(self.flag), L.ntk_stream(2)), "sclk end")
        check(L.ntk_stream_synchronize(L.ntk_stream(2)), "sync")
        check(L.ntk_stream_synchronize(L.ntk_stream(1)), "sync")
        v = self.out.numpy(np.uint64)
        if v[1] > 0:
            self.mhz = 100.0 * float(v[0]) / float(v[1])
        return False
```

Measured before the change: 551.9 tokens/s.

## Precompute per-step RoPE cos/sin table and reorder attention blocks by KV group

Adds a small device RoPE table of cos/sin values for the next position, filled by spare threads inside the greedy argmax/advance kernel (or by a position-advance kernel). The short-context fused decode attention kernel reads this table, checked against a position tag, instead of calling sincosf in every head block of every layer. The fused attention launch also maps blocks so heads sharing a KV head are spread across block indices when n_kv_heads is a multiple of 8. The cost is extra table bookkeeping and a fallback path when the tag does not match.

```diff
diff --git a/include/ntk_engine.h b/include/ntk_engine.h
--- a/include/ntk_engine.h
+++ b/include/ntk_engine.h
@@ -40,6 +40,17 @@
                                void* v_cache, const int* d_pos, const float* inv_freq, int n_heads, int n_kv_heads,
                                int head_dim, int max_seq, float scale, float theta_base, float freq_scale,
                                void* stream);
+#define NTK_ATTN_PLAIN_ORDER 1
+int ntk_attention_decode_fused_ex(float* output, const float* q, const float* k, const float* v, void* k_cache,
+                                  void* v_cache, const int* d_pos, const float* inv_freq, int n_heads, int n_kv_heads,
+                                  int head_dim, int max_seq, float scale, float theta_base, float freq_scale,
+                                  const void* rope_table, int variant, void* stream);
+size_t ntk_rope_table_bytes(int head_dim);
+int ntk_rope_table_write(void* rope_table, const float* inv_freq, int head_dim, float freq_scale, const int* d_pos, void* stream);
+int ntk_argmax_advance_rope(const float* logits, int n, int* d_out_token, int* h_mirror, unsigned long long* h_ring4, int* d_pos, float* scratch,
+                            void* rope_table, const float* inv_freq, int head_dim, float freq_scale, void* stream);
+int ntk_advance_pos_rope(int* d_pos, void* rope_table, const float* inv_freq, int head_dim, float freq_scale, void* stream);
+int ntk_debug_rope_table_slot(int pos, int i, int* out3);
 
 size_t ntk_attention_split_scratch_bytes(int n_heads, int head_dim, int nsplit);
 int ntk_attention_decode_split(float* output, const float* q, const float* k, const float* v, void* k_cache,
diff --git a/ntransformer_amd/_lib.py b/ntransformer_amd/_lib.py
--- a/ntransformer_amd/_lib.py
+++ b/ntransformer_amd/_lib.py
@@ -121,6 +121,12 @@
         "ntk_attention_split_scratch_init": (i, [vp, i, vp]),
         "ntk_attention_decode_split_merged": (i, [vp, vp, vp, vp, vp, vp, vp, vp, i, i, i, i, f, f, f, i, vp, vp]),
         "ntk_attention_decode_fused": (i, [vp, vp, vp, vp, vp, vp, vp, vp, i, i, i, i, f, f, f, vp]),
+        "ntk_attention_decode_fused_ex": (i, [vp, vp, vp, vp, vp, vp, vp, vp, i, i, i, i, f, f, f, vp, i, vp]),
+        "ntk_rope_table_bytes": (C.c_size_t, [i]),
+        "ntk_rope_table_write": (i, [vp, vp, i, f, vp, vp]),
+        "ntk_argmax_advance_rope": (i, [vp, i, vp, vp, vp, vp, vp, vp, vp, i, f, vp]),
+        "ntk_advance_pos_rope": (i, [vp, vp, vp, i, f, vp]),
+        "ntk_debug_rope_table_slot": (i, [i, i, C.POINTER(i)]),
         "ntk_attention_decode_batch": (i, [vp, vp, vp, vp, vp, vp, i, vp, i, i, i, i, f, f, f, i, vp, vp]),
         "ntk_kv_q8_cache_bytes": (C.c_size_t, [i, i, i]),
         "ntk_kv_store_q8": (i, [vp, vp, vp, vp, i, i, i, i, i, vp]),
diff --git a/ntransformer_amd/csrc/attention.hip b/ntransformer_amd/csrc/attention.hip
--- a/ntransformer_amd/csrc/attention.hip
+++ b/ntransformer_amd/csrc/attention.hip
@@ -38,9 +38,11 @@
 __global__ __launch_bounds__(256) void attention_decode_fused_v3_kernel(
     float* __restrict__ output, const float* __restrict__ q, const float* __restrict__ k, const float* __restrict__ v,
     uint16_t* __restrict__ kc, uint16_t* __restrict__ vc, const int* __restrict__ d_pos, const float* __restrict__ inv_freq,
-    int n_heads, int n_kv_heads, int hd, int max_seq, float scale, float theta, float fscale) {
+    int n_heads, int n_kv_heads, int hd, int max_seq, float scale, float theta, float fscale, int kv_order, const float* __restrict__ rope_cs) {
+    const int i = (int)blockIdx.x;
+    const int head = kv_order ? (i % n_kv_heads) * (n_heads / n_kv_heads) + i / n_kv_heads : i;
     attention_decode_walk<LPR, D, false>(output, q, k, v, kc, vc, d_pos, inv_freq, n_heads, n_kv_heads, hd, max_seq, scale, theta, fscale,
-                                         (int)blockIdx.x, 0, 1);
+                                         head, 0, 1, rope_cs);
 }
 
 template <int LPR, int D, bool MERGE>
@@ -367,12 +369,14 @@
                                  ntk::resolve_stream(stream));
 }
 
-int ntk_attention_decode_fused(float* output, const float* q, const float* k, const float* v, void* k_cache, void* v_cache,
-                               const int* d_pos, const float* inv_freq, int n_heads, int n_kv_heads, int head_dim, int max_seq,
-                               float scale, float theta_base, float freq_scale, void* stream) {
+static int attention_decode_fused_impl(float* output, const float* q, const float* k, const float* v, void* k_cache, void* v_cache,
+                                       const int* d_pos, const float* inv_freq, int n_heads, int n_kv_heads, int head_dim, int max_seq,
+                                       float scale, float theta_base, float freq_scale, const void* rope_table, int variant, void* stream) {
     if (!output || !q || !k || !v || !k_cache || !v_cache || !d_pos) return NTK_E_NULL;
     if (n_heads <= 0 || n_kv_heads <= 0 || n_heads % n_kv_heads != 0 || head_dim <= 0 || (head_dim & 1) || max_seq <= 0)
         return NTK_E_SHAPE;
+    if (variant & ~NTK_ATTN_PLAIN_ORDER) return NTK_E_SHAPE;
+    if (reinterpret_cast<uintptr_t>(rope_table) & 7) return NTK_E_ALIGN;
     if ((size_t)max_seq * n_kv_heads * head_dim * 2 >= 0xF0000000ull) return NTK_E_SHAPE;
     hipStream_t st = ntk::resolve_stream(stream);
     const bool aligned = (reinterpret_cast<uintptr_t>(k_cache) & 15) == 0 && (reinterpret_cast<uintptr_t>(v_cache) & 15) == 0;
@@ -381,8 +385,10 @@
     if (aligned && (head_dim == 128 || head_dim == 64 || head_dim == 256)) {
         const int G = 4 * (64 / (head_dim / 8));
         const size_t lds = sizeof(float) * ((size_t)3 * head_dim + 2 * G + (size_t)G * head_dim);
+        const int kv_order = (n_kv_heads % 8 == 0 && !(variant & NTK_ATTN_PLAIN_ORDER)) ? 1 : 0;
+        const float* rope_cs = inv_freq ? static_cast<const float*>(rope_table) : nullptr;
 #define NTK_ATTV(...) hipLaunchKernelGGL((ntk::attention_decode_fused_v3_kernel<__VA_ARGS__>), dim3(n_heads), dim3(256), lds, st, output, q, k, v, \
-                                           k16, v16, d_pos, inv_freq, n_heads, n_kv_heads, head_dim, max_seq, scale, theta_base, freq_scale)
+                                           k16, v16, d_pos, inv_freq, n_heads, n_kv_heads, head_dim, max_seq, scale, theta_base, freq_scale, kv_order, rope_cs)
         if (head_dim == 128) NTK_ATTV(16, 4);
         else if (head_dim == 64) NTK_ATTV(8, 4);
         else NTK_ATTV(32, 4);
@@ -397,6 +403,22 @@
     hipLaunchKernelGGL(ntk::attention_decode_fused_kernel<0>, dim3(n_heads), dim3(256), lds, st, output, q, k, v, k16, v16, d_pos,
                        n_heads, n_kv_heads, head_dim, max_seq, scale, theta_base, freq_scale);
     return ntk::last_launch_status();
+}
+
+int ntk_attention_decode_fused(float* output, const float* q, const float* k, const float* v, void* k_cache, void* v_cache,
+                               const int* d_pos, const float* inv_freq, int n_heads, int n_kv_heads, int head_dim, int max_seq,
+                               float scale, float theta_base, float freq_scale, void* stream) {
+    return attention_decode_fused_impl(output, q, k, v, k_cache, v_cache, d_pos, inv_freq, n_heads, n_kv_heads, head_dim, max_seq, scale, theta_base,
+                                       freq_scale, nullptr, 0, stream);
+}
+
+int ntk_attention_decode_fused_ex(float* output, const float* q, const float* k, const float* v, void* k_cache, void* v_cache,
+                                  const int* d_pos, const float* inv_freq, int n_heads, int n_kv_heads, int head_dim, int max_seq,
+                                  float scale, float theta_base, float freq_scale, const void* rope_table, int variant, void* stream) {
+    static const int force = NTK_TUNE_ENV_INT("NTK_ATTN_SHORT_FORCE", -1);
+    if (force >= 0) { variant = (force & 1) ? NTK_ATTN_PLAIN_ORDER : 0; if (force & 2) rope_table = nullptr; }
+    return attention_decode_fused_impl(output, q, k, v, k_cache, v_cache, d_pos, inv_freq, n_heads, n_kv_heads, head_dim, max_seq, scale, theta_base,
+                                       freq_scale, rope_table, variant, stream);
 }
 
 size_t ntk_attention_split_scratch_bytes(int n_heads, int head_dim, int nsplit) {
diff --git a/ntransformer_amd/csrc/attention_decode.hip.h b/ntransformer_amd/csrc/attention_decode.hip.h
--- a/ntransformer_amd/csrc/attention_decode.hip.h
+++ b/ntransformer_amd/csrc/attention_decode.hip.h
@@ -1,6 +1,7 @@
 #pragma once
 #include "common.hip.h"
 #include "attention_merge.hip.h"
+#include "rope_table.hip.h"
 #include <cfloat>
 #include <cstdlib>
 
@@ -190,7 +191,7 @@
     float* __restrict__ output, const float* __restrict__ q, const float* __restrict__ k, const float* __restrict__ v,
     uint16_t* __restrict__ kc, uint16_t* __restrict__ vc, const int* __restrict__ d_pos, const float* __restrict__ inv_freq,
     const int n_heads, const int n_kv_heads, const int hd, const int max_seq, const float scale, const float theta, const float fscale,
-    const int head, const int sp, const int nsplit) {
+    const int head, const int sp, const int nsplit, const float* __restrict__ rope_cs = nullptr) {
     constexpr int PPW = 64 / LPR, NW = 4, G = NW * PPW;
     constexpr float EMPTY = -3.0e38f;
     extern __shared__ __attribute__((aligned(16))) float lds[];
@@ -219,6 +220,17 @@
         freq = inv_freq ? inv_freq[ri] : 1.0f / (float)pow((double)theta, (double)((2.0f * ri) / hd));
         if (half_dim > 64) { in_c = src[ri + 64]; in_d = src[ri + 64 + half_dim]; }
     }
+    const bool tab = rope_cs != nullptr && inv_freq != nullptr;
+    int tab_tag = kRopeTableNoTag;
+    float tab_c0 = 0.0f, tab_s0 = 0.0f, tab_c1 = 0.0f, tab_s1 = 0.0f;
+    if (tab) {
+        tab_tag = *reinterpret_cast<const int*>(rope_cs);
+        if (rot) {
+            const RopeTableSlot s0 = rope_table_slot(0, ri), s1 = rope_table_slot(0, ri + 64);
+            tab_c0 = rope_cs[s0.cos_word]; tab_s0 = rope_cs[s0.sin_word];
+            if (half_dim > 64) { tab_c1 = rope_cs[s1.cos_word]; tab_s1 = rope_cs[s1.sin_word]; }
+        }
+    }
     float vin0 = 0.0f, vin1 = 0.0f;
     const int vi = tid - 128;
     if (role >= 2) {
@@ -242,10 +254,13 @@
     const bool writer = (head % group == 0) && sp == 0 && pos < max_seq;
     uint16_t st_h[4] = {0, 0, 0, 0};
     if (rot) {
-        auto rotate = [&](const int i, const float a, const float b, const float f, uint16_t& ha, uint16_t& hb) {
-            const float angle = pos * f * fscale;
-            float c, sn;
-            sincosf(angle, &sn, &c);
+        const bool from_table = tab && tab_tag == pos;
+        auto rotate = [&](const int i, const float a, const float b, const float f, const float tc, const float ts, uint16_t& ha, uint16_t& hb) {
+            float c = tc, sn = ts;
+            if (!from_table) {
+                const float angle = pos * f * fscale;
+                sincosf(angle, &sn, &c);
+            }
             float ra, rb;
             rope_rotate(a, b, c, sn, ra, rb);
             if (role == 0) { qs[i] = ra; qs[i + half_dim] = rb; }
@@ -254,11 +269,11 @@
                 kx[i] = h2f(ha); kx[i + half_dim] = h2f(hb);
             }
         };
-        rotate(ri, in_a, in_b, freq, st_h[0], st_h[1]);
+        rotate(ri, in_a, in_b, freq, tab_c0, tab_s0, st_h[0], st_h[1]);
         if (half_dim > 64) {
             const int i2 = ri + 64;
             const float f2 = inv_freq ? inv_freq[i2] : 1.0f / (float)pow((double)theta, (double)((2.0f * i2) / hd));
-            rotate(i2, in_c, in_d, f2, st_h[2], st_h[3]);
+            rotate(i2, in_c, in_d, f2, tab_c1, tab_s1, st_h[2], st_h[3]);
         }
     }
     if (role >= 2) {
diff --git a/ntransformer_amd/csrc/elementwise.hip b/ntransformer_amd/csrc/elementwise.hip
--- a/ntransformer_amd/csrc/elementwise.hip
+++ b/ntransformer_amd/csrc/elementwise.hip
@@ -1,4 +1,5 @@
 #include "common.hip.h"
+#include "rope_table.hip.h"
 #include <cfloat>
 
 namespace ntk {
@@ -160,6 +161,26 @@
 }
 __global__ void advance_pos_kernel(int* p) { if (threadIdx.x == 0 && blockIdx.x == 0) *p += 1; }
 
+__device__ __forceinline__ void rope_table_fill(float* __restrict__ tab, const float* __restrict__ inv_freq, const int half_dim, const float fscale,
+                                                const int pos, const int t, const int nthreads) {
+    for (int i = t; i < half_dim; i += nthreads) {
+        const RopeTableSlot sl = rope_table_slot(pos, i);
+        const float angle = pos * inv_freq[i] * fscale;
+        float c, sn;
+        sincosf(angle, &sn, &c);
+        tab[sl.cos_word] = c;
+        tab[sl.sin_word] = sn;
+        if (i == 0) { reinterpret_cast<int*>(tab)[0] = sl.tag; reinterpret_cast<int*>(tab)[1] = 0; }
+    }
+}
+__global__ __launch_bounds__(128) void rope_table_kernel(float* __restrict__ tab, const float* __restrict__ inv_freq, int half_dim, float fscale,
+                                                         int* __restrict__ d_pos, int delta) {
+    const int pos = *d_pos + delta;
+    __syncthreads();
+    rope_table_fill(tab, inv_freq, half_dim, fscale, pos, (int)threadIdx.x, (int)blockDim.x);
+    if (delta && threadIdx.x == 0) *d_pos = pos;
+}
+
 __global__ __launch_bounds__(64) void sclk_probe_kernel(unsigned long long* out) {
     const unsigned long long t0 = __builtin_amdgcn_s_memtime(), r0 = __builtin_amdgcn_s_memrealtime();
     unsigned long long r1 = r0;
@@ -188,19 +209,23 @@
 
 __global__ __launch_bounds__(256) void argmax_advance_stage2(const float* __restrict__ sv, const int* __restrict__ si, int nblk,
                                                              int* __restrict__ d_out, int* __restrict__ h_mirror,
-                                                             unsigned long long* __restrict__ h_ring, int* __restrict__ d_pos) {
+                                                             unsigned long long* __restrict__ h_ring, int* __restrict__ d_pos,
+                                                             float* __restrict__ rope_tab, const float* __restrict__ inv_freq, int half_dim,
+                                                             float fscale) {
     __shared__ float rv[4];
     __shared__ int ri[4];
+    const int pos0 = *d_pos;
     float v = -FLT_MAX;
     int idx = 0x7FFFFFFF;
     for (int i = threadIdx.x; i < nblk; i += blockDim.x) amax_merge(v, idx, sv[i], si[i]);
     for (int off = 32; off > 0; off >>= 1) amax_merge(v, idx, __shfl_xor(v, off, 64), __shfl_xor(idx, off, 64));
     if ((threadIdx.x & 63) == 0) { rv[threadIdx.x >> 6] = v; ri[threadIdx.x >> 6] = idx; }
     __syncthreads();
+    if (rope_tab && threadIdx.x >= 192) rope_table_fill(rope_tab, inv_freq, half_dim, fscale, pos0 + 1, (int)threadIdx.x - 192, 64);
     if (threadIdx.x == 0) {
         for (int w = 1; w < 4; ++w) amax_merge(v, idx, rv[w], ri[w]);
         if (idx == 0x7FFFFFFF) idx = 0;
-        const int pos = *d_pos;
+        const int pos = pos0;
         *d_out = idx;
         if (h_mirror) *h_mirror = idx;
         if (h_ring)
@@ -311,17 +336,43 @@
     hipLaunchKernelGGL(argmax_stage2, dim3(1), dim3(256), 0, st, (const float*)sv, (const int*)si, nblk, d_out_token, h_mirror);
     return last_launch_status();
 }
-int ntk_argmax_advance(const float* logits, int n, int* d_out_token, int* h_mirror, unsigned long long* h_ring4, int* d_pos, float* scratch,
-                       void* stream) {
+static int rope_table_args_ok(const void* rope_table, const float* inv_freq, int head_dim) {
+    if (!inv_freq) return NTK_E_NULL;
+    if (head_dim <= 0 || (head_dim & 1) || head_dim > 256) return NTK_E_SHAPE;
+    return (reinterpret_cast<uintptr_t>(rope_table) & 7) ? NTK_E_ALIGN : NTK_OK;
+}
+int ntk_argmax_advance_rope(const float* logits, int n, int* d_out_token, int* h_mirror, unsigned long long* h_ring4, int* d_pos, float* scratch,
+                            void* rope_table, const float* inv_freq, int head_dim, float freq_scale, void* stream) {
     if (!logits || !d_out_token || !scratch || !d_pos) return NTK_E_NULL;
     if (n <= 0) return NTK_E_SHAPE;
+    if (rope_table) { const int rc = rope_table_args_ok(rope_table, inv_freq, head_dim); if (rc != NTK_OK) return rc; }
     const int nblk = n < 256 * 8 ? 1 : (n / (256 * 8) < 1024 ? n / (256 * 8) : 1024);
     float* sv = scratch;
     int* si = reinterpret_cast<int*>(scratch + 1024);
     hipStream_t st = resolve_stream(stream);
     hipLaunchKernelGGL(argmax_stage1, dim3(nblk), dim3(256), 0, st, logits, n, sv, si);
-    hipLaunchKernelGGL(argmax_advance_stage2, dim3(1), dim3(256), 0, st, (const float*)sv, (const int*)si, nblk, d_out_token, h_mirror, h_ring4, d_pos);
-    return last_launch_status();
+    hipLaunchKernelGGL(argmax_advance_stage2, dim3(1), dim3(256), 0, st, (const float*)sv, (const int*)si, nblk, d_out_token, h_mirror, h_ring4, d_pos,
+                       static_cast<float*>(rope_table), inv_freq, head_dim / 2, freq_scale);
+    return last_launch_status();
+}
+int ntk_argmax_advance(const float* logits, int n, int* d_out_token, int* h_mirror, unsigned long long* h_ring4, int* d_pos, float* scratch,
+                       void* stream) {
+    return ntk_argmax_advance_rope(logits, n, d_out_token, h_mirror, h_ring4, d_pos, scratch, nullptr, nullptr, 0, 0.0f, stream);
+}
+size_t ntk_rope_table_bytes(int head_dim) { return head_dim > 0 && !(head_dim & 1) && head_dim <= 256 ? rope_table_words(head_dim) * 4 : 0; }
+int ntk_rope_table_write(void* rope_table, const float* inv_freq, int head_dim, float freq_scale, const int* d_pos, void* stream) {
+    if (!rope_table || !d_pos) return NTK_E_NULL;
+    const int rc = rope_table_args_ok(rope_table, inv_freq, head_dim);
+    if (rc != NTK_OK) return rc;
+    hipLaunchKernelGGL(rope_table_kernel, dim3(1), dim3(128), 0, resolve_stream(stream), static_cast<float*>(rope_table), inv_freq, head_dim / 2,
+                       freq_scale, const_cast<int*>(d_pos), 0);
+    return last_launch_status();
+}
+int ntk_debug_rope_table_slot(int pos, int i, int* out3) {
+    if (!out3) return NTK_E_NULL;
+    const RopeTableSlot sl = rope_table_slot(pos, i);
+    out3[0] = sl.tag; out3[1] = sl.cos_word; out3[2] = sl.sin_word;
+    return NTK_OK;
 }
 int ntk_debug_sclk(unsigned long long* d_out2, void* stream) {
     if (!d_out2) return NTK_E_NULL;
@@ -345,5 +396,14 @@
     hipLaunchKernelGGL(advance_pos_kernel, dim3(1), dim3(64), 0, resolve_stream(stream), d_pos);
     return last_launch_status();
 }
-
-}
+int ntk_advance_pos_rope(int* d_pos, void* rope_table, const float* inv_freq, int head_dim, float freq_scale, void* stream) {
+    if (!rope_table) return ntk_advance_pos(d_pos, stream);
+    if (!d_pos) return NTK_E_NULL;
+    const int rc = rope_table_args_ok(rope_table, inv_freq, head_dim);
+    if (rc != NTK_OK) return rc;
+    hipLaunchKernelGGL(rope_table_kernel, dim3(1), dim3(128), 0, resolve_stream(stream), static_cast<float*>(rope_table), inv_freq, head_dim / 2,
+                       freq_scale, d_pos, 1);
+    return last_launch_status();
+}
+
+}
diff --git a/ntransformer_amd/csrc/engine/capi.cpp b/ntransformer_amd/csrc/engine/capi.cpp
--- a/ntransformer_amd/csrc/engine/capi.cpp
+++ b/ntransformer_amd/csrc/engine/capi.cpp
@@ -71,6 +71,7 @@
     else if (k == "prefill_row_max") E(e)->model().set_prefill_row_max(on);
     else if (k == "prefill_fused_split") E(e)->model().set_prefill_fused_split(on);
     else if (k == "attention_merge") return E(e)->model().set_attention_merge(on);
+    else if (k == "rope_table") return E(e)->model().set_rope_table(on);
     else if (k == "repack") return E(e)->model().set_repack(atoi(value));
     else if (k == "persistent") { E(e)->options().persistent = on; E(e)->model().set_persistent(atoi(value)); }
     else if (k == "score_rows") {
diff --git a/ntransformer_amd/csrc/engine/model.cpp b/ntransformer_amd/csrc/engine/model.cpp
--- a/ntransformer_amd/csrc/engine/model.cpp
+++ b/ntransformer_amd/csrc/engine/model.cpp
@@ -49,6 +49,7 @@
     kv_capture_ = nullptr; kv_capture_layer_ = -1; kv_capture_T_ = 0;
     k_cache_q8_ = v_cache_q8_ = nullptr; kv_f16_k_ = kv_f16_v_ = nullptr; kv_q8_layer_bytes_ = 0; kv_cache_bytes_ = 0;
     hidden_ = residual_ = workspace_ = logits_ = argmax_scratch_ = rope_inv_freq_ = attn_scratch_ = row_max_ = nullptr;
+    rope_cs_ = nullptr;
     positions_ = tokens_dev_ = d_pos_ = d_token_ = nullptr;
     score_logits_ = score_logprob_ = nullptr; score_targets_ = score_top1_ = nullptr; score_cap_ = 0;
     score_ws_ = nullptr; score_ws_bytes_ = 0;
@@ -96,6 +97,16 @@
     return NTK_OK;
 }
 
+int Model::set_rope_table(bool on) {
+    if (on == rope_table_) return NTK_OK;
+    if (!layers_.empty()) {
+        NT_TRY(sync());
+        drop_graphs();
+    }
+    rope_table_ = on;
+    return NTK_OK;
+}
+
 int Model::set_repack(int level) {
     level = level < 0 ? 0 : level > 3 ? 3 : level;
     if (shares_weights_) { err_ = "set_repack: this sequence shares another model's tensors"; return NTK_E_SHAPE; }
@@ -142,6 +153,7 @@
 int Model::set_device_pos(int pos) {
     host_pos_ = pos;
     NT_TRY(ntk_memcpy_h2d_async(d_pos_, &pos, 4, stream_));
+    if (rope_table()) NT_TRY(ntk_rope_table_write(rope_table(), rope_inv_freq_, cfg_.head_dim, cfg_.rope_freq_scale, d_pos_, stream_));
     NT_TRY(ntk_stream_synchronize(stream_));
     if (h_ring_) memset(h_ring_, 0, 64);
     return NTK_OK;
diff --git a/ntransformer_amd/csrc/engine/model.h b/ntransformer_amd/csrc/engine/model.h
--- a/ntransformer_amd/csrc/engine/model.h
+++ b/ntransformer_amd/csrc/engine/model.h
@@ -95,6 +95,7 @@
     void set_prefill_row_max(bool on) { prefill_row_max_ = on; }
     void set_prefill_fused_split(bool on) { prefill_fused_split_ = on; }
     int set_attention_merge(bool on);
+    int set_rope_table(bool on);
     int set_repack(int level);
     bool repack() const { return repack_ != 0; }
     int repack_level() const { return repack_; }
@@ -224,6 +225,9 @@
     int* h_recent_ = nullptr;
     static constexpr int kRecentCap = kMaxRecent;
     float* rope_inv_freq_ = nullptr;
+    void* rope_cs_ = nullptr;
+    bool rope_table_ = true;
+    void* rope_table() const { return rope_table_ && rope_inv_freq_ && cfg_.head_dim <= 256 ? rope_cs_ : nullptr; }
     void* stream_ = nullptr;
     bool batched_prefill_ = true;
     struct Timed { int cls; void* a; void* b; int n; bool shared_a; };
diff --git a/ntransformer_amd/csrc/engine/model_decode.cpp b/ntransformer_amd/csrc/engine/model_decode.cpp
--- a/ntransformer_amd/csrc/engine/model_decode.cpp
+++ b/ntransformer_amd/csrc/engine/model_decode.cpp
@@ -39,8 +39,9 @@
         if (timed) prof_mark(0, false);
     }
     prof_mark(2, true);
-    if (greedy) NT_TRY(ntk_argmax_advance(logits_, cfg_.vocab_size, d_token_, h_token_, h_ring_, d_pos_, argmax_scratch_, s));
-    else NT_TRY(ntk_advance_pos(d_pos_, s));
+    if (greedy) NT_TRY(ntk_argmax_advance_rope(logits_, cfg_.vocab_size, d_token_, h_token_, h_ring_, d_pos_, argmax_scratch_, rope_table(), rope_inv_freq_,
+                                               cfg_.head_dim, cfg_.rope_freq_scale, s));
+    else NT_TRY(ntk_advance_pos_rope(d_pos_, rope_table(), rope_inv_freq_, cfg_.head_dim, cfg_.rope_freq_scale, s));
     if (tp_world_ > 1) NT_TRY(ntk_tp_advance_epoch(tp_comm_, s));
     prof_mark(2, false);
     return NTK_OK;
@@ -136,8 +137,8 @@
                                                v_cache_q8_ + (size_t)i * kv_q8_layer_bytes_, d_pos_, rope_inv_freq_, nh, nkv, hd, cfg_.max_seq_len, scale,
                                                cfg_.rope_theta, cfg_.rope_freq_scale, kv_q8_splits(attn_regime_), attn_scratch_, s));
             else if (attn_regime_ == 0)
-                NT_TRY(ntk_attention_decode_fused(act.attn_out, act.q, act.k, act.v, kc, vc, d_pos_, rope_inv_freq_, nh, nkv, hd,
-                                                  cfg_.max_seq_len, scale, cfg_.rope_theta, cfg_.rope_freq_scale, s));
+                NT_TRY(ntk_attention_decode_fused_ex(act.attn_out, act.q, act.k, act.v, kc, vc, d_pos_, rope_inv_freq_, nh, nkv, hd,
+                                                     cfg_.max_seq_len, scale, cfg_.rope_theta, cfg_.rope_freq_scale, rope_table(), 0, s));
             else
                 NT_TRY((attn_merge_ ? ntk_attention_decode_split_merged : ntk_attention_decode_split)(
                     act.attn_out, act.q, act.k, act.v, kc, vc, d_pos_, rope_inv_freq_, nh, nkv, hd, cfg_.max_seq_len, scale, cfg_.rope_theta,
diff --git a/ntransformer_amd/csrc/engine/model_load.cpp b/ntransformer_amd/csrc/engine/model_load.cpp
--- a/ntransformer_amd/csrc/engine/model_load.cpp
+++ b/ntransformer_amd/csrc/engine/model_load.cpp
@@ -341,6 +341,10 @@
     d_token_ = (int*)dev(64, true);
     argmax_scratch_ = (float*)dev(2 * 1024 * 4, false);
     rope_inv_freq_ = (float*)dev((size_t)cfg_.head_dim / 2 * 4 + 64, false);
+    if (const size_t tb = ntk_rope_table_bytes(cfg_.head_dim)) {
+        rope_cs_ = dev(tb + 64, false);
+        if (rope_cs_) nt_hip_memset(rope_cs_, 0xFF, tb);
+    }
     row_max_ = (float*)dev((size_t)S * 2 * 4, true);
     attn_scratch_ = (float*)dev(ntk_attention_split_scratch_bytes(cfg_.n_heads, cfg_.head_dim, kMaxAttnSplits), true);
     h_token_ = (int*)nt_hip_malloc_host(64);
diff --git a/ntransformer_amd/csrc/rope_table.hip.h b/ntransformer_amd/csrc/rope_table.hip.h
--- /dev/null
+++ b/ntransformer_amd/csrc/rope_table.hip.h
@@ -0,0 +1,23 @@
+#pragma once
+#include <stddef.h>
+
+#if defined(__HIPCC__)
+#define NTK_ROPE_TABLE_HD __host__ __device__
+#else
+#define NTK_ROPE_TABLE_HD
+#endif
+
+namespace ntk {
+
+constexpr int kRopeTableNoTag = -1;
+
+struct RopeTableSlot {
+    int tag;
+    int cos_word;
+    int sin_word;
+};
+
+NTK_ROPE_TABLE_HD inline RopeTableSlot rope_table_slot(const int pos, const int i) { return {pos, 2 + 2 * i, 3 + 2 * i}; }
+NTK_ROPE_TABLE_HD inline size_t rope_table_words(const int head_dim) { return 2 + 2 * (size_t)(head_dim / 2); }
+
+}
diff --git a/ntransformer_amd/ops.py b/ntransformer_amd/ops.py
--- a/ntransformer_amd/ops.py
+++ b/ntransformer_amd/ops.py
@@ -371,6 +371,26 @@
                                                 freq_scale, stream), "attention_decode_fused")
 
 
+ATTN_PLAIN_ORDER = 1
+
+
+def attention_decode_fused_ex(output, q, k, v, k_cache, v_cache, d_pos, n_heads, n_kv_heads, head_dim, max_seq, scale,
+                              theta_base, rope_table=None, variant=0, freq_scale=1.0, inv_freq=None, stream=None):
+    check(_lib.lib().ntk_attention_decode_fused_ex(_p(output), _p(q), _p(k), _p(v), _p(k_cache), _p(v_cache), _p(d_pos),
+                                                   _p(inv_freq), n_heads, n_kv_heads, head_dim, max_seq, scale, theta_base,
+                                                   freq_scale, _p(rope_table), variant, stream), "attention_decode_fused_ex")
+
+
+def rope_table_new(head_dim):
+    b = DeviceBuffer(int(_lib.lib().ntk_rope_table_bytes(head_dim)))
+    _lib.lib().nt_hip_memset(b.ptr, 0xFF, b.nbytes)
+    return b
+
+
+def rope_table_write(table, inv_freq, head_dim, d_pos, freq_scale=1.0, stream=None):
+    check(_lib.lib().ntk_rope_table_write(_p(table), _p(inv_freq), head_dim, freq_scale, _p(d_pos), stream), "rope_table_write")
+
+
 def attention_decode_split(output, q, k, v, k_cache, v_cache, d_pos, n_heads, n_kv_heads, head_dim, max_seq, scale,
                            theta_base, nsplit, freq_scale=1.0, inv_freq=None, stream=None):
     scratch = DeviceBuffer(int(_lib.lib().ntk_attention_split_scratch_bytes(n_heads, head_dim, nsplit)))
```

New measurement: 551.2 tokens/s. No clear change (-0.1%).
